# lyclyc52/Instance_NeRF

Measured on AMD Instinct MI355X. Metric: Msamples/sec (train+infer) 3D-FRONT 800x800 at 1/2/4/8 MI355X; PSNR parity, higher is better.
Workload: dtype f32; 1 GPU; render 800x800 synthetic 3D-FRONT-like room, hash-grid NeRF L=16 F=2 T=6119864 sigma+rgb (BASELINE configs[1]), one view per step per GPU; parallelism=views sharded over 1 GPU(s), no data-path collective

## Files before the change

### include/inr.h

```cpp
#ifndef INR_H
#define INR_H

#include <stdint.h>

#ifdef __cplusplus
extern "C" {
#endif

#define INR_ABI_VERSION 13
#define INR_MAX_LEVELS 16

enum {
  INR_OK = 0,
  INR_EINVAL = -1,
  INR_ELAUNCH = -2,
  INR_ENODEV = -3
};

typedef void* inr_stream_t;

enum {
  INR_NUMERICS_TABLE_F16 = 1,
  INR_NUMERICS_MLP_F16 = 2
};

typedef struct inr_grid_desc {
  int32_t num_levels;
  int32_t level_dim;
  uint32_t offsets[INR_MAX_LEVELS + 1];
  float scales[INR_MAX_LEVELS];
  uint32_t resolutions[INR_MAX_LEVELS];
  uint32_t hashed[INR_MAX_LEVELS];
} inr_grid_desc;

int inr_abi_version(void);
const char* inr_last_error(void);
int inr_device_info(int32_t device, int64_t* props);
int inr_set_overlap_placement(int32_t on);
int inr_set_march_mode(int32_t mode);

int inr_get_rays(const float* poses, int64_t B, float fx, float fy, float cx, float cy, int32_t W,
                 const int64_t* inds , int64_t n, float* rays_o, float* rays_d, inr_stream_t s);

int inr_sample_training_batch(const float* pose , float fx, float fy, float cx, float cy, int32_t H, int32_t W,
                              const float* image , int32_t channels, const int32_t* mask ,
                              int32_t num_instances, int64_t seed, int64_t step, int64_t n, int64_t* inds ,
                              float* rays_o, float* rays_d, float* rgb , int64_t* labels ,
                              inr_stream_t s);

int inr_near_far_from_aabb(const float* rays_o, const float* rays_d, const float* aabb ,
                           int64_t N, float min_near, float* nears, float* fars, inr_stream_t s);
int inr_near_far_from_aabb_skip(const float* rays_o, const float* rays_d, const float* aabb , int64_t N,
                                float min_near, const int64_t* labels, int64_t ignore_index, float* nears, float* fars,
                                inr_stream_t s);

int inr_morton3D(const int32_t* coords , int64_t N, int32_t* indices, inr_stream_t s);
int inr_morton3D_invert(const int32_t* indices, int64_t N, int32_t* coords , inr_stream_t s);
int inr_packbits(const float* grid, int64_t n_bytes, float thresh, uint8_t* bitfield, inr_stream_t s);

int inr_mark_untrained_grid(const float* poses, int32_t B, float fx, float fy, float cx, float cy, int32_t H,
                            int32_t cascade, float bound, float* grid , inr_stream_t s);
int inr_occ_cell_positions(const int32_t* morton_idx, const float* noise, int64_t n, int32_t H, float cascade_bound,
                           float* xyz , inr_stream_t s);
int inr_occ_update(float* grid , const float* sigma , const int32_t* morton_idx ,
                   int64_t n_cells, int64_t m, float decay, float density_scale, float* tmp, double* mean_sum,
                   inr_stream_t s);
int inr_packbits_mean(const float* grid, int64_t n_cells , const double* mean_sum, float density_thresh,
                      uint8_t* bitfield, float* mean_out , const int32_t* counters ,
                      int32_t n_counters, int32_t counter_stride , double* stats_out ,
                      inr_stream_t s);
int64_t inr_occ_sample_workspace_bytes(int64_t n_cells);
int inr_occ_sample_cells(const float* grid , int64_t n_cells, const float* u ,
                         int64_t n, int32_t* morton_idx , void* workspace, inr_stream_t s);

int inr_march_write_fills_unowned_rows(int64_t N, int32_t sample_cap, int32_t max_steps);
int64_t inr_march_workspace_bytes(int64_t N, int32_t sample_cap);
int inr_march_rays_train_count(const float* rays_o, const float* rays_d, const uint8_t* bitfield,
                               float bound, float dt_gamma, int32_t max_steps, int64_t N,
                               int32_t cascade, int32_t H, const float* nears, const float* fars,
                               const float* noises , int32_t* rays ,
                               int32_t* counter , void* workspace, int32_t sample_cap, inr_stream_t s);
int inr_march_rays_train_write(const float* rays_o, const float* rays_d, const uint8_t* bitfield,
                               float bound, float dt_gamma, int32_t max_steps, int64_t N,
                               int32_t cascade, int32_t H, int64_t M, const float* nears,
                               const float* fars, const float* noises ,
                               const int32_t* rays , float* xyzs ,
                               float* dirs , float* deltas , const void* workspace,
                               int32_t sample_cap, inr_stream_t s);

int inr_march_rays_patch_write(const float* rays_o, const float* rays_d, const uint8_t* bitfield,
                               float bound, float dt_gamma, int32_t max_steps, int64_t N,
                               int32_t cascade, int32_t H, int64_t M, const float* nears,
                               const float* fars, const float* noises ,
                               const int32_t* rays ,
                               float* xyzs, float* dirs , float* deltas,
                               const void* workspace, int32_t sample_cap, int32_t* ray_ids ,
                               int32_t normalise , inr_stream_t s);
int inr_composite_rays_patch_forward(const float* sigmas, const float* rgbs, const float* deltas,
                                     const int32_t* rays, int64_t N, int64_t M, float T_thresh,
                                     const float* extra , int32_t K,
                                     float* weights_sum, float* depth, float* image,
                                     float* extra_out , float* weights ,
                                     uint64_t* skippable ,
                                     inr_stream_t s);
int inr_project_masks_patch(const float* xyzs, const float* weights, const int32_t* rays, int64_t N, int64_t M,
                            const uint32_t* mask_words, int32_t W, int32_t L, int32_t H, const float* bbox ,
                            int32_t k_total, int32_t k_base, int32_t k_count, float* out, inr_stream_t s);

int inr_march_rays(int64_t n_alive, int32_t n_step, const int32_t* rays_alive, const float* rays_t,
                   const float* rays_o, const float* rays_d, float bound, float dt_gamma,
                   int32_t max_steps, int32_t cascade, int32_t H, const uint8_t* bitfield,
                   const float* nears, const float* fars, float* xyzs, float* dirs, float* deltas,
                   inr_stream_t s);
int inr_composite_rays(int64_t n_alive, int32_t n_step, int32_t* rays_alive, float* rays_t,
                       const float* sigmas, const float* rgbs, const float* deltas,
                       float* weights_sum, float* depth, float* image, float T_thresh,
                       const float* extra , float* extra_acc ,
                       int32_t K, inr_stream_t s);
int inr_compact_alive(const int32_t* rays_alive, int64_t n_alive, int32_t* out, int32_t* n_out,
                      inr_stream_t s);

int inr_composite_rays_train_forward(const float* sigmas, const float* rgbs, const float* deltas,
                                     const int32_t* rays, int64_t N, int64_t M, float T_thresh,
                                     const float* extra , int32_t K,
                                     float* weights_sum, float* depth, float* image,
                                     float* extra_out , float* weights ,
                                     int32_t* sample_ray , inr_stream_t s);
int inr_composite_rays_extra_forward(const float* weights , const float* extra , const int32_t* rays,
                                     int64_t N, int64_t M, int32_t K, float* extra_out ,
                                     const int64_t* labels , int32_t n_classes, int64_t ignore_index,
                                     float* grad_pix, void* workspace, float* loss_out, inr_stream_t s);
int inr_composite_rays_train_backward(const float* grad_weights_sum, const float* grad_image,
                                      const float* grad_extra_out , const float* sigmas,
                                      const float* rgbs, const float* extra, const float* deltas,
                                      const int32_t* rays, const float* weights_sum,
                                      const float* image, const float* weights ,
                                      int64_t N, int64_t M, float T_thresh, int32_t K,
                                      float* grad_sigmas, float* grad_rgbs ,
                                      float* grad_extra , const int32_t* total_dev ,
                                      inr_stream_t s);

int inr_grid_encode_forward(const float* x , const float* embeddings ,
                            const inr_grid_desc* desc , int64_t M, float bound,
                            float* out , inr_stream_t s);
int inr_grid_encode_backward(const float* x, const float* grad_out ,
                             const inr_grid_desc* desc , int64_t M, float bound,
                             float* grad_embeddings , inr_stream_t s);

int inr_grid_encode_backward_ordered(const float* x, const float* grad_out, const int32_t* order,
                                     const inr_grid_desc* desc , int64_t M, float bound,
                                     float* grad_embeddings , inr_stream_t s);
int inr_grid_encode_backward_input(const float* x, const float* grad_out , const float* embeddings,
                                   const inr_grid_desc* desc , int64_t M, float bound, float* grad_x,
                                   inr_stream_t s);
int inr_grid_encode_backward_levels(const float* x, const float* grad_out, const int32_t* order,
                                    const inr_grid_desc* desc, int64_t M, float bound, float* grad_embeddings,
                                    int32_t level_lo, int32_t level_hi, inr_stream_t s);

#define INR_GRID_FX_STATE_FLOATS 4192
int inr_grid_encode_backward_levels_fx(const float* x, const float* grad_out, const int32_t* order,
                                       const inr_grid_desc* desc, int64_t M, float bound, float* grad_embeddings,
                                       int32_t level_lo, int32_t level_hi, float* fx_state ,
                                       inr_stream_t s);
int inr_grid_grad_finish_fx(float* grad_embeddings, const inr_grid_desc* desc , int32_t level_lo,
                            int32_t level_hi, float* fx_state, inr_stream_t s);
int inr_grid_fx_update(float* fx_state, int32_t num_levels, float headroom, int32_t sum_bits , inr_stream_t s);
int inr_grid_encode_backward_levels_fx64(const float* x, const float* grad_out, const int32_t* order,
                                         const inr_grid_desc* desc, int64_t M, float bound, float* grad_embeddings,
                                         int64_t* acc64 , int32_t level_lo, int32_t level_hi, float* fx_state,
                                         inr_stream_t s);
int inr_grid_grad_finish_fx64(int64_t* acc64, float* grad_embeddings, const inr_grid_desc* desc , int32_t level_lo,
                              int32_t level_hi, float* fx_state, inr_stream_t s);

int inr_sh_encode_forward(const float* d , int64_t M, int32_t degree, float* out, inr_stream_t s);
int inr_sh_encode_backward(const float* grad_out, const float* d, int64_t M, int32_t degree,
                           float* grad_d, inr_stream_t s);
int inr_sh_table_q(const float* d , int64_t N, float* out , inr_stream_t s);

int64_t inr_nerf_packed_floats(void);
int inr_nerf_pack_weights(const float* sigma_w0, const float* sigma_w1, const float* color_w0,
                          const float* color_w1, const float* color_w2, float* packed , int32_t numerics);
int64_t inr_instance_packed_floats(int32_t K);
int inr_instance_pack_weights(const float* w0, const float* w1, const float* w2, int32_t K,
                              float* packed , int32_t numerics);
int inr_nerf_forward(const float* x, const float* d, int64_t M, const int32_t* n_samples_dev,
                     float bound, const void* embeddings, const inr_grid_desc* desc ,
                     const float* packed , float density_scale, float* sigma, float* rgb,
                     float* geo_feat, int32_t numerics, inr_stream_t s);
int inr_nerf_forward_table(const float* x01, const int32_t* ray_ids, const float* sh_table_q, int64_t M,
                           float bound, const void* embeddings, const inr_grid_desc* desc ,
                           const float* packed , float density_scale, float* sigma, float* rgb,
                           int32_t numerics, inr_stream_t s);
int64_t inr_nerf_forward_table_sliced_workspace_bytes(int64_t M);
int inr_nerf_forward_table_sliced(const float* x01, const int32_t* ray_ids, const float* sh_table_q, int64_t M,
                                  float bound, const float* embeddings, const inr_grid_desc* desc ,
                                  const float* packed , float density_scale, float* sigma, float* rgb,
                                  float* fine_ws, inr_stream_t s);
int64_t inr_nerf_bwd_packed_floats(void);
int inr_nerf_pack_weights_device(const float* sigma_w0, const float* sigma_w1, const float* color_w0,
                                 const float* color_w1, const float* color_w2, float* packed_fwd,
                                 float* packed_bwd, inr_stream_t s);
int inr_nerf_forward_train(const float* x, const float* d, int64_t M, float bound, const float* embeddings,
                           const inr_grid_desc* desc , const float* packed_fwd, float* sigma, float* rgb,
                           float* enc, float* h1, float* so, float* cin, float* c1, float* c2, inr_stream_t s);
int inr_nerf_backward(const float* grad_sigma, const float* grad_rgb, const float* rgb, const float* so,
                      const float* h1, const float* c1, const float* c2, int64_t M, float density_scale,
                      const float* packed_bwd, float* grad_o, float* grad_zc2, float* grad_zc1, float* grad_so,
                      float* grad_zh1, float* grad_enc, inr_stream_t s);
int inr_nerf_forward_enc(const float* x, const float* d, int64_t M, float bound, const float* embeddings,
                         const inr_grid_desc* desc , const float* packed_fwd, float* sigma, float* rgb,
                         float* enc, inr_stream_t s);
int inr_nerf_head_backward(const float* enc, const float* d, const float* grad_sigma, const float* grad_rgb, int64_t M,
                           float density_scale, const float* packed_fwd, const float* packed_bwd, float* grad_enc,
                           void* workspace, float* grad_ws0, float* grad_ws1, float* grad_wc0, float* grad_wc1,
                           float* grad_wc2, float* zero_buf , int64_t zero_floats, inr_stream_t s);
int64_t inr_instance_bwd_packed_floats(void);
int inr_instance_pack_weights_device(const float* w0 , const float* w1 ,
                                     const float* w2 , int32_t K, float* packed_fwd, float* packed_bwd,
                                     inr_stream_t s);
int inr_instance_forward_train(const float* x, int64_t M, float bound, const float* embeddings,
                               const inr_grid_desc* desc , const float* packed_fwd, int32_t K,
                               float* logits, float* enc, float* h1, float* h2, inr_stream_t s);
int inr_instance_backward(const float* grad_logits, int32_t K, const float* h1, const float* h2, int64_t M,
                          const float* packed_bwd, float* grad_z2, float* grad_z1, float* grad_enc,
                          inr_stream_t s);
int inr_instance_forward_enc(const float* x, int64_t M, const int32_t* n_samples_dev, float bound,
                             const float* embeddings, const inr_grid_desc* desc , const float* packed_fwd,
                             int32_t K, float* logits, float* enc, inr_stream_t s);
int64_t inr_instance_head_workspace_bytes(void);
int inr_instance_head_backward(const float* enc, const float* weights, const int32_t* sample_ray,
                               const float* grad_pix, int32_t K, int64_t N, int64_t M, const int32_t* n_samples_dev,
                               const float* scale_a , const float* scale_b ,
                               const float* packed_fwd, const float* packed_bwd, float* grad_enc, void* workspace,
                               float* grad_w0, float* grad_w1, float* grad_w2, float* zero_buf ,
                               int64_t zero_floats, inr_stream_t s);
int inr_nerf_forward_dirs(const float* x, int64_t M, float bound, const float* embeddings, const inr_grid_desc* desc ,
                          const float* packed , const float* sh_dirs, int32_t n_dirs, float* out, inr_stream_t s);
int inr_nerf_forward_lattice(const float* ax_w, const float* ax_l, const float* ax_h, int32_t W, int32_t L, int32_t H,
                             float bound, const float* embeddings, const inr_grid_desc* desc ,
                             const float* packed , const float* sh_dirs, int32_t n_dirs, float logit_min,
                             float* out, inr_stream_t s);
int inr_instance_forward(const float* x, int64_t M, const int32_t* n_samples_dev, float bound,
                         const float* embeddings, const inr_grid_desc* desc ,
                         const float* packed , int32_t K, float* logits ,
                         inr_stream_t s);
int inr_instance_lattice(const float* ax_w, const float* ax_l, const float* ax_h, int32_t W, int32_t L, int32_t H,
                         float bound, const float* nerf_embeddings, const inr_grid_desc* nerf_desc ,
                         const float* nerf_packed , float density_scale, float sigma_thresh,
                         const float* inst_embeddings, const inr_grid_desc* inst_desc ,
                         const float* inst_packed , int32_t K, uint8_t* labels, float* confidence,
                         float* density_logit, inr_stream_t s);
#define INR_INSTANCE_STATS_WORKSPACE_BYTES (512 * 64 * 8 * 4)
int inr_instance_volume_stats(const uint8_t* labels, const float* confidence, int32_t W, int32_t L, int32_t H, int32_t K,
                              void* workspace, int64_t workspace_bytes, int32_t* counts, int32_t* boxes, float* conf_sum,
                              inr_stream_t s);

int64_t inr_mesh_workspace_bytes(int32_t W, int32_t L, int32_t H, int32_t cap);
int inr_mesh_count(const float* field, int32_t field_stride, float iso, float clamp, const uint8_t* labels ,
                   int32_t select, int32_t W, int32_t L, int32_t H, int32_t cap, void* workspace, int64_t workspace_bytes,
                   int32_t* counts, inr_stream_t s);
int inr_mesh_emit(const float* field, int32_t field_stride, float iso, float clamp, const uint8_t* labels ,
                  int32_t select, const float* rgb , const float* ax_w, const float* ax_l, const float* ax_h,
                  int32_t W, int32_t L, int32_t H, float ext_w, float ext_l, float ext_h, int32_t cap,
                  const void* workspace, int64_t workspace_bytes, int32_t V, int32_t F, float* vertices, int32_t* faces,
                  float* colors , uint8_t* face_labels , inr_stream_t s);

int64_t inr_components_workspace_bytes(int32_t W, int32_t L, int32_t H);
int inr_components_label(const uint8_t* labels, int32_t W, int32_t L, int32_t H, int32_t connectivity, void* workspace,
                         int64_t workspace_bytes, int32_t* roots, inr_stream_t s);
int inr_components_filter(const uint8_t* labels, const int32_t* roots, const float* confidence , int32_t W,
                          int32_t L, int32_t H, int32_t K, int32_t first_channel, int32_t min_voxels, int32_t keep_largest,
                          void* workspace, int64_t workspace_bytes, uint8_t* labels_out, float* confidence_out ,
                          int32_t* n_components, int32_t* kept_voxels, int32_t* kept_root, inr_stream_t s);

int inr_pack_mask_bits(const float* soft, const int64_t* inds , int64_t N, int32_t k, float thresh, int64_t P,
// ... 104 lines not shown
```

### instance_nerf_amd/_lib.py

```python
import ctypes
import os
from ctypes import POINTER, Structure, c_char_p, c_float, c_int32, c_int64, c_uint32, c_void_p

import torch

_HERE = os.path.dirname(os.path.abspath(__file__))
LIB_PATH = os.environ.get("INR_LIB_PATH") or os.path.join(_HERE, "csrc", "libinr_hip.so")
MAX_LEVELS = 16
GRID_FX_STATE_FLOATS = 4192
ROI_MAX_LEVELS = 8
NUMERICS_TABLE_F16, NUMERICS_MLP_F16 = 1, 2


class GridDesc(Structure):
    _fields_ = [("num_levels", c_int32), ("level_dim", c_int32),
                ("offsets", c_uint32 * (MAX_LEVELS + 1)), ("scales", c_float * MAX_LEVELS),
                ("resolutions", c_uint32 * MAX_LEVELS), ("hashed", c_uint32 * MAX_LEVELS)]


P = c_void_p
_SIGS = {
    "inr_abi_version": (c_int32, []),
    "inr_last_error": (c_char_p, []),
    "inr_set_overlap_placement": (c_int32, [c_int32]),
    "inr_set_march_mode": (c_int32, [c_int32]),
    "inr_device_info": (c_int32, [c_int32, POINTER(c_int64)]),
    "inr_get_rays": (c_int32, [P, c_int64, c_float, c_float, c_float, c_float, c_int32, P, c_int64, P, P, P]),
    "inr_sample_training_batch": (c_int32, [P, c_float, c_float, c_float, c_float, c_int32, c_int32, P, c_int32, P, c_int32,
                                            c_int64, c_int64, c_int64, P, P, P, P, P, P]),
    "inr_near_far_from_aabb": (c_int32, [P, P, P, c_int64, c_float, P, P, P]),
    "inr_near_far_from_aabb_skip": (c_int32, [P, P, P, c_int64, c_float, P, c_int64, P, P, P]),
    "inr_morton3D": (c_int32, [P, c_int64, P, P]),
    "inr_morton3D_invert": (c_int32, [P, c_int64, P, P]),
    "inr_packbits": (c_int32, [P, c_int64, c_float, P, P]),
    "inr_mark_untrained_grid": (c_int32, [P, c_int32, c_float, c_float, c_float, c_float, c_int32, c_int32, c_float, P, P]),
    "inr_occ_cell_positions": (c_int32, [P, P, c_int64, c_int32, c_float, P, P]),
    "inr_occ_update": (c_int32, [P, P, P, c_int64, c_int64, c_float, c_float, P, P, P]),
    "inr_packbits_mean": (c_int32, [P, c_int64, P, c_float, P, P, P, c_int32, c_int32, P, P]),
    "inr_occ_sample_workspace_bytes": (c_int64, [c_int64]),
    "inr_occ_sample_cells": (c_int32, [P, c_int64, P, c_int64, P, P, P]),
    "inr_march_write_fills_unowned_rows": (c_int32, [c_int64, c_int32, c_int32]),
    "inr_march_workspace_bytes": (c_int64, [c_int64, c_int32]),
    "inr_march_rays_train_count": (c_int32, [P, P, P, c_float, c_float, c_int32, c_int64, c_int32, c_int32,
                                             P, P, P, P, P, P, c_int32, P]),
    "inr_march_rays_train_write": (c_int32, [P, P, P, c_float, c_float, c_int32, c_int64, c_int32, c_int32,
                                             c_int64, P, P, P, P, P, P, P, P, c_int32, P]),
    "inr_march_rays_patch_write": (c_int32, [P, P, P, c_float, c_float, c_int32, c_int64, c_int32, c_int32,
                                             c_int64, P, P, P, P, P, P, P, P, c_int32, P, c_int32, P]),
    "inr_nerf_bwd_packed_floats": (c_int64, []),
    "inr_nerf_pack_weights_device": (c_int32, [P, P, P, P, P, P, P, P]),
    "inr_nerf_forward_train": (c_int32, [P, P, c_int64, c_float, P, POINTER(GridDesc), P, P, P, P, P, P, P, P, P, P]),
    "inr_nerf_backward": (c_int32, [P, P, P, P, P, P, P, c_int64, c_float, P, P, P, P, P, P, P, P]),
    "inr_instance_bwd_packed_floats": (c_int64, []),
    "inr_instance_pack_weights_device": (c_int32, [P, P, P, c_int32, P, P, P]),
    "inr_instance_forward_train": (c_int32, [P, c_int64, c_float, P, POINTER(GridDesc), P, c_int32, P, P, P, P, P]),
    "inr_instance_backward": (c_int32, [P, c_int32, P, P, c_int64, P, P, P, P, P]),
    "inr_nerf_forward_enc": (c_int32, [P, P, c_int64, c_float, P, POINTER(GridDesc), P, P, P, P, P]),
    "inr_nerf_head_backward": (c_int32, [P, P, P, P, c_int64, c_float, P, P, P, P, P, P, P, P, P, P, c_int64, P]),
    "inr_instance_forward_enc": (c_int32, [P, c_int64, P, c_float, P, POINTER(GridDesc), P, c_int32, P, P, P]),
    "inr_instance_head_workspace_bytes": (c_int64, []),
    "inr_instance_head_backward": (c_int32, [P, P, P, P, c_int32, c_int64, c_int64, P, P, P, P, P, P, P, P, P, P, P, c_int64, P]),
    "inr_adam_step_multi": (c_int32, [c_int32, P, P, P, P, P, P, c_float, c_float, c_float, c_int32, c_float, P]),
    "inr_adam_ema_step_multi": (c_int32, [c_int32, P, P, P, P, P, P, c_float, c_float, c_float, c_int32, c_float, P,
                                          c_float, P]),
    "inr_adam_set_hyper": (c_int32, [P, c_int32, c_float, c_float, c_float, c_int32, P, P]),
    "inr_adam_step_multi_dev": (c_int32, [c_int32, P, P, P, P, P, P, c_float, c_float, c_float, P]),
    "inr_copy_multi": (c_int32, [c_int32, P, P, P, P]),
    "inr_adam_set_hyper_ema": (c_int32, [P, c_int32, c_float, c_float, c_float, c_int32, c_float, P, P]),
    "inr_adam_ema_step_multi_dev": (c_int32, [c_int32, P, P, P, P, P, P, c_float, c_float, c_float, P, P]),
    "inr_cross_entropy": (c_int32, [P, P, c_int64, c_int32, c_int64, P, P, P, P]),
    "inr_finish_rays": (c_int32, [P, P, P, P, P, P, c_float, c_float, c_float, c_int64, P, P, P]),
    "inr_finish_rays_mse": (c_int32, [P, P, P, P, P, c_float, c_float, c_float, P, P, c_int64, P, P, P, P, P]),
    "inr_sh_table_q": (c_int32, [P, c_int64, P, P]),
    "inr_nerf_forward_table": (c_int32, [P, P, P, c_int64, c_float, P, POINTER(GridDesc), P, c_float, P, P, c_int32, P]),
    "inr_nerf_forward_table_sliced_workspace_bytes": (c_int64, [c_int64]),
    "inr_nerf_forward_table_sliced": (c_int32, [P, P, P, c_int64, c_float, P, POINTER(GridDesc), P, c_float, P, P, P, P]),
    "inr_composite_rays_patch_forward": (c_int32, [P, P, P, P, c_int64, c_int64, c_float, P, c_int32, P, P, P, P, P, P, P]),
    "inr_project_masks_patch": (c_int32, [P, P, P, c_int64, c_int64, P, c_int32, c_int32, c_int32, P, c_int32, c_int32, c_int32,
                                          P, P]),
    "inr_march_rays": (c_int32, [c_int64, c_int32, P, P, P, P, c_float, c_float, c_int32, c_int32, c_int32,
                                 P, P, P, P, P, P, P]),
    "inr_composite_rays": (c_int32, [c_int64, c_int32, P, P, P, P, P, P, P, P, c_float, P, P, c_int32, P]),
    "inr_compact_alive": (c_int32, [P, c_int64, P, P, P]),
    "inr_composite_rays_extra_forward": (c_int32, [P, P, P, c_int64, c_int64, c_int32, P, P, c_int32, c_int64, P, P, P, P]),
    "inr_composite_rays_train_forward": (c_int32, [P, P, P, P, c_int64, c_int64, c_float, P, c_int32, P, P, P, P, P, P, P]),
    "inr_composite_rays_train_backward": (c_int32, [P, P, P, P, P, P, P, P, P, P, P, c_int64, c_int64, c_float, c_int32,
                                                    P, P, P, P, P]),
    "inr_grid_encode_forward": (c_int32, [P, P, POINTER(GridDesc), c_int64, c_float, P, P]),
    "inr_grid_encode_backward": (c_int32, [P, P, POINTER(GridDesc), c_int64, c_float, P, P]),
    "inr_grid_encode_backward_ordered": (c_int32, [P, P, P, POINTER(GridDesc), c_int64, c_float, P, P]),
    "inr_grid_encode_backward_input": (c_int32, [P, P, P, POINTER(GridDesc), c_int64, c_float, P, P]),
    "inr_grid_encode_backward_levels": (c_int32, [P, P, P, POINTER(GridDesc), c_int64, c_float, P, c_int32, c_int32, P]),
    "inr_grid_encode_backward_levels_fx": (c_int32, [P, P, P, POINTER(GridDesc), c_int64, c_float, P, c_int32, c_int32, P, P]),
    "inr_grid_grad_finish_fx": (c_int32, [P, POINTER(GridDesc), c_int32, c_int32, P, P]),
    "inr_grid_fx_update": (c_int32, [P, c_int32, c_float, c_int32, P]),
    "inr_grid_encode_backward_levels_fx64": (c_int32, [P, P, P, POINTER(GridDesc), c_int64, c_float, P, P, c_int32, c_int32, P, P]),
    "inr_grid_grad_finish_fx64": (c_int32, [P, P, POINTER(GridDesc), c_int32, c_int32, P, P]),
    "inr_sh_encode_forward": (c_int32, [P, c_int64, c_int32, P, P]),
    "inr_sh_encode_backward": (c_int32, [P, P, c_int64, c_int32, P, P]),
    "inr_nerf_packed_floats": (c_int64, []),
    "inr_nerf_pack_weights": (c_int32, [P, P, P, P, P, P, c_int32]),
    "inr_instance_packed_floats": (c_int64, [c_int32]),
    "inr_instance_pack_weights": (c_int32, [P, P, P, c_int32, P, c_int32]),
    "inr_nerf_forward": (c_int32, [P, P, c_int64, P, c_float, P, POINTER(GridDesc), P, c_float, P, P, P, c_int32, P]),
    "inr_nerf_forward_dirs": (c_int32, [P, c_int64, c_float, P, POINTER(GridDesc), P, P, c_int32, P, P]),
    "inr_nerf_forward_lattice": (c_int32, [P, P, P, c_int32, c_int32, c_int32, c_float, P, POINTER(GridDesc), P, P, c_int32,
                                           c_float, P, P]),
    "inr_instance_forward": (c_int32, [P, c_int64, P, c_float, P, POINTER(GridDesc), P, c_int32, P, P]),
    "inr_instance_lattice": (c_int32, [P, P, P, c_int32, c_int32, c_int32, c_float, P, POINTER(GridDesc), P, c_float,
                                       c_float, P, POINTER(GridDesc), P, c_int32, P, P, P, P]),
    "inr_instance_volume_stats": (c_int32, [P, P, c_int32, c_int32, c_int32, c_int32, P, c_int64, P, P, P, P]),
    "inr_mesh_workspace_bytes": (c_int64, [c_int32, c_int32, c_int32, c_int32]),
    "inr_mesh_count": (c_int32, [P, c_int32, c_float, c_float, P, c_int32, c_int32, c_int32, c_int32, c_int32, P, c_int64, P, P]),
    "inr_mesh_emit": (c_int32, [P, c_int32, c_float, c_float, P, c_int32, P, P, P, P, c_int32, c_int32, c_int32, c_float,
                                c_float, c_float, c_int32, P, c_int64, c_int32, c_int32, P, P, P, P, P]),
    "inr_components_workspace_bytes": (c_int64, [c_int32, c_int32, c_int32]),
    "inr_components_label": (c_int32, [P, c_int32, c_int32, c_int32, c_int32, P, c_int64, P, P]),
    "inr_components_filter": (c_int32, [P, P, P, c_int32, c_int32, c_int32, c_int32, c_int32, c_int32, c_int32, P, c_int64,
                                        P, P, P, P, P, P]),
    "inr_pack_mask_bits": (c_int32, [P, P, c_int64, c_int32, c_float, c_int64, P, P]),
    "inr_match_count": (c_int32, [P, P, c_int64, c_int64, c_int32, c_int32, P, P, P, P, P]),
    "inr_match_assign": (c_int32, [P, P, P, P, P, c_int64, c_int64, c_int32, c_int32, P, P, P, P]),
    "inr_pack_mask_planes": (c_int32, [P, c_int32, c_int64, P, P, P]),
    "inr_pack_label_planes": (c_int32, [P, c_int64, c_int32, c_int32, P, P, P]),
    "inr_mask_overlap": (c_int32, [P, c_int32, P, c_int32, c_int64, c_int32, P, P]),
    "inr_paste_masks": (c_int32, [P, P, c_int32, c_int32, c_int32, c_int32, c_int32, c_float, P, P, P, P]),
    "inr_planes_to_voxel_words": (c_int32, [P, c_int32, c_int64, c_int32, P, P]),
    "inr_nms_3d_pairs": (c_int32, [P, P, c_int32, c_float, P, P]),
    "inr_nms_3d_scan": (c_int32, [P, c_int32, P, P, P]),
    "inr_roi_align_3d_set_mode": (c_int32, [c_int32]),
    "inr_roi_align_3d_forward": (c_int32, [P, P, P, c_int32, c_int32, c_int32, c_int32, c_int32, c_int64, c_int32,
                                           c_int32, c_int32, c_float, P, P]),
    "inr_roi_align_3d_backward": (c_int32, [P, P, P, c_int32, c_int32, c_int32, c_int32, c_int32, c_int64, c_int32,
                                            c_int32, c_int32, c_float, P, P]),
    "inr_roi_align_3d_backward_workspace_bytes": (c_int64, [c_int32, c_int32, c_int32, c_int32, c_int32, c_int64, c_int32,
                                                            c_int32, c_int32]),
    "inr_roi_align_3d_backward_prefers_workspace": (c_int32, [c_int32, c_int32, c_int32, c_int32, c_int32, c_int64, c_int32,
                                                              c_int32, c_int32, c_int64]),
    "inr_roi_align_3d_backward_ws": (c_int32, [P, P, P, c_int32, c_int32, c_int32, c_int32, c_int32, c_int64, c_int32,
                                               c_int32, c_int32, c_float, P, P, c_int64, P]),
    "inr_roi_align_3d_pyramid_forward": (c_int32, [P, P, P, c_int32, P, P, P, P, c_int32, c_int32, c_int64, c_int32,
                                                   c_int32, c_int32, P, P]),
    "inr_roi_align_3d_pyramid_backward": (c_int32, [P, P, P, c_int32, P, P, P, P, c_int32, c_int32, c_int64, c_int32,
                                                    c_int32, c_int32, P, P]),
    "inr_nerf_render": (c_int32, [P, P, P, P, c_int64, c_int64, c_float, P, POINTER(GridDesc), P, c_float, c_float,
                                  P, P, P, P, P, c_int32, c_int32, P]),
    "inr_instance_render": (c_int32, [P, P, P, c_int64, c_int64, c_float, P, POINTER(GridDesc), P, c_int32, P, c_int32, P,
                                      c_int32, P]),
    "inr_linear_wgrad_workspace_bytes": (c_int64, []),
    "inr_linear_wgrad": (c_int32, [P, P, c_int64, c_int32, c_int32, P, P, P]),
    "inr_adam_step": (c_int32, [P, P, P, P, c_int64, c_float, c_float, c_float, c_float, c_int32, c_float, P]),
}
EXPORTS = tuple(_SIGS)

ABI_VERSION = 13
INSTANCE_STATS_WORKSPACE_BYTES = 512 * 64 * 8 * 4
_lib = None


def load():
# ... 76 lines not shown
```

### instance_nerf_amd/build.py

```python
import os
import shutil
import subprocess
import sys

HERE = os.path.dirname(os.path.abspath(__file__))
CSRC = os.path.join(HERE, "csrc")
LIB = os.path.join(CSRC, "libinr_hip.so")
SOURCES = ["raymarch.hip", "encoders.hip", "field_fused.hip", "roialign.hip", "mesh.hip", "components.hip", "match.hip",
           "overlap.hip", "detect.hip"]
HEADERS = ["common.h", "grid_common.h", os.path.join("..", "..", "include", "inr.h")]
FLAGS = ["--offload-arch=gfx950", "-O3", "-std=c++17", "-fPIC", "-ffp-contract=off",
         "-munsafe-fp-atomics", "-Wall", "-Wno-unused-function"]


KERNEL_FILES = {
    "field": ["field_fused.hip", "common.h", "grid_common.h"],
    "scatter": ["encoders.hip", "common.h", "grid_common.h"],
}


def source_sha(kind=None):
    import hashlib
    h = hashlib.sha256()
    for f in sorted(KERNEL_FILES[kind] if kind else SOURCES + HEADERS):
        h.update(f.encode())
        h.update(open(os.path.join(CSRC, f), "rb").read())
    return h.hexdigest()


LIB_FP32 = os.path.join(CSRC, "libinr_hip_fp32.so")


def build_fp32(force=False, verbose=True):
    deps = [os.path.join(CSRC, f) for f in SOURCES + HEADERS] + [os.path.abspath(__file__)]
    if not force and os.path.exists(LIB_FP32) and all(os.path.getmtime(d) <= os.path.getmtime(LIB_FP32) for d in deps):
        return LIB_FP32
    hipcc = shutil.which("hipcc") or "/opt/rocm/bin/hipcc"
    objs = []
    for src in SOURCES:
        obj = os.path.join(CSRC, src.replace(".hip", ".fp32.o"))
        cmd = [hipcc, "-x", "hip", "-c", os.path.join(CSRC, src), "-o", obj, "-DINR_MLP_FP32=1"] + FLAGS
        if verbose:
            print(" ".join(cmd), flush=True)
        subprocess.check_call(cmd)
        objs.append(obj)
    subprocess.check_call([hipcc, "-shared", "-o", LIB_FP32] + objs + ["--offload-arch=gfx950"])
    return LIB_FP32


def _stale():
    if not os.path.exists(LIB):
        return True
    t = os.path.getmtime(LIB)
    deps = [os.path.join(CSRC, f) for f in SOURCES + HEADERS] + [os.path.abspath(__file__)]
    return any(os.path.getmtime(d) > t for d in deps)


def build(force=False, verbose=True):
    if not force and not _stale():
        return LIB
    hipcc = shutil.which("hipcc") or "/opt/rocm/bin/hipcc"
    if not os.path.exists(hipcc):
        raise RuntimeError("hipcc not found: cannot build libinr_hip.so")
    objs = []
    for src in SOURCES:
        obj = os.path.join(CSRC, src.replace(".hip", ".o"))
        cmd = [hipcc, "-x", "hip", "-c", os.path.join(CSRC, src), "-o", obj] + FLAGS
        if verbose:
            print(" ".join(cmd), flush=True)
        subprocess.check_call(cmd)
        objs.append(obj)
    cmd = [hipcc, "-shared", "-o", LIB] + objs + ["--offload-arch=gfx950"]
    if verbose:
        print(" ".join(cmd), flush=True)
    subprocess.check_call(cmd)
    return LIB


if __name__ == "__main__":
    build(force="--force" in sys.argv)
    build_fp32(force="--force" in sys.argv)
    print(LIB)
```

### instance_nerf_amd/csrc/field_fused.hip

```cpp
#include <atomic>
#include <mutex>
#include <type_traits>

#include "common.h"
#include "grid_common.h"

namespace inr {

typedef float f32x4 __attribute__((ext_vector_type(4)));
typedef __bf16 bf16x8 __attribute__((ext_vector_type(8)));

#ifndef INR_MLP_FP32
#define INR_MLP_FP32 0
#endif

#ifdef INR_PROBE_BUILD
#include "probe/field_probe.h"
#else
#if defined(INR_PROBE_MODE) || defined(INR_PROBE_STATIC) || defined(INR_PROBE_SLOW_XCD)
#error "INR_PROBE_* switches need -DINR_PROBE_BUILD (tools/build_probe.py): those variants produce wrong results"
#endif
#define INR_PROBE_PROLOGUE()
#define INR_PROBE_SCHEDULE(steal)
#define INR_PROBE_TILE()
#define INR_PROBE_AFTER_GATHER()
#define INR_PROBE_GEO_IS_OUTPUT 1
#define INR_PROBE_EPILOGUE()
#endif


constexpr int kSig0 = 0;
constexpr int kSig1 = kSig0 + 64 * 32;
constexpr int kCol0 = kSig1 + 16 * 64;
constexpr int kCol1 = kCol0 + 64 * 32;
constexpr int kCol2 = kCol1 + 64 * 64;
constexpr int kNerfFloats = kCol2 + 16 * 64;
constexpr int kIns0 = 0;
constexpr int kIns1 = kIns0 + 64 * 32;
constexpr int kIns2 = kIns1 + 64 * 64;

__host__ __device__ inline int frag_pos(int mt, int ks, int lane, int n_ks) {
  return ((mt * (n_ks / 4) + ks / 4) * 64 + lane) * 4 + (ks & 3);
}

__device__ __forceinline__ f32x4 mfma4(const float4 a, const f32x4 b, f32x4 c) {
  c = __builtin_amdgcn_mfma_f32_16x16x4f32(a.x, b[0], c, 0, 0, 0);
  c = __builtin_amdgcn_mfma_f32_16x16x4f32(a.y, b[1], c, 0, 0, 0);
  c = __builtin_amdgcn_mfma_f32_16x16x4f32(a.z, b[2], c, 0, 0, 0);
  c = __builtin_amdgcn_mfma_f32_16x16x4f32(a.w, b[3], c, 0, 0, 0);
  return c;
}
__device__ __forceinline__ float relu1(float x) { return __int_as_float(max(__float_as_int(x), 0)); }
__device__ __forceinline__ f32x4 relu4(f32x4 v) {
  v[0] = relu1(v[0]); v[1] = relu1(v[1]); v[2] = relu1(v[2]); v[3] = relu1(v[3]);
  return v;
}

struct LevelRec {
  uint4 a, b;
};
constexpr int kLevelRecBytes = 16 * sizeof(LevelRec);

__device__ __forceinline__ void stage_level_recs(const GridDesc& G, LevelRec* recs) {
  const int t = threadIdx.x;
  if (t < 16) {
    const int q = t >> 2, li = t & 3;
    const int l = (li >> 1) * 8 + 2 * q + (li & 1);
    const bool live = l < G.num_levels;
    const int lc = live ? l : 0;
    const uint32_t m = G.mask[lc], s = G.res1[lc];
    LevelRec r;
    r.a.x = live ? __float_as_uint(G.scales[lc]) : 0u;
    r.a.y = live ? G.offsets[lc] * 8u : 0u;
    r.a.z = !live ? 0u : (m ? 2654435761u : s);
    r.a.w = !live ? 0u : (m ? 805459861u : s * s);
    r.b.x = !live ? 0u : (m ? m : 0xFFFFFFFFu);
    r.b.y = (live && m) ? 1u : 0u;
    r.b.z = (live && m) ? 0xFFFFFFFFu : 0u;
    r.b.w = (live && !m) ? 0xFFFFFFFFu : 0u;
    recs[t] = r;
  }
}

__device__ __forceinline__ bool slot_all_hashed(const GridDesc& G, int li) {
  bool ah = true;
#pragma unroll
  for (int qq = 0; qq < 4; ++qq) {
    const int lq = (li >> 1) * 8 + 2 * qq + (li & 1);
// ... 469 lines not shown
  bool dyn;
  __device__ __forceinline__ void init(const TileSched& sched, unsigned long long* cursors) {
    s = sched; cur = cursors; lane = threadIdx.x & 63; it = 0; dyn = false; sub = kStealDraw; k_base = 0; raw_next = 0;
    own = owner = (int)(((blockIdx.x >> 3) % kStealPools) * 8 + (blockIdx.x & 7));
    if (!cursors) s.hybrid = false;
    if (!s.hybrid) s.static_local = s.main_local;
  }
  __device__ __forceinline__ int64_t pool_len(int o) const {
    const int64_t nb = (s.local_end(o & 7) - s.static_local + (1 << kStealBlockLog2) - 1) >> kStealBlockLog2;
    const int p = o >> 3;
    return nb > p ? ((nb - p + kStealPools - 1) / kStealPools) << kStealBlockLog2 : 0;
  }
  __device__ __forceinline__ int64_t local_of(int o, int64_t k) const {
    return s.static_local + ((((k >> kStealBlockLog2) * kStealPools) + (o >> 3)) << kStealBlockLog2) +
           (k & ((1 << kStealBlockLog2) - 1));
  }
  __device__ __forceinline__ unsigned long long issue(int o) const {
    unsigned long long v = 0;
    if (lane == 0) v = atomicAdd(cur + o, (unsigned long long)kStealDraw);
    return v;
  }
  __device__ __forceinline__ static int64_t uniform(unsigned long long v) {
    return (int64_t)(((unsigned long long)(uint32_t)__builtin_amdgcn_readfirstlane((int)(v >> 32)) << 32) |
                     (uint32_t)__builtin_amdgcn_readfirstlane((int)v));
  }
  __device__ __forceinline__ int scan() const {
    bool live = false;
    if (lane < kStealOwners) live = (int64_t)__hip_atomic_load(cur + lane, __ATOMIC_RELAXED, __HIP_MEMORY_SCOPE_AGENT) < pool_len(lane);
    const uint32_t mask = (uint32_t)__ballot(live);
    for (int i = 0; i < kStealOwners; ++i) {
      const int o = (((own >> 3) + i) % kStealPools) * 8 + (((own & 7) + i / kStealPools) & 7);
      if ((mask >> o) & 1u) return o;
    }
    return -1;
  }
  __device__ __forceinline__ int64_t next() {
    if (!dyn) {
      if (!s.hybrid) {
        const int64_t t = s.tile(it++);
        return t < s.hi ? t : -1;
      }
      const int64_t u = s.first + (it++) * s.stride;
      if (u < s.static_local) return s.tile_of((int)s.xcd, u);
      dyn = true;
      raw_next = issue(owner);
    }
    for (;;) {
      if (sub < kStealDraw) {
        const int64_t u = local_of(owner, k_base + sub);
        ++sub;
        if (u < s.local_end(owner & 7)) return s.tile_of(owner & 7, u);
        continue;
      }
      int64_t k = uniform(raw_next);
      while (k >= pool_len(owner)) {
        const int o = scan();
        if (o < 0) return -1;
        owner = o;
        k = uniform(issue(owner));
      }
      k_base = k;
      sub = 0;
      raw_next = issue(owner);
    }
  }
};
constexpr int kFieldMinWaves = 2;

__device__ __forceinline__ f32x4 load4(const float* p) {
  const float4 v = *reinterpret_cast<const float4*>(p);
  return f32x4{v.x, v.y, v.z, v.w};
}
__device__ __forceinline__ void store4(float* p, f32x4 v) {
  *reinterpret_cast<float4*>(p) = make_float4(v[0], v[1], v[2], v[3]);
}
__device__ __forceinline__ f32x4 mask4(f32x4 g, f32x4 h) {
  return f32x4{h[0] > 0.f ? g[0] : 0.f, h[1] > 0.f ? g[1] : 0.f, h[2] > 0.f ? g[2] : 0.f, h[3] > 0.f ? g[3] : 0.f};
}

struct NerfSave {
  float *enc, *h1, *so, *cin, *c1, *c2;
};

template <bool kColor, bool kTable = false, int kSave = 0, bool kHalf = false, bool kFast = false, bool kPre = false>
__global__ void __launch_bounds__(kFieldThreads, kFieldMinWaves) k_nerf_fwd(const float* __restrict__ x, const float* __restrict__ d,
                                                               int64_t M, const int32_t* __restrict__ n_dev, float bound,
                                                               const float2* __restrict__ emb, uint32_t emb_bytes, GridDesc G,
                                                               const float4* __restrict__ packed, float density_scale,
                                                               float* __restrict__ sigma, float* __restrict__ rgb,
                                                               float* __restrict__ geo, const int32_t* __restrict__ ray_ids,
                                                               const float4* __restrict__ shq, NerfSave sv,
                                                               unsigned long long* __restrict__ steal) {
  extern __shared__ __attribute__((aligned(16))) float4 wl[];
  INR_PROBE_PROLOGUE();
  __builtin_amdgcn_s_setprio(3);
  constexpr int kStage = (kColor ? kNerfFloats : kCol0) / 4;
  for (int i = threadIdx.x; i < kStage; i += kFieldThreads) wl[i] = packed[i];
  LevelRec* recs = reinterpret_cast<LevelRec*>(wl + kStage);
  stage_level_recs(G, recs);
  __syncthreads();

  constexpr int kWaves = kFieldThreads / 64;
  const int lane = threadIdx.x & 63, q = lane >> 4, j = lane & 15;
  int64_t n = M;
  if (n_dev) n = min((int64_t)*n_dev, M);
  const int64_t n_tiles = (n + 15) >> 4;
  const float rb = 2.0f * bound;
  const float rb_inv = 0.0f;
  INR_PROBE_SCHEDULE(steal);
  TileWalk walk;
  walk.init(make_sched(n_tiles, kWaves, steal != nullptr), steal);

  const bool all_hashed[4] = {slot_all_hashed(G, 0), slot_all_hashed(G, 1), slot_all_hashed(G, 2), slot_all_hashed(G, 3)};
  const __amdgpu_buffer_rsrc_t rsrc = __builtin_amdgcn_make_buffer_rsrc((void*)emb, 0, (int)emb_bytes, 0x00020000);

  for (int64_t tile = walk.next(); tile >= 0; tile = walk.next()) {
    INR_PROBE_TILE();
    const int64_t m = tile * 16 + j;
    const bool valid = m < n;
    TileIn me;
    f32x4 sh_in = {0.f, 0.f, 0.f, 0.f};
    if constexpr (kTable) {
      const int64_t mm = valid ? m : n - 1;
      me.x0 = x[mm * 3 + 0]; me.x1 = x[mm * 3 + 1]; me.x2 = x[mm * 3 + 2];
      const float4 t4 = shq[(int64_t)ray_ids[mm] * 4 + q];
      sh_in = f32x4{t4.x, t4.y, t4.z, t4.w};
    } else {
      load_tile_in<kColor>(x, d, valid ? m : n - 1, bound, rb, rb_inv, me);
    }

    f32x4 enc[2];
    {
      Gathered g;
      uint32_t rec_off = (uint32_t)q * 4u * (uint32_t)sizeof(LevelRec);
      asm volatile("" : "+v"(rec_off));
      typedef float v2f __attribute__((ext_vector_type(2)));
      v2f fine_a = {0.f, 0.f}, fine_b = {0.f, 0.f};
      if constexpr (kPre) {
        static_assert(!kPre || kTable, "the sliced feed is a variant of the table feed");
        static_assert(kSliceLevels == 3, "lane map below");
        const v2f* pre = reinterpret_cast<const v2f*>(d);
        const int64_t m_pad = (M + 31) & ~(int64_t)31, mm = valid ? m : n - 1;
        const int sl = (q & 1) ? 1 : 0;
        fine_a = __builtin_nontemporal_load(pre + (int64_t)sl * m_pad + mm);
        fine_b = __builtin_nontemporal_load(pre + (int64_t)(sl + 1) * m_pad + mm);
      }
      issue_gathers<kHalf, kPre>(reinterpret_cast<const LevelRec*>(reinterpret_cast<const char*>(recs) + rec_off), all_hashed,
                                 rsrc, me.x0, me.x1, me.x2, g);
      __builtin_amdgcn_sched_barrier(0);
      blend<kHalf>(g, enc[0], enc[1]);
      if constexpr (kPre) {
        if (q == 2) enc[1] = f32x4{enc[1][0], enc[1][1], fine_a.x, fine_a.y};
        else if (q == 3) enc[1] = f32x4{fine_a.x, fine_a.y, fine_b.x, fine_b.y};
      }
    }
    if constexpr (!kTable) {
      if (me.oob) enc[0] = enc[1] = f32x4{0.f, 0.f, 0.f, 0.f};
    }
    INR_PROBE_AFTER_GATHER();

    f32x4 h1[4];
    mlp_layer<4, 2, kFast>(wl + kSig0 / 4, lane, enc, h1);
#pragma unroll
    for (int t = 0; t < 4; ++t) h1[t] = relu4(h1[t]);
    f32x4 h2[1];
    mlp_layer<1, 4, kFast>(wl + kSig1 / 4, lane, h1, h2);

    if (valid) {
      if (q == 0) sigma[m] = __expf(h2[0][0]) * density_scale;
      if (INR_PROBE_GEO_IS_OUTPUT && geo) {
#pragma unroll
        for (int r = 0; r < 4; ++r) {
          const int row = 4 * q + r;
          if (row >= 1) geo[m * 15 + row - 1] = h2[0][r];
        }
      }
    }

    if constexpr (kColor) {
      f32x4 cin[2];
      if constexpr (kTable) {
        cin[0] = sh_in;
      } else {
        float sh[16];
        sh4(me.d0, me.d1, me.d2, sh);
#pragma unroll
        for (int ks = 0; ks < 4; ++ks) cin[0][ks] = select4(q, sh[4 * ks], sh[4 * ks + 1], sh[4 * ks + 2], sh[4 * ks + 3]);
      }
      cin[1] = h2[0];
      f32x4 c1[4], c2[4], o[1];
      mlp_layer<4, 2, kFast>(wl + kCol0 / 4, lane, cin, c1);
#pragma unroll
      for (int t = 0; t < 4; ++t) c1[t] = relu4(c1[t]);
      mlp_layer<4, 4, kFast>(wl + kCol1 / 4, lane, c1, c2);
#pragma unroll
      for (int t = 0; t < 4; ++t) c2[t] = relu4(c2[t]);
      mlp_layer<1, 4, kFast>(wl + kCol2 / 4, lane, c2, o);
      if constexpr (kSave == 2) {
        if (valid) {
#pragma unroll
          for (int t = 0; t < 2; ++t) store4(sv.enc + m * 32 + 16 * t + 4 * q, enc[t]);
        }
      }
      if constexpr (kSave == 1) {
        if (valid) {
// ... 1523 lines not shown
};

struct FieldTable {
  GridDesc G;
  const float2* emb;
  uint32_t bytes;
};
static int field_table(const char* what, const inr_grid_desc* desc, const void* emb, bool half, FieldTable& t) {
  if (int rc = make_grid_desc(desc, t.G)) return rc;
  const uint64_t bytes = (uint64_t)desc->offsets[desc->num_levels] * (half ? 4ull : 8ull);
  if (bytes >= (1ull << 31)) {
    set_error("%s: table larger than 2 GiB is not addressable by the 32-bit gather offsets", what);
    return INR_EINVAL;
  }
  t.emb = reinterpret_cast<const float2*>(emb);
  t.bytes = (uint32_t)bytes;
  return INR_OK;
}
static const float4* f4(const float* p) { return reinterpret_cast<const float4*>(p); }

struct HybridSchedule {
  StealSet set;
  bool begin(hipStream_t s, int64_t n_tiles) {
    if ((n_tiles >> (kXcdChunkLog2 + 3)) < 4 || stream_is_capturing(s)) return true;
    set = steal_cursors(s);
    return set.cursors != nullptr;
  }
  unsigned long long* cursors() const { return set.cursors; }
  void finish(hipStream_t s) { steal_release(set, s); }
};

template <typename Kern, typename... Args>
static void launch_field(Kern kern, size_t lds, int64_t n_tiles, hipStream_t s, Args... args) {
  kern<<<grid_for(kern, lds, n_tiles), kFieldThreads, lds, s>>>(args...);
}

template <typename F>
static void with_kmt(int k_mt, F&& f) {
  switch (k_mt) {
    case 1: f(std::integral_constant<int, 1>{}); break;
    case 2: f(std::integral_constant<int, 2>{}); break;
    case 3: f(std::integral_constant<int, 3>{}); break;
    default: f(std::integral_constant<int, 4>{}); break;
  }
}
template <typename F>
static void with_flag(bool on, F&& f) {
  if (on) f(std::true_type{});
  else f(std::false_type{});
}
template <typename F>
static void with_mlp_f16(bool on, F&& f) {
#if !INR_MLP_FP32
  if (on) return f(std::true_type{});
#endif
  f(std::false_type{});
}

constexpr int kNumericsO = INR_NUMERICS_TABLE_F16 | INR_NUMERICS_MLP_F16;
constexpr unsigned kAcceptPlainOrO = 1u | 1u << kNumericsO;
constexpr unsigned kAcceptAny = 0xFu;
constexpr unsigned kAcceptPack = 1u | 1u << INR_NUMERICS_MLP_F16;
static int check_numerics(const char* what, int32_t numerics, unsigned accepted) {
  if (numerics < 0 || numerics > 3 || !((accepted >> numerics) & 1u)) {
    set_error("%s: numerics %d is not accepted here", what, numerics);
    return INR_EINVAL;
  }
#if INR_MLP_FP32
  if (numerics & INR_NUMERICS_MLP_F16) {
    set_error("%s: INR_NUMERICS_MLP_F16 is not available in the exact-fp32 build", what);
    return INR_EINVAL;
  }
#endif
  return INR_OK;
}

template <class KIdx>
static void pack_section_as(int32_t numerics, float* dst, const float* W, int n_out, int n_in, int n_mt, int n_ks,
                            KIdx kidx) {
  if (numerics & INR_NUMERICS_MLP_F16) pack_section_f16(dst, W, n_out, n_in, n_mt, n_ks, kidx);
  else pack_section(dst, W, n_out, n_in, n_mt, n_ks, kidx);
}

}

using namespace inr;

extern "C" {

int64_t inr_nerf_packed_floats(void) { return kNerfFloats; }

int inr_nerf_pack_weights(const float* sigma_w0, const float* sigma_w1, const float* color_w0, const float* color_w1,
                          const float* color_w2, float* packed, int32_t numerics) {
  INR_REQUIRE(sigma_w0 && sigma_w1 && color_w0 && color_w1 && color_w2 && packed, "null pointer");
  if (int rc = check_numerics(__func__, numerics, kAcceptPack)) return rc;
  pack_section_as(numerics, packed + kSig0, sigma_w0, 64, 32, 4, 8, kidx_enc);
  pack_section_as(numerics, packed + kSig1, sigma_w1, 16, 64, 1, 16, kidx_hidden);
  pack_section_as(numerics, packed + kCol0, color_w0, 64, 31, 4, 8, kidx_color_in);
  pack_section_as(numerics, packed + kCol1, color_w1, 64, 64, 4, 16, kidx_hidden);
  pack_section_as(numerics, packed + kCol2, color_w2, 3, 64, 1, 16, kidx_hidden);
  return INR_OK;
}

int64_t inr_instance_packed_floats(int32_t K) {
  INR_REQUIRE(K > 0 && K <= 64 && K % 16 == 0, "K must be 16, 32, 48 or 64");
  return kIns2 + K * 64;
}

int inr_instance_pack_weights(const float* w0, const float* w1, const float* w2, int32_t K, float* packed,
                              int32_t numerics) {
  INR_REQUIRE(w0 && w1 && w2 && packed, "null pointer");
  INR_REQUIRE(K > 0 && K <= 64 && K % 16 == 0, "K must be 16, 32, 48 or 64");
  if (int rc = check_numerics(__func__, numerics, kAcceptPack)) return rc;
  pack_section_as(numerics, packed + kIns0, w0, 64, 32, 4, 8, kidx_enc);
  pack_section_as(numerics, packed + kIns1, w1, 64, 64, 4, 16, kidx_hidden);
  pack_section_as(numerics, packed + kIns2, w2, K, 64, K / 16, 16, kidx_hidden);
  return INR_OK;
}

int inr_nerf_forward(const float* x, const float* d, int64_t M, const int32_t* n_samples_dev, float bound,
                     const void* embeddings, const inr_grid_desc* desc, const float* packed, float density_scale,
                     float* sigma, float* rgb, float* geo_feat, int32_t numerics, inr_stream_t s) {
  const bool o = numerics == kNumericsO;
  INR_REQUIRE(M >= 0 && desc, "bad argument");
  if (M == 0) return INR_OK;
  INR_REQUIRE(x && embeddings && packed && sigma && (rgb || !o), "null pointer");
  INR_REQUIRE(!rgb || d, "rgb requested without view directions");
  INR_REQUIRE(!(o && geo_feat), "no geo_feat under the -O numerics");
  INR_REQUIRE(((uintptr_t)embeddings & (o ? 3 : 7)) == 0 && ((uintptr_t)packed & 15) == 0, "embeddings/packed misaligned");
  FieldTable t;
  if (int rc = field_table(__func__, desc, embeddings, o, t)) return rc;
  if (int rc = check_numerics(__func__, numerics, kAcceptPlainOrO)) return rc;
  const int64_t n_tiles = (M + 15) / 16;
  const hipStream_t st = as_stream(s);
  HybridSchedule hybrid;
  if (!o && !hybrid.begin(st, n_tiles)) return INR_ELAUNCH;
  const size_t lds = (rgb ? kNerfFloats : kCol0) * sizeof(float) + kLevelRecBytes;
  const auto launch = [&](auto kern) {
    launch_field(kern, lds, n_tiles, st, x, d, M, n_samples_dev, bound, t.emb, t.bytes, t.G, f4(packed), density_scale,
                 sigma, rgb, geo_feat, nullptr, nullptr, NerfSave{}, hybrid.cursors());
  };
  with_mlp_f16(o, [&](auto fast) {
    if constexpr (decltype(fast)::value) launch(k_nerf_fwd<true, false, 0, true, true>);
    else if (rgb) launch(k_nerf_fwd<true>);
    else launch(k_nerf_fwd<false>);
  });
  hybrid.finish(st);
  return check_launch("nerf_forward");
}

int inr_nerf_forward_table(const float* x01, const int32_t* ray_ids, const float* sh_table_q, int64_t M, float bound,
                           const void* embeddings, const inr_grid_desc* desc, const float* packed, float density_scale,
                           float* sigma, float* rgb, int32_t numerics, inr_stream_t s) {
  INR_REQUIRE(M >= 0 && desc, "bad argument");
  if (M == 0) return INR_OK;
  INR_REQUIRE(x01 && ray_ids && sh_table_q && embeddings && packed && sigma && rgb, "null pointer");
  INR_REQUIRE(((uintptr_t)embeddings & 7) == 0 && ((uintptr_t)packed & 15) == 0 && ((uintptr_t)sh_table_q & 15) == 0,
              "embeddings/packed/sh_table_q misaligned");
  FieldTable t;
  if (int rc = field_table(__func__, desc, embeddings, numerics & INR_NUMERICS_TABLE_F16, t)) return rc;
  if (int rc = check_numerics(__func__, numerics, kAcceptAny)) return rc;
  const size_t lds = std::max(kNerfFloats * sizeof(float) + kLevelRecBytes, (size_t)g_field_lds_min);
  const int64_t n_tiles = (M + 15) / 16;
  const hipStream_t st = as_stream(s);
  HybridSchedule hybrid;
  if (!hybrid.begin(st, n_tiles)) return INR_ELAUNCH;
  with_flag(numerics & INR_NUMERICS_TABLE_F16, [&](auto half) {
    with_mlp_f16(numerics & INR_NUMERICS_MLP_F16, [&](auto fast) {
      launch_field(k_nerf_fwd<true, true, 0, decltype(half)::value, decltype(fast)::value>, lds, n_tiles, st, x01,
                   nullptr, M, nullptr, bound, t.emb, t.bytes, t.G, f4(packed), density_scale, sigma, rgb, nullptr,
                   ray_ids, f4(sh_table_q), NerfSave{}, hybrid.cursors());
    });
  });
  hybrid.finish(st);
  return check_launch("nerf_forward_table");
}

int64_t inr_nerf_forward_table_sliced_workspace_bytes(int64_t M) {
  return M < 0 ? -1 : kSliceLevels * ((M + 31) & ~(int64_t)31) * (int64_t)sizeof(float2);
}

int inr_nerf_forward_table_sliced(const float* x01, const int32_t* ray_ids, const float* sh_table_q, int64_t M, float bound,
                                  const float* embeddings, const inr_grid_desc* desc, const float* packed,
                                  float density_scale, float* sigma, float* rgb, float* fine_ws, inr_stream_t s) {
  INR_REQUIRE(M >= 0 && desc, "bad argument");
  if (M == 0) return INR_OK;
  INR_REQUIRE(x01 && ray_ids && sh_table_q && embeddings && packed && sigma && rgb && fine_ws, "null pointer");
  INR_REQUIRE(((uintptr_t)embeddings & 7) == 0 && ((uintptr_t)packed & 15) == 0 && ((uintptr_t)sh_table_q & 15) == 0 &&
              ((uintptr_t)fine_ws & 7) == 0, "embeddings/packed/sh_table_q/fine_ws misaligned");
  INR_REQUIRE(desc->num_levels == 16, "the sliced frame path needs the 16-level table");
  for (int l = 8; l < 16; ++l) INR_REQUIRE(desc->hashed[l], "the sliced frame path needs hashed fine levels (8..15)");
  FieldTable t;
  if (int rc = field_table(__func__, desc, embeddings, false, t)) return rc;
  const size_t lds = std::max(kNerfFloats * sizeof(float) + kLevelRecBytes, (size_t)g_field_lds_min);
  hipStream_t st = as_stream(s);
  static int fit = 0;
  if (fit < 1 && (hipOccupancyMaxActiveBlocksPerMultiprocessor(&fit, k_grid_fine_slices, kSliceThreads, 0) != hipSuccess || fit < 1))
    fit = 4;
  const int64_t per_wg = 32 * kSliceTilesPerIter * (kSliceThreads / 64);
  const int gx = (int)std::max<int64_t>(1, std::min<int64_t>((M + per_wg - 1) / per_wg, (int64_t)cu_count() * fit));
  k_grid_fine_slices<<<dim3(gx, kSliceLevels), kSliceThreads, 0, st>>>(x01, M, t.emb, t.bytes, t.G, fine_ws);
  HybridSchedule hybrid;
  if (!hybrid.begin(st, (M + 15) / 16)) return INR_ELAUNCH;
  launch_field(k_nerf_fwd<true, true, 0, false, false, true>, lds, (M + 15) / 16, st, x01, fine_ws, M, nullptr, bound,
               t.emb, t.bytes, t.G, f4(packed), density_scale, sigma, rgb, nullptr, ray_ids, f4(sh_table_q), NerfSave{},
               hybrid.cursors());
  hybrid.finish(st);
  return check_launch("nerf_forward_table_sliced");
}

int inr_nerf_forward_dirs(const float* x, int64_t M, float bound, const float* embeddings, const inr_grid_desc* desc,
                          const float* packed, const float* sh_dirs, int32_t n_dirs, float* out, inr_stream_t s) {
  INR_REQUIRE(M >= 0 && desc, "bad argument");
  if (M == 0) return INR_OK;
  INR_REQUIRE(x && embeddings && packed && sh_dirs && out, "null pointer");
  INR_REQUIRE(n_dirs >= 1 && n_dirs <= kMaxExtractDirs, "1..8 view directions");
  INR_REQUIRE(((uintptr_t)embeddings & 7) == 0 && ((uintptr_t)packed & 15) == 0 && ((uintptr_t)out & 15) == 0,
              "embeddings/packed/out misaligned");
  FieldTable t;
  if (int rc = field_table(__func__, desc, embeddings, false, t)) return rc;
  const size_t lds = kNerfFloats * sizeof(float) + kLevelRecBytes + kMaxExtractDirs * 16 * sizeof(float);
  launch_field(k_nerf_fwd_dirs<false>, lds, (M + 15) / 16, as_stream(s), x, M, bound, t.emb, t.bytes, t.G, f4(packed),
               sh_dirs, n_dirs, reinterpret_cast<float4*>(out), LatticeDesc{}, -INFINITY);
  return check_launch("nerf_forward_dirs");
}

int inr_nerf_forward_lattice(const float* ax_w, const float* ax_l, const float* ax_h, int32_t W, int32_t L, int32_t H,
                             float bound, const float* embeddings, const inr_grid_desc* desc, const float* packed,
                             const float* sh_dirs, int32_t n_dirs, float logit_min, float* out, inr_stream_t s) {
  INR_REQUIRE(W >= 0 && L >= 0 && H >= 0 && desc, "bad argument");
  if ((int64_t)W * L * H == 0) return INR_OK;
  INR_REQUIRE(ax_w && ax_l && ax_h && embeddings && packed && sh_dirs && out, "null pointer");
  INR_REQUIRE(n_dirs >= 1 && n_dirs <= kMaxExtractDirs, "1..8 view directions");
  INR_REQUIRE(((uintptr_t)embeddings & 7) == 0 && ((uintptr_t)packed & 15) == 0 && ((uintptr_t)out & 15) == 0,
              "embeddings/packed/out misaligned");
  FieldTable t;
  if (int rc = field_table(__func__, desc, embeddings, false, t)) return rc;
  LatticeDesc lat{ax_w, ax_l, ax_h, W, L, H, (W + 15) / 16 * 16};
  const int64_t M = (int64_t)lat.Wp * L * H;
  const size_t lds = kNerfFloats * sizeof(float) + kLevelRecBytes + kMaxExtractDirs * 16 * sizeof(float);
  launch_field(k_nerf_fwd_dirs<true>, lds, (M + 15) / 16, as_stream(s), nullptr, M, bound, t.emb, t.bytes, t.G,
               f4(packed), sh_dirs, n_dirs, reinterpret_cast<float4*>(out), lat, logit_min);
  return check_launch("nerf_forward_lattice");
}

int inr_instance_forward(const float* x, int64_t M, const int32_t* n_samples_dev, float bound, const float* embeddings,
                         const inr_grid_desc* desc, const float* packed, int32_t K, float* logits, inr_stream_t s) {
  INR_REQUIRE(M >= 0 && desc, "bad argument");
  if (M == 0) return INR_OK;
  INR_REQUIRE(x && embeddings && packed && logits, "null pointer");
  INR_REQUIRE(K > 0 && K <= 64 && K % 16 == 0, "K must be 16, 32, 48 or 64");
  INR_REQUIRE(((uintptr_t)embeddings & 7) == 0 && ((uintptr_t)packed & 15) == 0 && ((uintptr_t)logits & 15) == 0,
              "embeddings/packed/logits misaligned");
  FieldTable t;
  if (int rc = field_table(__func__, desc, embeddings, false, t)) return rc;
  const size_t lds = (size_t)(kIns2 + K * 64) * sizeof(float) + kLevelRecBytes;
  with_kmt(K / 16, [&](auto kmt) {
    launch_field(k_instance_fwd<decltype(kmt)::value>, lds, (M + 15) / 16, as_stream(s), x, M, n_samples_dev, bound,
// ... 331 lines not shown
```

### instance_nerf_amd/csrc/raymarch.hip

```cpp
#include "common.h"

namespace inr {

static thread_local char g_err[512] = "";
int g_field_lds_min = 0;
int g_march_lds_pad = 0;
void set_error(const char* fmt, ...) {
  va_list ap;
  va_start(ap, fmt);
  vsnprintf(g_err, sizeof(g_err), fmt, ap);
  va_end(ap);
}

constexpr int kRayBlock = 256;
constexpr float kSqrt3x2 = 3.4641016151377544f;

__global__ void __launch_bounds__(kRayBlock) k_near_far(const float* __restrict__ rays_o,
                                                        const float* __restrict__ rays_d,
                                                        const float* __restrict__ aabb, int64_t N,
                                                        float min_near, float* __restrict__ nears,
                                                        float* __restrict__ fars,
                                                        const int64_t* __restrict__ labels, int64_t ignore) {
  const int64_t n = (int64_t)blockIdx.x * blockDim.x + threadIdx.x;
  if (n >= N) return;
  float near = -INFINITY, far = INFINITY;
  bool miss = labels != nullptr && labels[n] == ignore;
#pragma unroll
  for (int a = 0; a < 3; ++a) {
    const float o = rays_o[n * 3 + a];
    const float rd = 1.0f / rays_d[n * 3 + a];
    const float t0 = (aabb[a] - o) * rd;
    const float t1 = (aabb[a + 3] - o) * rd;
    const float lo = t0 > t1 ? t1 : t0;
    const float hi = t0 > t1 ? t0 : t1;
    if (a > 0) miss = miss || (near > hi) || (lo > far);
    near = lo > near ? lo : near;
    far = hi < far ? hi : far;
  }
  if (near < min_near) near = min_near;
  nears[n] = miss ? 3.402823466e+38f : near;
  fars[n] = miss ? 3.402823466e+38f : far;
}

__global__ void __launch_bounds__(kRayBlock) k_get_rays(const float* __restrict__ poses, int64_t B, float fx, float fy,
                                                        float cx, float cy, int W, const int64_t* __restrict__ inds,
                                                        int64_t n, float* __restrict__ rays_o,
                                                        float* __restrict__ rays_d) {
  const int64_t idx = (int64_t)blockIdx.x * blockDim.x + threadIdx.x;
  if (idx >= B * n) return;
  const int64_t b = idx / n, k = idx - b * n;
  const int64_t pix = inds ? inds[k] : k;
  const float i = (float)(pix % W) + 0.5f, j = (float)(pix / W) + 0.5f;
  const float xs = (i - cx) / fx, ys = (j - cy) / fy;
  const float nrm = sqrtf(xs * xs + ys * ys + 1.0f * 1.0f);
  const float dx = xs / nrm, dy = ys / nrm, dz = 1.0f / nrm;
  const float* P = poses + b * 16;
#pragma unroll
  for (int r = 0; r < 3; ++r) {
    rays_d[idx * 3 + r] = dx * P[r * 4 + 0] + dy * P[r * 4 + 1] + dz * P[r * 4 + 2];
    rays_o[idx * 3 + r] = P[r * 4 + 3];
  }
}

__device__ __forceinline__ uint64_t mix64(uint64_t z) {
  z = (z ^ (z >> 30)) * 0xBF58476D1CE4E5B9ull;
  z = (z ^ (z >> 27)) * 0x94D049BB133111EBull;
  return z ^ (z >> 31);
}
__global__ void __launch_bounds__(kRayBlock) k_sample_batch(const float* __restrict__ pose, float fx, float fy, float cx,
                                                            float cy, int H, int W, const float* __restrict__ image,
                                                            int C, const int32_t* __restrict__ mask, int num_instances,
                                                            uint64_t seed, uint64_t step, int64_t n,
                                                            int64_t* __restrict__ inds, float* __restrict__ rays_o,
                                                            float* __restrict__ rays_d, float* __restrict__ rgb,
                                                            int64_t* __restrict__ labels) {
  const int64_t k = (int64_t)blockIdx.x * blockDim.x + threadIdx.x;
  if (k >= n) return;
  const uint64_t h = mix64(seed + 0x9E3779B97F4A7C15ull * ((step << 32) + (uint64_t)k));
  const uint64_t pix = ((h >> 32) * (uint64_t)((int64_t)H * W)) >> 32;
  inds[k] = (int64_t)pix;
  const float i = (float)(pix % (uint64_t)W) + 0.5f, j = (float)(pix / (uint64_t)W) + 0.5f;
  const float xs = (i - cx) / fx, ys = (j - cy) / fy;
  const float nrm = sqrtf(xs * xs + ys * ys + 1.0f * 1.0f);
// ... 98 lines not shown
  for (int64_t i = n4 * 4 + (int64_t)blockIdx.x * blockDim.x + threadIdx.x; i < n; i += (int64_t)gridDim.x * blockDim.x) {
    bool changed = false;
    const float g = cell(grid[i], tmp[i], changed);
    if (changed) grid[i] = g;
  }
#pragma unroll
  for (int d = 32; d >= 1; d >>= 1) acc += __shfl_xor(acc, d, 64);
  if ((threadIdx.x & 63) == 0) red[threadIdx.x >> 6] = acc;
  __syncthreads();
  if (threadIdx.x == 0) atomicAdd(mean_sum, red[0] + red[1] + red[2] + red[3]);
}
__global__ void k_packbits_mean(const float* __restrict__ grid, int64_t n_bytes, const double* __restrict__ mean_sum,
                                double inv_cells, float density_thresh, uint8_t* __restrict__ bits,
                                float* __restrict__ mean_out, const int32_t* __restrict__ counters, int n_counters,
                                int counter_stride, double* __restrict__ stats_out) {
  const int64_t n = (int64_t)blockIdx.x * blockDim.x + threadIdx.x;
  const float mean = (float)(*mean_sum * inv_cells);
  if (n == 0 && mean_out) *mean_out = mean;
  if (n == 0 && stats_out) {
    int64_t total = 0;
    for (int k = 0; k < n_counters; ++k) total += counters[(int64_t)k * counter_stride];
    stats_out[0] = (double)mean;
    stats_out[1] = (double)total;
  }
  if (n >= n_bytes) return;
  const float thresh = fminf(mean, density_thresh);
  const float4 a = reinterpret_cast<const float4*>(grid)[n * 2];
  const float4 b = reinterpret_cast<const float4*>(grid)[n * 2 + 1];
  uint32_t v = (a.x > thresh) | ((a.y > thresh) << 1) | ((a.z > thresh) << 2) | ((a.w > thresh) << 3) |
               ((b.x > thresh) << 4) | ((b.y > thresh) << 5) | ((b.z > thresh) << 6) | ((b.w > thresh) << 7);
  bits[n] = (uint8_t)v;
}

struct MarchParams {
  const uint8_t* bits;
  float bound, dt_gamma, dt_min, dt_max, rH;
  int C, H, H3;
};

struct Ray {
  float ox, oy, oz, dx, dy, dz, rdx, rdy, rdz, sx, sy, sz;
};

__device__ __forceinline__ Ray load_ray(const float* __restrict__ o, const float* __restrict__ d, int64_t n) {
  Ray r;
  r.ox = o[n * 3]; r.oy = o[n * 3 + 1]; r.oz = o[n * 3 + 2];
  r.dx = d[n * 3]; r.dy = d[n * 3 + 1]; r.dz = d[n * 3 + 2];
  r.rdx = 1.0f / r.dx; r.rdy = 1.0f / r.dy; r.rdz = 1.0f / r.dz;
  r.sx = copysignf(1.0f, r.dx); r.sy = copysignf(1.0f, r.dy); r.sz = copysignf(1.0f, r.dz);
  return r;
}

__device__ __forceinline__ float step_dt(const MarchParams& P, float t) {
  return clampf(t * P.dt_gamma, P.dt_min, P.dt_max);
}
template <bool kConst>
struct StepRule {
  float c;
  __device__ __forceinline__ explicit StepRule(const MarchParams& P) : c(step_dt(P, 0.0f)) {}
  __device__ __forceinline__ float operator()(const MarchParams& P, float t) const {
    if constexpr (kConst) return c;
    else return step_dt(P, t);
  }
};

struct MortonCalc {
  __device__ __forceinline__ uint32_t operator()(uint32_t x, uint32_t y, uint32_t z) const { return morton3(x, y, z); }
};
struct MortonLut {
  const uint32_t* lut;
  __device__ __forceinline__ uint32_t operator()(uint32_t x, uint32_t y, uint32_t z) const {
    return lut[x] | (lut[y] << 1) | (lut[z] << 2);
  }
};

template <bool kSingle = false, bool kConstDt = false, class Emit, class Advance, class Morton = MortonCalc>
__device__ __forceinline__ int march_ray(const MarchParams& P, const Ray& r, float t, float far,
                                         int max_emit, Emit&& emit, Advance&& advance, Morton morton = Morton()) {
  int n = 0;
  float last_t = t;
  const StepRule<kConstDt> step(P);
  const float mb1 = fminf(ldexpf(1.0f, 0), P.bound), rmb1 = 1.0f / mb1;
  while (t < far && n < max_emit) {
    const float px = clampf(r.ox + t * r.dx, -P.bound, P.bound);
    const float py = clampf(r.oy + t * r.dy, -P.bound, P.bound);
    const float pz = clampf(r.oz + t * r.dz, -P.bound, P.bound);
    const float dt = step(P, t);
    int level = 0;
    float mb = mb1, rmb = rmb1;
    if constexpr (!kSingle) {
      int e0, e1;
      (void)frexpf(fmaxf(fabsf(px), fmaxf(fabsf(py), fabsf(pz))), &e0);
      (void)frexpf(dt * (float)P.H * 0.5f, &e1);
      level = max(clampi(e0, 0, P.C - 1), clampi(e1, 0, P.C - 1));
      mb = fminf(ldexpf(1.0f, level), P.bound);
      rmb = 1.0f / mb;
    }
    const int nx = clampi((int)(((px * rmb + 1.0f) * 0.5f) * (float)P.H), 0, P.H - 1);
    const int ny = clampi((int)(((py * rmb + 1.0f) * 0.5f) * (float)P.H), 0, P.H - 1);
    const int nz = clampi((int)(((pz * rmb + 1.0f) * 0.5f) * (float)P.H), 0, P.H - 1);
    const uint32_t idx = (uint32_t)level * (uint32_t)P.H3 + morton((uint32_t)nx, (uint32_t)ny, (uint32_t)nz);
    const bool occ = (P.bits[idx >> 3] >> (idx & 7)) & 1;
    if (occ) {
      const float tn = t + dt;
      emit(px, py, pz, dt, tn - last_t, t);
      t = tn;
      advance();
      last_t = tn;
      ++n;
    } else {
      const float ax = ((float)nx + 0.5f) + 0.5f * r.sx;
      const float ay = ((float)ny + 0.5f) + 0.5f * r.sy;
      const float az = ((float)nz + 0.5f) + 0.5f * r.sz;
      const float cx = (((ax * P.rH) * 2.0f - 1.0f) * mb - px) * r.rdx;
      const float cy = (((ay * P.rH) * 2.0f - 1.0f) * mb - py) * r.rdy;
      const float cz = (((az * P.rH) * 2.0f - 1.0f) * mb - pz) * r.rdz;
      const float tt = t + fmaxf(0.0f, fminf(cx, fminf(cy, cz)));
      do {
        t = t + step(P, t);
        advance();
      } while (t < tt);
    }
  }
  return n;
}
template <class Emit>
__device__ __forceinline__ int march_ray(const MarchParams& P, const Ray& r, float t, float far,
                                         int max_emit, Emit&& emit) {
  return P.dt_gamma == 0.0f ? march_ray<false, true>(P, r, t, far, max_emit, emit, [] {})
                            : march_ray<false, false>(P, r, t, far, max_emit, emit, [] {});
}
template <class Emit, class Advance, class Morton>
__device__ __forceinline__ int march_ray_any(const MarchParams& P, const Ray& r, float t, float far,
                                             int max_emit, Emit&& emit, Advance&& advance, Morton morton) {
  if (P.dt_gamma == 0.0f)
    return P.C == 1 ? march_ray<true, true>(P, r, t, far, max_emit, emit, advance, morton)
                    : march_ray<false, true>(P, r, t, far, max_emit, emit, advance, morton);
  return P.C == 1 ? march_ray<true, false>(P, r, t, far, max_emit, emit, advance, morton)
                  : march_ray<false, false>(P, r, t, far, max_emit, emit, advance, morton);
}

__device__ __forceinline__ float start_t(const MarchParams& P, float near, float noise) {
  return near + step_dt(P, near) * noise;
}

__global__ void __launch_bounds__(kRayBlock) k_march_count(MarchParams P, const float* __restrict__ rays_o,
                                                           const float* __restrict__ rays_d, int64_t N,
                                                           int max_steps, const float* __restrict__ nears,
                                                           const float* __restrict__ fars,
                                                           const float* __restrict__ noises,
                                                           int32_t* __restrict__ counts,
                                                           int32_t* __restrict__ block_sums,
                                                           uint32_t* __restrict__ mask, int cap_words) {
  __shared__ int32_t wsum[kRayBlock / 64];
  __shared__ uint32_t lut[1024];
  for (int i = threadIdx.x; i < P.H; i += kRayBlock) lut[i] = expand_bits10((uint32_t)i);
  __syncthreads();
  const MortonLut morton{lut};
  const int64_t n = (int64_t)blockIdx.x * blockDim.x + threadIdx.x;
  int cnt = 0;
  if (n < N) {
    const Ray r = load_ray(rays_o, rays_d, n);
    const float t0 = start_t(P, nears[n], noises ? noises[n] : 0.0f);
    if (cap_words > 0) {
      uint32_t word = 0;
      int widx = 0, cand = 0;
      bool ok = true;
      cnt = march_ray_any(P, r, t0, fars[n], max_steps,
                      [&](float, float, float, float, float, float) {
// ... 12 lines not shown
                      [&] { ++cand; }, morton);
      if (widx < cap_words) mask[(int64_t)widx * N + n] = word;
      mask[(int64_t)cap_words * N + n] = ok ? 1u : 0u;
    } else {
      cnt = march_ray_any(P, r, t0, fars[n], max_steps, [](float, float, float, float, float, float) {}, [] {}, morton);
    }
    counts[n] = cnt;
  }
  const int incl = wave_inclusive_scan(cnt);
  if ((threadIdx.x & 63) == 63) wsum[threadIdx.x >> 6] = incl;
  __syncthreads();
  if (threadIdx.x == 0) {
    int s = 0;
#pragma unroll
    for (int w = 0; w < kRayBlock / 64; ++w) s += wsum[w];
    block_sums[blockIdx.x] = s;
  }
}

__global__ void __launch_bounds__(1024) k_scan_block_sums(int32_t* __restrict__ block_sums, int n_blocks,
                                                          int64_t N, int32_t* __restrict__ counter) {
  __shared__ int32_t wsum[16];
  __shared__ int32_t carry_s;
  if (threadIdx.x == 0) carry_s = 0;
  __syncthreads();
  for (int base = 0; base < n_blocks; base += 1024) {
    const int i = base + threadIdx.x;
    const int v = i < n_blocks ? block_sums[i] : 0;
    const int incl = wave_inclusive_scan(v);
    if ((threadIdx.x & 63) == 63) wsum[threadIdx.x >> 6] = incl;
    __syncthreads();
    int wave_off = 0;
    for (int w = 0; w < (int)(threadIdx.x >> 6); ++w) wave_off += wsum[w];
    const int carry = carry_s;
    if (i < n_blocks) block_sums[i] = carry + wave_off + incl - v;
    __syncthreads();
    if (threadIdx.x == 1023) carry_s = carry + wave_off + incl;
    __syncthreads();
  }
  if (threadIdx.x == 0) {
    counter[0] = carry_s;
    counter[1] = (int32_t)N;
  }
}

__global__ void __launch_bounds__(kRayBlock) k_finalize_offsets(const int32_t* __restrict__ counts,
                                                                const int32_t* __restrict__ block_prefix,
                                                                int64_t N, int32_t* __restrict__ rays) {
  __shared__ int32_t wsum[kRayBlock / 64];
  const int64_t n = (int64_t)blockIdx.x * blockDim.x + threadIdx.x;
  const int cnt = n < N ? counts[n] : 0;
  const int incl = wave_inclusive_scan(cnt);
  if ((threadIdx.x & 63) == 63) wsum[threadIdx.x >> 6] = incl;
  __syncthreads();
  int off = block_prefix[blockIdx.x] + incl - cnt;
  for (int w = 0; w < (int)(threadIdx.x >> 6); ++w) off += wsum[w];
  if (n < N) {
    rays[n * 3 + 0] = (int32_t)n;
    rays[n * 3 + 1] = off;
    rays[n * 3 + 2] = cnt;
  }
}

template <bool kConstDt, class Emit>
__device__ __forceinline__ void replay_ray_t(const MarchParams& P, const Ray& r, const uint32_t* __restrict__ mask, int64_t N,
                                             int64_t n, float t, int cnt, Emit&& emit) {
  const StepRule<kConstDt> step(P);
  float last_t = t;
  int emitted = 0;
  for (int w = 0; emitted < cnt; ++w) {
    const uint32_t bits = mask[(int64_t)w * N + n];
    for (int b0 = 0; b0 < 32; b0 += 8) {
      const uint32_t sub = (bits >> b0) & 0xFFu;
      if (__ballot(sub != 0u) == 0ull) {
#pragma unroll
        for (int j = 0; j < 8; ++j) t = t + step(P, t);
        continue;
      }
#pragma unroll
      for (int j = 0; j < 8; ++j) {
        const float dt = step(P, t);
        const float tn = t + dt;
        if (sub & (1u << j)) {
          const float px = clampf(r.ox + t * r.dx, -P.bound, P.bound);
          const float py = clampf(r.oy + t * r.dy, -P.bound, P.bound);
          const float pz = clampf(r.oz + t * r.dz, -P.bound, P.bound);
          emit(px, py, pz, dt, tn - last_t, t);
          last_t = tn;
          ++emitted;
        }
        t = tn;
      }
    }
  }
}
template <class Emit>
__device__ __forceinline__ void replay_ray(const MarchParams& P, const Ray& r, const uint32_t* __restrict__ mask, int64_t N,
                                           int64_t n, float t, int cnt, Emit&& emit) {
  if (P.dt_gamma == 0.0f) replay_ray_t<true>(P, r, mask, N, n, t, cnt, emit);
  else replay_ray_t<false>(P, r, mask, N, n, t, cnt, emit);
}

__global__ void __launch_bounds__(kRayBlock) k_march_write(MarchParams P, const float* __restrict__ rays_o,
                                                           const float* __restrict__ rays_d, int64_t N,
                                                           int64_t M, const float* __restrict__ nears,
                                                           const float* __restrict__ fars,
                                                           const float* __restrict__ noises,
                                                           const int32_t* __restrict__ rays,
                                                           float* __restrict__ xyzs, float* __restrict__ dirs,
                                                           float* __restrict__ deltas,
                                                           const uint32_t* __restrict__ mask, int cap_words) {
  const int64_t n = (int64_t)blockIdx.x * blockDim.x + threadIdx.x;
  if (n >= N) return;
  const int off = rays[n * 3 + 1];
  const int cnt = rays[n * 3 + 2];
  if (cnt == 0 || (int64_t)off + cnt > M) return;
  const Ray r = load_ray(rays_o, rays_d, n);
  int64_t i = off;
  auto emit = [&](float px, float py, float pz, float dt, float delta, float) {
    xyzs[i * 3 + 0] = px; xyzs[i * 3 + 1] = py; xyzs[i * 3 + 2] = pz;
    dirs[i * 3 + 0] = r.dx; dirs[i * 3 + 1] = r.dy; dirs[i * 3 + 2] = r.dz;
    deltas[i * 2 + 0] = dt; deltas[i * 2 + 1] = delta;
    ++i;
  };
  const float t0 = start_t(P, nears[n], noises ? noises[n] : 0.0f);
  if (cap_words > 0 && mask[(int64_t)cap_words * N + n]) {
    replay_ray(P, r, mask, N, n, t0, cnt, emit);
  } else {
    march_ray(P, r, t0, fars[n], cnt, emit);
  }
}

template <bool kSingle = false, class Emit>
__device__ __forceinline__ int march_ray_coop(const MarchParams& P, const Ray& r, float t, float far, int max_emit,
                                              Emit&& emit) {
  const float mb1 = fminf(ldexpf(1.0f, 0), P.bound), rmb1 = 1.0f / mb1;
  const int lane = threadIdx.x & 63;
  const uint64_t lt_mask = (1ull << lane) - 1ull;
  int n = 0;
  float last_t = t;
  while (t < far && n < max_emit) {
    float c = t;
    if (P.dt_gamma == 0.0f) {
      const float dt0 = step_dt(P, t);
      asm volatile(
          ".rept 63\n"
          "s_nop 1\n"
          "v_add_f32_dpp %0, %0, %1 wave_shr:1 row_mask:0xf bank_mask:0xf\n"
          ".endr\n"
          : "+v"(c)
          : "v"(dt0));
    } else {
      for (int j = 0; j < 63; ++j) c = j < lane ? c + step_dt(P, c) : c;
    }
    const bool in = c < far;
    const float px = clampf(r.ox + c * r.dx, -P.bound, P.bound);
    const float py = clampf(r.oy + c * r.dy, -P.bound, P.bound);
    const float pz = clampf(r.oz + c * r.dz, -P.bound, P.bound);
    const float dt = step_dt(P, c);
    const float tn = c + dt;
    int level = 0;
    float mb = mb1, rmb = rmb1;
    if constexpr (!kSingle) {
      int e0, e1;
      (void)frexpf(fmaxf(fabsf(px), fmaxf(fabsf(py), fabsf(pz))), &e0);
      (void)frexpf(dt * (float)P.H * 0.5f, &e1);
      level = max(clampi(e0, 0, P.C - 1), clampi(e1, 0, P.C - 1));
      mb = fminf(ldexpf(1.0f, level), P.bound);
      rmb = 1.0f / mb;
    }
    const int nx = clampi((int)(((px * rmb + 1.0f) * 0.5f) * (float)P.H), 0, P.H - 1);
    const int ny = clampi((int)(((py * rmb + 1.0f) * 0.5f) * (float)P.H), 0, P.H - 1);
    const int nz = clampi((int)(((pz * rmb + 1.0f) * 0.5f) * (float)P.H), 0, P.H - 1);
    const uint32_t idx = (uint32_t)level * (uint32_t)P.H3 + morton3((uint32_t)nx, (uint32_t)ny, (uint32_t)nz);
    const bool occ = (P.bits[idx >> 3] >> (idx & 7)) & 1;
    const float ax = ((float)nx + 0.5f) + 0.5f * r.sx;
    const float ay = ((float)ny + 0.5f) + 0.5f * r.sy;
    const float az = ((float)nz + 0.5f) + 0.5f * r.sz;
    const float cx = (((ax * P.rH) * 2.0f - 1.0f) * mb - px) * r.rdx;
    const float cy = (((ay * P.rH) * 2.0f - 1.0f) * mb - py) * r.rdy;
    const float cz = (((az * P.rH) * 2.0f - 1.0f) * mb - pz) * r.rdz;
    const float tt = c + fmaxf(0.0f, fminf(cx, fminf(cy, cz)));
    int lo = lane + 1, hi = 64;
    bool settled_all = false;
    if (P.dt_gamma == 0.0f) {
      const int i0 = lane + (int)fminf((tt - c) * (1.0f / dt), 64.0f);
      const float ca = __shfl(c, clampi(i0 - 1, 0, 63), 64);
      const float cb = __shfl(c, min(i0, 63), 64);
      const float cc = __shfl(c, min(i0 + 1, 63), 64);
      const bool lt_a = i0 - 1 <= lane || ca < tt;
      const bool ge_b = i0 >= 64 || !(cb < tt);
      const bool ge_c = i0 + 1 >= 64 || !(cc < tt);
      const bool take_b = i0 > lane && ge_b;
      const bool settled = take_b ? lt_a : ge_c;
      lo = take_b ? min(i0, 64) : i0 + 1;
      settled_all = __ballot(in && !occ && !settled) == 0;
    }
    if (!settled_all) {
      lo = lane + 1;
#pragma unroll
      for (int it = 0; it < 7; ++it) {
        const int mid = (lo + hi) >> 1;
        const float cm = __shfl(c, min(mid, 63), 64);
        const bool below = mid < 64 && cm < tt;
        if (lo < hi) {
          if (below) lo = mid + 1; else hi = mid;
        }
      }
    }
    const int next = lo;
    const uint64_t in_mask = __ballot(in);
    const uint64_t miss_mask = __ballot(in && !occ);
    const int n_in = __popcll(in_mask);
    uint64_t visited = 0;
    int v = 0, last_miss = -1;
    while (v < n_in) {
      const uint64_t rest = miss_mask >> v;
      const int m = rest ? v + __builtin_ctzll(rest) : 64;
      const int stop = min(m, n_in);
      if (stop > v) visited |= (stop - v >= 64 ? ~0ull : ((1ull << (stop - v)) - 1ull)) << v;
      if (m >= n_in) { v = stop; last_miss = -1; break; }
      visited |= 1ull << m;
      last_miss = m;
      v = __builtin_amdgcn_readlane(next, m);
    }
    uint64_t emit_mask = visited & in_mask & ~miss_mask;
    int k_new = __popcll(emit_mask);
    bool full = false;
    if (n + k_new >= max_emit) {
      full = true;
      const int keep = max_emit - n;
      uint64_t m2 = emit_mask;
      for (int i = 0; i < keep; ++i) m2 &= m2 - 1;
      emit_mask &= ~m2;
      k_new = keep;
    }
    const uint64_t before = emit_mask & lt_mask;
    const int prev = before ? 63 - __builtin_clzll(before) : 0;
    const float prev_tn = __shfl(tn, prev, 64);
    if ((emit_mask >> lane) & 1ull) {
      const float last = before ? prev_tn : last_t;
// ... 651 lines not shown
    }
    float alpha = 0.f, d0 = 0.f, cr = 0.f, cg = 0.f, cb = 0.f;
    if (act) {
      d0 = deltas[i * 2];
      alpha = 1.0f - expf(-sigmas[i] * d0);
      cr = rgbs[i * 3]; cg = rgbs[i * 3 + 1]; cb = rgbs[i * 3 + 2];
    }
    const float P = wave_incl_prod(1.0f - alpha, lane);
    float Pprev = __shfl_up(P, 1, 64);
    if (lane == 0) Pprev = 1.0f;
    const float T = T_carry * Pprev, Tn = T_carry * P;
    const bool used = act && (T >= T_thresh || (base + lane) == 0);
    const float w = used ? alpha * T : 0.0f;
    const float ar = cr_carry + wave_incl_sum(w * cr, lane);
    const float ag = cg_carry + wave_incl_sum(w * cg, lane);
    const float ab = cb_carry + wave_incl_sum(w * cb, lane);
    if (act) {
      grad_rgbs[i * 3] = gr * w; grad_rgbs[i * 3 + 1] = gg * w; grad_rgbs[i * 3 + 2] = gb * w;
      grad_sigmas[i] = used ? d0 * (gr * (Tn * cr - (rf - ar)) + gg * (Tn * cg - (gf - ag)) + gb * (Tn * cb - (bf - ab)) +
                                    gw * (1.0f - wsf))
                            : 0.0f;
    }
    T_carry *= __shfl(P, 63, 64);
    cr_carry = __shfl(ar, 63, 64); cg_carry = __shfl(ag, 63, 64); cb_carry = __shfl(ab, 63, 64);
    if (!(T_carry >= T_thresh)) dead = true;
  }
}

__global__ void __launch_bounds__(kRayBlock) k_composite_train_extra_bwd(
    const float* __restrict__ g_extra_out, const float* __restrict__ wbuf, const int32_t* __restrict__ rays, int64_t N,
    int64_t M, int K, float* __restrict__ grad_extra) {
  const int64_t n = ((int64_t)blockIdx.x * blockDim.x + threadIdx.x) >> 6;
  const int lane = threadIdx.x & 63;
  if (n >= N) return;
  const int32_t rid = rays[n * 3], off = rays[n * 3 + 1];
  int32_t cnt = rays[n * 3 + 2];
  if ((int64_t)off + cnt > M) cnt = 0;
  if (lane >= K) return;
  const float g = g_extra_out[(int64_t)rid * K + lane];
  for (int s = 0; s < cnt; ++s) grad_extra[((int64_t)off + s) * K + lane] = wbuf[(int64_t)off + s] * g;
}

constexpr int kGroup = 16;

struct GroupCursor {
  int c[kGroup];
  int S;
  int r;
  int k;
  __device__ __forceinline__ void init(int my_count, int my_offset) {
    const int lane = threadIdx.x & 63, g0 = lane & ~(kGroup - 1);
    r = lane & (kGroup - 1);
#pragma unroll
    for (int i = 0; i < kGroup; ++i) c[i] = __shfl(my_count, g0 + i, 64);
    S = __shfl(my_offset, g0, 64);
    k = 0;
  }
  __device__ __forceinline__ int total() const {
    int t = 0;
#pragma unroll
    for (int i = 0; i < kGroup; ++i) t += c[i];
    return t;
  }
  int nact_ = 0, rank_ = 0, k_change_ = 0;
  __device__ __forceinline__ int next() {
    if (k >= k_change_) {
      int nact = 0, rank = 0, nxt = 0x7FFFFFFF;
#pragma unroll
      for (int i = 0; i < kGroup; ++i) {
        const bool gt = c[i] > k;
        nact += gt ? 1 : 0;
        rank += (gt && i < r) ? 1 : 0;
        nxt = gt ? min(nxt, c[i]) : nxt;
      }
      nact_ = nact; rank_ = rank; k_change_ = nxt;
    }
    const int slot = S + rank_;
    S += nact_;
    ++k;
    return slot;
  }
};

__global__ void __launch_bounds__(kRayBlock) k_march_write_patch(MarchParams P, const float* __restrict__ rays_o,
                                                                 const float* __restrict__ rays_d, int64_t N, int64_t M,
                                                                 const float* __restrict__ nears,
                                                                 const float* __restrict__ fars,
                                                                 const float* __restrict__ noises,
                                                                 const int32_t* __restrict__ rays,
                                                                 float* __restrict__ xyzs, float* __restrict__ dirs,
                                                                 float* __restrict__ deltas,
                                                                 const uint32_t* __restrict__ mask, int cap_words,
                                                                 int32_t* __restrict__ ray_ids, int normalise) {
  const int64_t n = (int64_t)blockIdx.x * blockDim.x + threadIdx.x;
  const int off = n < N ? rays[n * 3 + 1] : 0;
  const int cnt = n < N ? rays[n * 3 + 2] : 0;
  GroupCursor cur;
  cur.init(cnt, off);
  if (cnt == 0 || (int64_t)cur.S + cur.total() > M) return;
  const Ray r = load_ray(rays_o, rays_d, n);
  const float rb = 2.0f * P.bound;
  auto emit = [&](float px, float py, float pz, float dt, float delta, float) {
    const int64_t i = cur.next();
    if (normalise) {
      px = (px + P.bound) / rb; py = (py + P.bound) / rb; pz = (pz + P.bound) / rb;
    }
    xyzs[i * 3 + 0] = px; xyzs[i * 3 + 1] = py; xyzs[i * 3 + 2] = pz;
    if (dirs) { dirs[i * 3 + 0] = r.dx; dirs[i * 3 + 1] = r.dy; dirs[i * 3 + 2] = r.dz; }
    if (ray_ids) ray_ids[i] = (int32_t)n;
    deltas[i * 2 + 0] = dt; deltas[i * 2 + 1] = delta;
  };
  const float t0 = start_t(P, nears[n], noises ? noises[n] : 0.0f);
  if (cap_words > 0 && mask[(int64_t)cap_words * N + n]) {
    replay_ray(P, r, mask, N, n, t0, cnt, emit);
  } else {
    march_ray(P, r, t0, fars[n], cnt, emit);
  }
}

__global__ void __launch_bounds__(kRayBlock) k_composite_patch_fwd(const float* __restrict__ sigmas,
                                                                   const float* __restrict__ rgbs,
                                                                   const float* __restrict__ deltas,
                                                                   const int32_t* __restrict__ rays, int64_t N, int64_t M,
                                                                   float T_thresh, float* __restrict__ wbuf,
                                                                   float* __restrict__ weights_sum,
                                                                   float* __restrict__ depth, float* __restrict__ image,
                                                                   unsigned long long* __restrict__ skippable) {
  const int64_t n = (int64_t)blockIdx.x * blockDim.x + threadIdx.x;
  const int lane = threadIdx.x & 63, g0 = lane & ~(kGroup - 1), rr = lane & (kGroup - 1);
  const int32_t rid = n < N ? rays[n * 3] : 0;
  const int off = n < N ? rays[n * 3 + 1] : 0;
  int cnt = n < N ? rays[n * 3 + 2] : 0;
  int S = __shfl(off, g0, 64);
  int gtot = cnt;
#pragma unroll
  for (int d = 1; d < kGroup; d <<= 1) gtot += __shfl_xor(gtot, d, 64);
  if ((int64_t)S + gtot > M) cnt = 0;
  int maxc = cnt;
#pragma unroll
  for (int d = 1; d < 64; d <<= 1) maxc = max(maxc, __shfl_xor(maxc, d, 64));
  float T = 1.0f, r = 0, g = 0, b = 0, ws = 0, t = 0, dsum = 0;
  bool done = false;
  unsigned n_skip = 0;
  constexpr int kAhead = 8;
  for (int k = 0; k < maxc; k += kAhead) {
    unsigned field[kAhead];
    int64_t slot[kAhead];
    bool active[kAhead];
    float2 dl[kAhead];
    float sg[kAhead], cr[kAhead], cg[kAhead], cb[kAhead];
#pragma unroll
    for (int j = 0; j < kAhead; ++j) {
      active[j] = k + j < cnt;
      field[j] = (unsigned)(__ballot(active[j]) >> g0) & 0xFFFFu;
      slot[j] = (int64_t)S + __popc(field[j] & ((1u << rr) - 1u));
      S += __popc(field[j]);
      const int64_t i = (active[j] && !done) ? slot[j] : 0;
      dl[j] = reinterpret_cast<const float2*>(deltas)[i];
      sg[j] = sigmas[i];
      cr[j] = rgbs[i * 3]; cg[j] = rgbs[i * 3 + 1]; cb[j] = rgbs[i * 3 + 2];
    }
#pragma unroll
    for (int j = 0; j < kAhead; ++j) {
      if (skippable) {
        const unsigned live = (unsigned)(__ballot(active[j] && !done) >> g0) & 0xFFFFu;
        if (rr == 0 && field[j] != 0 && live == 0) n_skip += __popc(field[j]);
      }
      if (active[j] && !done) {
        const float alpha = 1.0f - expf(-sg[j] * dl[j].x);
        const float w = alpha * T;
        r += w * cr[j]; g += w * cg[j]; b += w * cb[j];
        t += dl[j].y;
        dsum += w * t;
        ws += w;
        if (wbuf) wbuf[slot[j]] = w;
        T *= 1.0f - alpha;
        if (T < T_thresh) done = true;
      } else if (active[j] && wbuf) {
        wbuf[slot[j]] = 0.0f;
      }
    }
  }
  if (n < N) {
    weights_sum[rid] = ws; depth[rid] = dsum;
    image[rid * 3] = r; image[rid * 3 + 1] = g; image[rid * 3 + 2] = b;
  }
  if (skippable) {
#pragma unroll
    for (int d = 1; d < 64; d <<= 1) n_skip += __shfl_xor(n_skip, d, 64);
    if (lane == 0 && n_skip) atomicAdd(skippable, (unsigned long long)n_skip);
  }
}

__global__ void __launch_bounds__(kRayBlock) k_composite_patch_extra(const float* __restrict__ wbuf,
                                                                     const float* __restrict__ extra,
                                                                     const int32_t* __restrict__ rays, int64_t N,
                                                                     int64_t M, int K, float* __restrict__ extra_out) {
  const int64_t n = ((int64_t)blockIdx.x * blockDim.x + threadIdx.x) >> 6;
  const int lane = threadIdx.x & 63;
  if (n >= N) return;
  const int64_t g0 = n & ~(int64_t)(kGroup - 1);
  const int r = (int)(n - g0);
  int c[kGroup];
  int total = 0;
#pragma unroll
  for (int i = 0; i < kGroup; ++i) {
    c[i] = (g0 + i < N) ? rays[(g0 + i) * 3 + 2] : 0;
    total += c[i];
  }
  const int32_t rid = rays[n * 3];
  int64_t S = rays[g0 * 3 + 1];
  const int cnt = (S + total <= M) ? c[r] : 0;
  float acc = 0.0f;
  for (int k = 0; k < cnt; ++k) {
    int nact = 0, rank = 0;
#pragma unroll
    for (int i = 0; i < kGroup; ++i) {
      const int gt = c[i] > k ? 1 : 0;
      nact += gt;
      rank += (i < r) ? gt : 0;
    }
    const int64_t slot = S + rank;
    S += nact;
    const float w = wbuf[slot];
    if (lane < K && w != 0.0f) acc += w * extra[slot * K + lane];
  }
  if (lane < K) extra_out[(int64_t)rid * K + lane] = acc;
}

struct MaskVolume {
  float lo[3], hi[3], res[3];
  int W, L, H;
};
__global__ void __launch_bounds__(kRayBlock) k_project_masks_patch(const float* __restrict__ xyzs,
                                                                   const float* __restrict__ wbuf,
                                                                   const int32_t* __restrict__ rays, int64_t N, int64_t M,
                                                                   const uint32_t* __restrict__ words, MaskVolume V,
                                                                   int k_total, int k_base, int k_count,
                                                                   float* __restrict__ out) {
  const int64_t n = (int64_t)blockIdx.x * blockDim.x + threadIdx.x;
  const int lane = threadIdx.x & 63, g0 = lane & ~(kGroup - 1), rr = lane & (kGroup - 1);
  const int32_t rid = n < N ? rays[n * 3] : 0;
  const int off = n < N ? rays[n * 3 + 1] : 0;
  int cnt = n < N ? rays[n * 3 + 2] : 0;
  int S = __shfl(off, g0, 64);
  int gtot = cnt;
#pragma unroll
  for (int d = 1; d < kGroup; d <<= 1) gtot += __shfl_xor(gtot, d, 64);
  if ((int64_t)S + gtot > M) cnt = 0;
  int maxc = cnt;
#pragma unroll
// ... 259 lines not shown
  return (b + 15) / 16 * 16;
}
int inr_march_write_fills_unowned_rows(int64_t N, int32_t sample_cap, int32_t max_steps) {
  return use_stage(N, sample_cap, max_steps) ? 1 : 0;
}
int64_t inr_march_workspace_bytes(int64_t N, int32_t sample_cap) {
  const int64_t base = stage_offset_bytes(N, sample_cap);
  return base + (N <= kStageMaxRays && sample_cap == 0 ? N * (int64_t)kStagePitch * 5 * (int64_t)sizeof(float) : 0);
}

static size_t march_lds_pad() { return (size_t)inr::g_march_lds_pad; }

int inr_march_rays_train_count(const float* rays_o, const float* rays_d, const uint8_t* bitfield, float bound,
                               float dt_gamma, int32_t max_steps, int64_t N, int32_t cascade, int32_t H,
                               const float* nears, const float* fars, const float* noises, int32_t* rays,
                               int32_t* counter, void* workspace, int32_t sample_cap, inr_stream_t s) {
  INR_REQUIRE(rays_o && rays_d && bitfield && nears && fars && rays && counter && workspace, "null pointer");
  INR_REQUIRE(N > 0 && N < (1ll << 31), "N out of range");
  INR_REQUIRE(max_steps > 0 && cascade >= 1 && H >= 8 && H <= 1024, "bad grid parameters");
  const MarchParams P = make_params(bitfield, bound, dt_gamma, max_steps, cascade, H);
  const unsigned nb = blocks_for(N, kRayBlock);
  INR_REQUIRE(sample_cap >= 0 && ((uintptr_t)workspace & 7) == 0, "workspace must be 8-byte aligned");
  int32_t* counts = reinterpret_cast<int32_t*>(workspace);
  int32_t* block_sums = counts + N;
  uint32_t* mask = reinterpret_cast<uint32_t*>(counts + ws_ints(N));
  hipStream_t st = as_stream(s);
  if (use_coop(N, sample_cap)) {
    float* stage = use_stage(N, sample_cap, max_steps)
                       ? reinterpret_cast<float*>(reinterpret_cast<char*>(workspace) + stage_offset_bytes(N, sample_cap)) : nullptr;
    k_march_count_coop<<<blocks_for(N, kCoopRaysPerBlock), kCoopRaysPerBlock * 64, 0, st>>>(P, rays_o, rays_d, N, max_steps,
                                                                                          nears, fars, noises, counts, stage,
                                                                                          kStagePitch);
    k_scan_counts<<<1, 1024, 0, st>>>(counts, N, rays, counter);
    return check_launch("march_rays_train_count");
  }
  k_march_count<<<nb, kRayBlock, march_lds_pad(), st>>>(P, rays_o, rays_d, N, max_steps, nears, fars, noises, counts, block_sums,
                                          mask, cap_words_of(sample_cap));
  k_scan_block_sums<<<1, 1024, 0, st>>>(block_sums, (int)nb, N, counter);
  k_finalize_offsets<<<nb, kRayBlock, 0, st>>>(counts, block_sums, N, rays);
  return check_launch("march_rays_train_count");
}

int inr_march_rays_train_write(const float* rays_o, const float* rays_d, const uint8_t* bitfield, float bound,
                               float dt_gamma, int32_t max_steps, int64_t N, int32_t cascade, int32_t H, int64_t M,
                               const float* nears, const float* fars, const float* noises, const int32_t* rays,
                               float* xyzs, float* dirs, float* deltas, const void* workspace, int32_t sample_cap,
                               inr_stream_t s) {
  INR_REQUIRE(rays_o && rays_d && bitfield && nears && fars && rays, "null pointer");
  INR_REQUIRE(N > 0 && M >= 0, "bad sizes");
  if (M == 0) return INR_OK;
  INR_REQUIRE(M == 0 || (xyzs && dirs && deltas), "null output");
  const MarchParams P = make_params(bitfield, bound, dt_gamma, max_steps, cascade, H);
  INR_REQUIRE(sample_cap == 0 || workspace, "sample_cap > 0 needs the workspace of the count pass");
  const uint32_t* mask = sample_cap > 0 ? reinterpret_cast<const uint32_t*>(reinterpret_cast<const int32_t*>(workspace) + ws_ints(N)) : nullptr;
  if (use_stage(N, sample_cap, max_steps)) {
    INR_REQUIRE(workspace, "the staged marcher needs the workspace of the count pass");
    const float* stage = reinterpret_cast<const float*>(reinterpret_cast<const char*>(workspace) + stage_offset_bytes(N, sample_cap));
    k_march_write_staged<<<blocks_for(N, kCoopRaysPerBlock), kCoopRaysPerBlock * 64, 0, as_stream(s)>>>(
        rays_d, N, M, rays, stage, kStagePitch, xyzs, dirs, deltas);
    return check_launch("march_rays_train_write");
  }
  if (use_coop(N, sample_cap)) {
    k_march_write_coop<<<blocks_for(N, kCoopRaysPerBlock), kCoopRaysPerBlock * 64, 0, as_stream(s)>>>(
        P, rays_o, rays_d, N, M, nears, fars, noises, rays, xyzs, dirs, deltas);
    return check_launch("march_rays_train_write");
  }
  k_march_write<<<blocks_for(N, kRayBlock), kRayBlock, 0, as_stream(s)>>>(P, rays_o, rays_d, N, M, nears, fars, noises,
                                                                          rays, xyzs, dirs, deltas, mask, cap_words_of(sample_cap));
  return check_launch("march_rays_train_write");
}

int inr_march_rays_patch_write(const float* rays_o, const float* rays_d, const uint8_t* bitfield, float bound,
                               float dt_gamma, int32_t max_steps, int64_t N, int32_t cascade, int32_t H, int64_t M,
                               const float* nears, const float* fars, const float* noises, const int32_t* rays,
                               float* xyzs, float* dirs, float* deltas, const void* workspace, int32_t sample_cap,
                               int32_t* ray_ids, int32_t normalise, inr_stream_t s) {
  INR_REQUIRE(rays_o && rays_d && bitfield && nears && fars && rays, "null pointer");
  INR_REQUIRE(N > 0 && M >= 0, "bad sizes");
  if (M == 0) return INR_OK;
  INR_REQUIRE(M == 0 || (xyzs && deltas && (dirs || ray_ids)), "null output");
  const MarchParams P = make_params(bitfield, bound, dt_gamma, max_steps, cascade, H);
  INR_REQUIRE(sample_cap == 0 || workspace, "sample_cap > 0 needs the workspace of the count pass");
  const uint32_t* mask = sample_cap > 0 ? reinterpret_cast<const uint32_t*>(reinterpret_cast<const int32_t*>(workspace) + ws_ints(N)) : nullptr;
  k_march_write_patch<<<blocks_for(N, kRayBlock), kRayBlock, march_lds_pad(), as_stream(s)>>>(P, rays_o, rays_d, N, M, nears, fars,
                                                                                noises, rays, xyzs, dirs, deltas, mask,
                                                                                cap_words_of(sample_cap), ray_ids, normalise);
  return check_launch("march_rays_patch_write");
}

int inr_composite_rays_patch_forward(const float* sigmas, const float* rgbs, const float* deltas, const int32_t* rays,
                                     int64_t N, int64_t M, float T_thresh, const float* extra, int32_t K,
                                     float* weights_sum, float* depth, float* image, float* extra_out,
                                     float* weights, uint64_t* skippable, inr_stream_t s) {
  INR_REQUIRE(N >= 0 && M >= 0, "bad sizes");
  if (N == 0) return INR_OK;
  INR_REQUIRE(rays && weights_sum && depth && image, "null pointer");
  INR_REQUIRE(M == 0 || (sigmas && rgbs && deltas), "null sample arrays");
  INR_REQUIRE(!extra || (extra_out && weights && K > 0 && K <= 64), "extra needs extra_out, weights and 0 < K <= 64");
  INR_REQUIRE(((uintptr_t)deltas & 7) == 0, "deltas must be 8-byte aligned");
  hipStream_t st = as_stream(s);
  k_composite_patch_fwd<<<blocks_for(N, kRayBlock), kRayBlock, 0, st>>>(sigmas, rgbs, deltas, rays, N, M, T_thresh,
                                                                        weights, weights_sum, depth, image,
                                                                        reinterpret_cast<unsigned long long*>(skippable));
  if (extra_out && K > 0)
    k_composite_patch_extra<<<blocks_for(N * 64, kRayBlock), kRayBlock, 0, st>>>(weights, extra, rays, N, M, K,
                                                                                 extra_out);
  return check_launch("composite_rays_patch_forward");
}

int inr_project_masks_patch(const float* xyzs, const float* weights, const int32_t* rays, int64_t N, int64_t M,
                            const uint32_t* mask_words, int32_t W, int32_t L, int32_t H, const float* bbox ,
                            int32_t k_total, int32_t k_base, int32_t k_count, float* out, inr_stream_t s) {
  INR_REQUIRE(N >= 0 && M >= 0 && W > 0 && L > 0 && H > 0, "bad sizes");
  INR_REQUIRE(k_total > 0 && k_base >= 0 && k_count > 0 && k_count <= 32 && k_base + k_count <= k_total, "bad mask range");
  if (N == 0) return INR_OK;
  INR_REQUIRE(rays && mask_words && bbox && out, "null pointer");
  INR_REQUIRE(M == 0 || (xyzs && weights), "null sample arrays");
  MaskVolume V;
  for (int a = 0; a < 3; ++a) { V.lo[a] = bbox[a]; V.hi[a] = bbox[3 + a]; }
  V.res[0] = (float)W; V.res[1] = (float)L; V.res[2] = (float)H;
  V.W = W; V.L = L; V.H = H;
  k_project_masks_patch<<<blocks_for(N, kRayBlock), kRayBlock, 0, as_stream(s)>>>(xyzs, weights, rays, N, M, mask_words, V,
                                                                                 k_total, k_base, k_count, out);
  return check_launch("project_masks_patch");
}

int inr_march_rays(int64_t n_alive, int32_t n_step, const int32_t* rays_alive, const float* rays_t,
                   const float* rays_o, const float* rays_d, float bound, float dt_gamma, int32_t max_steps,
                   int32_t cascade, int32_t H, const uint8_t* bitfield, const float* nears, const float* fars,
                   float* xyzs, float* dirs, float* deltas, inr_stream_t s) {
  (void)nears;
  INR_REQUIRE(rays_alive && rays_t && rays_o && rays_d && bitfield && fars && xyzs && dirs && deltas, "null pointer");
  INR_REQUIRE(n_alive >= 0 && n_step > 0, "bad sizes");
  if (n_alive == 0) return INR_OK;
  const MarchParams P = make_params(bitfield, bound, dt_gamma, max_steps, cascade, H);
  k_march_rays<<<blocks_for(n_alive, kRayBlock), kRayBlock, 0, as_stream(s)>>>(P, n_alive, n_step, rays_alive, rays_t,
                                                                               rays_o, rays_d, fars, xyzs, dirs, deltas);
  return check_launch("march_rays");
}

int inr_composite_rays(int64_t n_alive, int32_t n_step, int32_t* rays_alive, float* rays_t, const float* sigmas,
                       const float* rgbs, const float* deltas, float* weights_sum, float* depth, float* image,
                       float T_thresh, const float* extra, float* extra_acc, int32_t K, inr_stream_t s) {
  INR_REQUIRE(rays_alive && rays_t && sigmas && rgbs && deltas && weights_sum && depth && image, "null pointer");
  INR_REQUIRE(!extra || (extra_acc && K > 0), "extra given without extra_acc/K");
  if (n_alive == 0) return INR_OK;
  k_composite_rays<<<blocks_for(n_alive, kRayBlock), kRayBlock, 0, as_stream(s)>>>(
      n_alive, n_step, rays_alive, rays_t, sigmas, rgbs, deltas, weights_sum, depth, image, T_thresh, extra, extra_acc, K);
  return check_launch("composite_rays");
}

int inr_compact_alive(const int32_t* rays_alive, int64_t n_alive, int32_t* out, int32_t* n_out, inr_stream_t s) {
  INR_REQUIRE(rays_alive && out && n_out && n_alive >= 0, "bad argument");
  if (n_alive == 0) {
    (void)hipMemsetAsync(n_out, 0, 2 * sizeof(int32_t), as_stream(s));
    return check_launch("compact_alive");
  }
  const unsigned nb = blocks_for(n_alive, kRayBlock);
  int32_t* counts = out + n_alive;
  int32_t* block_sums = counts + n_alive;
  hipStream_t st = as_stream(s);
  k_alive_flags<<<nb, kRayBlock, 0, st>>>(rays_alive, n_alive, counts, block_sums);
  k_scan_block_sums<<<1, 1024, 0, st>>>(block_sums, (int)nb, n_alive, n_out);
  k_alive_scatter<<<nb, kRayBlock, 0, st>>>(rays_alive, n_alive, block_sums, out);
  return check_launch("compact_alive");
}

int inr_cross_entropy(const float* logits, const int64_t* labels, int64_t N, int32_t K, int64_t ignore_index,
                      float* grad_logits, float* acc, float* loss, inr_stream_t s) {
  INR_REQUIRE(N >= 0 && K > 0 && K <= 64, "K must be in 1..64");
  INR_REQUIRE(acc && loss && ((uintptr_t)acc & 7) == 0, "null or misaligned pointer");
  hipStream_t st = as_stream(s);
  int nb = 0;
  if (N > 0) {
    INR_REQUIRE(logits && labels && grad_logits, "null pointer");
    nb = (int)std::min<int64_t>((N + 3) / 4, kCeBlocks);
    k_ce_rows<<<nb, 256, 0, st>>>(logits, labels, N, K, ignore_index, grad_logits, reinterpret_cast<float2*>(acc));
  }
  const unsigned nb2 = (unsigned)std::max<int64_t>(1, std::min<int64_t>((N * K + 255) / 256, (int64_t)cu_count() * 4));
  k_ce_scale<<<nb2, 256, 0, st>>>(grad_logits, N * K, reinterpret_cast<const float2*>(acc), nb, loss);
  return check_launch("cross_entropy");
}

int inr_finish_rays(const float* image, const float* depth, const float* weights_sum, const float* nears,
                    const float* fars, const float* t0, float bg_r, float bg_g, float bg_b, int64_t N, float* image_out,
                    float* depth_out, inr_stream_t s) {
  INR_REQUIRE(N >= 0, "negative N");
  if (N == 0) return INR_OK;
  INR_REQUIRE(image && depth && weights_sum && nears && fars && image_out && depth_out, "null pointer");
  k_finish_rays<<<blocks_for(N, 256), 256, 0, as_stream(s)>>>(image, depth, weights_sum, nears, fars, t0, bg_r, bg_g, bg_b,
// ... 79 lines not shown
```

### instance_nerf_amd/nerf/network.py

```python
import os

import torch
import torch.nn as nn
import torch.nn.functional as F

from .. import _lib
from .._lib import check, host_ptr, ptr, stream_ptr
from ..activation import trunc_exp
from ..encoding import get_encoder
from .renderer import NeRFRenderer

_O_NUMERICS = _lib.NUMERICS_TABLE_F16 | _lib.NUMERICS_MLP_F16


class _LinearFn(torch.autograd.Function):

    @staticmethod
    def forward(ctx, x, w):
        ctx.save_for_backward(x, w)
        return F.linear(x, w)

    @staticmethod
    def backward(ctx, gy):
        x, w = ctx.saved_tensors
        gx = gw = None
        if ctx.needs_input_grad[0]:
            gx = gy @ w
        if ctx.needs_input_grad[1]:
            lib = _lib.load()
            gyc, xc = gy.contiguous(), x.contiguous()
            gw = torch.zeros_like(w)
            ws = torch.empty(lib.inr_linear_wgrad_workspace_bytes() // 4, dtype=torch.float32, device=w.device)
            check(lib.inr_linear_wgrad(ptr(xc, torch.float32, "x"), ptr(gyc, torch.float32, "grad_y"), xc.shape[0],
                                       w.shape[1], w.shape[0], ptr(gw), ptr(ws), stream_ptr()), "linear_wgrad")
        return gx, gw


_before_scatter = {}


def _fx_env():
    v = os.environ.get("INR_FX_GRAD", "0")
    return {"0": 0, "": 0, "1": 32, "32": 32, "64": 64}.get(v, 0)


FX_GRAD = _fx_env()
FX_HEADROOM = float(os.environ.get("INR_FX_HEADROOM", "128"))
FX_HEADROOM64 = float(os.environ.get("INR_FX_HEADROOM64", "1024"))


def fx_bits():
    return 64 if FX_GRAD == 64 else (32 if FX_GRAD else 0)


def fx_acc64(emb, create=True):
    acc = getattr(emb, "_fx_acc64", None)
    if (acc is None or acc.device != emb.device or acc.shape != emb.shape) and create and emb.is_cuda:
        acc = torch.zeros(emb.shape, dtype=torch.int64, device=emb.device)
        emb._fx_acc64 = acc
    return acc


def fx_state(emb, create=True):
    st = getattr(emb, "_fx_state", None)
    if (st is None or st.device != emb.device) and create and emb.is_cuda:
        st = torch.zeros(_lib.GRID_FX_STATE_FLOATS, dtype=torch.float32, device=emb.device)
        emb._fx_state = st
        emb._fx_primed = 0
    return st


def _table_backward(lib, x, denc, desc, M, bound, g_emb, emb):
    from .utils import grad_sync
    L = int(desc.num_levels)
    hook = _before_scatter.pop("hook", None)
    if hook is not None:
        hook()
    if grad_sync.active() and emb.data_ptr() in grad_sync.early:
        raise RuntimeError("gradient accumulation over several backward passes is not supported together with the "
                           "overlapped table-gradient all-reduce; set INR_GRAD_OVERLAP=0")
    overlap = grad_sync.active() and L > 8 and emb.grad is None
    bits = fx_bits() if (g_emb.is_cuda and g_emb.data_ptr() % 16 == 0) else 0
# ... 285 lines not shown
        if (x.is_cuda and x.dim() == 2 and x.dtype == torch.float32 and self.in_features <= 64
                and self.out_features <= 64 and torch.is_grad_enabled() and self.weight.requires_grad):
            return _LinearFn.apply(x, self.weight)
        return F.linear(x, self.weight)


def _mlp(in_dim, hidden, out_dim, num_layers):
    layers = []
    for l in range(num_layers):
        layers.append(HipLinear(in_dim if l == 0 else hidden, out_dim if l == num_layers - 1 else hidden, bias=False))
    return nn.ModuleList(layers)


def _run_mlp(net, h):
    for l, layer in enumerate(net):
        h = layer(h)
        if l != len(net) - 1:
            h = F.relu(h, inplace=True)
    return h


class NeRFNetwork(NeRFRenderer):
    _warned_unfused = False

    def __init__(self, encoding="hashgrid", encoding_dir="sphere_harmonics", encoding_bg="hashgrid", num_layers=2,
                 hidden_dim=64, geo_feat_dim=15, num_layers_color=3, hidden_dim_color=64, num_layers_bg=2,
                 hidden_dim_bg=64, bound=1, num_instances=0, num_layers_instance=3, hidden_dim_instance=64,
                 encoder_kwargs=None, **kwargs):
        super().__init__(bound, **kwargs)
        self.num_layers, self.hidden_dim, self.geo_feat_dim = num_layers, hidden_dim, geo_feat_dim
        enc_kw = dict(desired_resolution=2048 * bound)
        enc_kw.update(encoder_kwargs or {})
        self.encoder, self.in_dim = get_encoder(encoding, **enc_kw)
        self.sigma_net = _mlp(self.in_dim, hidden_dim, 1 + geo_feat_dim, num_layers)
        self.num_layers_color, self.hidden_dim_color = num_layers_color, hidden_dim_color
        self.encoder_dir, self.in_dim_dir = get_encoder(encoding_dir)
        self.color_net = _mlp(self.in_dim_dir + geo_feat_dim, hidden_dim_color, 3, num_layers_color)
        self.num_instances = int(num_instances)
        in_dim_inst = 0
        if self.num_instances:
            self.instance_encoder, in_dim_inst = get_encoder(encoding, **enc_kw)
            self.instance_net = _mlp(in_dim_inst, hidden_dim_instance, self.num_instances, num_layers_instance)
        for enc in (self.encoder, getattr(self, "instance_encoder", None)):
            desc = getattr(enc, "desc", None)
            if desc is not None and int(desc.num_levels) > 8:
                enc.embeddings._inr_split_row = int(desc.offsets[8])
        self._fusable = (encoding == "hashgrid" and encoding_dir == "sphere_harmonics" and num_layers == 2
                         and hidden_dim == 64 and geo_feat_dim == 15 and num_layers_color == 3
                         and hidden_dim_color == 64 and self.in_dim == 32)
        self._k_pad = 16 * ((self.num_instances + 15) // 16)
        self._fusable_inst = (0 < self.num_instances <= 64 and num_layers_instance == 3
                              and hidden_dim_instance == 64 and encoding == "hashgrid" and in_dim_inst == 32)
        why = []
        if not self._fusable:
            why.append("NeRF field: " + ", ".join(
                f"{n}={v!r} (fused: {w!r})" for n, v, w in (
                    ("encoding", encoding, "hashgrid"), ("encoding_dir", encoding_dir, "sphere_harmonics"),
                    ("num_layers", num_layers, 2), ("hidden_dim", hidden_dim, 64), ("geo_feat_dim", geo_feat_dim, 15),
                    ("num_layers_color", num_layers_color, 3), ("hidden_dim_color", hidden_dim_color, 64),
                    ("encoder output (levels x features)", self.in_dim, 32)) if v != w))
        if self.num_instances and not self._fusable_inst:
            why.append("instance field: " + ", ".join(
                f"{n}={v!r} (fused: {w})" for n, v, w in (
                    ("num_instances", self.num_instances, "<= 64"), ("num_layers_instance", num_layers_instance, 3),
                    ("hidden_dim_instance", hidden_dim_instance, 64), ("encoder output", in_dim_inst, 32))
                if not (v <= 64 if w == "<= 64" else v == w)))
        self.unfused_reason = "; ".join(why) or None
        if self.unfused_reason and not NeRFNetwork._warned_unfused:
            NeRFNetwork._warned_unfused = True
            import warnings
            warnings.warn("NeRFNetwork: this shape leaves the fused HIP field kernels and runs on the composable path "
                          "(HIP hash-grid / SH encoders + BLAS MLP layers; slower, not the benchmarked path) - "
                          + self.unfused_reason, RuntimeWarning, stacklevel=2)
        self._packed = {}
        self.fused_instance_train = True
        self.fused_nerf_train = True
        self.fused_nerf_head = True
        self.half_table = False
        self._half_cache = {}
        self.mlp_fp16 = False
        self.frame_slices = __import__("os").environ.get("INR_FRAME_SLICES", "auto")
        self._slice_probe = None
        self.last_frame_path = "fused"

    def _packed_weights(self, which, numerics=0):
        lib = _lib.load()
        mlp_f16 = numerics & _lib.NUMERICS_MLP_F16
        if which == "nerf":
            ws = [self.sigma_net[0].weight, self.sigma_net[1].weight, self.color_net[0].weight,
                  self.color_net[1].weight, self.color_net[2].weight]
        else:
            ws = [l.weight for l in self.instance_net]
        key = tuple((w.data_ptr(), w._version) for w in ws)
        hit = self._packed.get((which, mlp_f16))
        if hit is not None and hit[0] == key:
            return hit[1]
        if not mlp_f16 and ws[0].is_cuda and not getattr(self, "_host_pack_only", False):
            f32 = torch.float32
            dev_ws = [w.detach().float().contiguous() for w in ws]
            try:
                if which == "nerf":
                    pf = torch.empty(lib.inr_nerf_packed_floats(), dtype=f32, device=ws[0].device)
                    pb = torch.empty(lib.inr_nerf_bwd_packed_floats(), dtype=f32, device=ws[0].device)
                    check(lib.inr_nerf_pack_weights_device(*[ptr(w, f32, "weight") for w in dev_ws], ptr(pf), ptr(pb),
                                                           stream_ptr()), "nerf_pack_weights_device")
                else:
                    if self._k_pad != self.num_instances:
                        dev_ws[2] = torch.nn.functional.pad(dev_ws[2], (0, 0, 0, self._k_pad - self.num_instances)).contiguous()
                    pf = torch.empty(lib.inr_instance_packed_floats(self._k_pad), dtype=f32, device=ws[0].device)
                    pb = torch.empty(lib.inr_instance_bwd_packed_floats(), dtype=f32, device=ws[0].device)
                    check(lib.inr_instance_pack_weights_device(*[ptr(w, f32, "weight") for w in dev_ws], self._k_pad,
                                                               ptr(pf), ptr(pb), stream_ptr()), "instance_pack_weights_device")
                self._packed[(which, mlp_f16)] = (key, pf)
                return pf
            except RuntimeError:
                self._host_pack_only = True
        host = [w.detach().float().cpu().contiguous() for w in ws]
        if which == "instance" and self._k_pad != self.num_instances:
            host[2] = torch.nn.functional.pad(host[2], (0, 0, 0, self._k_pad - self.num_instances)).contiguous()
        if which == "nerf":
            buf = torch.empty(lib.inr_nerf_packed_floats(), dtype=torch.float32)
            check(lib.inr_nerf_pack_weights(*[host_ptr(h, torch.float32) for h in host], host_ptr(buf, torch.float32),
                                            mlp_f16), "nerf_pack_weights")
        else:
            buf = torch.empty(lib.inr_instance_packed_floats(self._k_pad), dtype=torch.float32)
            check(lib.inr_instance_pack_weights(*[host_ptr(h, torch.float32) for h in host], self._k_pad,
                                                host_ptr(buf, torch.float32), mlp_f16), "instance_pack_weights")
        dev = buf.to(ws[0].device)
        self._packed[(which, mlp_f16)] = (key, dev)
        return dev

    def _table_ptr(self, encoder, numerics=0):
        emb = encoder.embeddings
        if not numerics & _lib.NUMERICS_TABLE_F16:
            return ptr(emb.data, torch.float32, "embeddings")
        key = (emb.data_ptr(), emb._version)
        hit = self._half_cache.get(id(encoder))
        if hit is None or hit[0] != key:
            hit = self._half_cache[id(encoder)] = (key, emb.detach().to(torch.float16).contiguous())
        return ptr(hit[1], torch.float16, "embeddings")

    def _needs_grad(self, params):
        return torch.is_grad_enabled() and any(p.requires_grad for p in params)

    def _nerf_params(self):
        return [self.encoder.embeddings] + [l.weight for l in self.sigma_net] + [l.weight for l in self.color_net]

    def _fused_nerf(self, x, d, want_rgb, want_geo, out=None):
        lib = _lib.load()
        x = x.contiguous().float()
        M = x.shape[0]
        dev = x.device
        if out is not None:
            sigma, rgb = out
        else:
            sigma = torch.empty(M, dtype=torch.float32, device=dev)
            rgb = torch.empty(M, 3, dtype=torch.float32, device=dev) if want_rgb else None
        geo = torch.empty(M, self.geo_feat_dim, dtype=torch.float32, device=dev) if want_geo else None
        if want_rgb:
            d = d.contiguous().float()
        numerics = 0
        if (want_rgb and not want_geo and self.half_table and self.mlp_fp16
                and (not self.training or not self.encoder.embeddings.requires_grad)):
            numerics = _O_NUMERICS
        check(lib.inr_nerf_forward(ptr(x, torch.float32, "x"), ptr(d, torch.float32, "d", allow_none=not want_rgb),
                                   M, None, float(self.bound), self._table_ptr(self.encoder, numerics),
# ... 1 lines not shown
                                   ptr(rgb, allow_none=True), ptr(geo, allow_none=True), numerics, stream_ptr()),
              "nerf_forward")
        return sigma, rgb, geo

    _SLICE_PROBE_ORDER = (False, True, True, False, False, True)

    def _use_slices(self, M):
        mode = self.frame_slices
        self.last_frame_path = "fused"
        if mode in (False, 0, "0", "off", "False"):
            return False
        tb = self.encoder.table
        if not (M > 0 and int(tb["num_levels"]) == 16 and bool(tb["hashed"][8:].all())):
            return False
        if mode in (True, 1, "1", "on", "True"):
            self.last_frame_path = "sliced"
            return True
        if M < (1 << 21):
            return False
        if int(tb["resolutions"][-1]) < 8192:
            return False
        p = self._slice_probe
        if p is not None and p["choice"] is not None:
            mc = int(getattr(self, "mean_count", 0) or 0)
            if (getattr(self, "iter_density", 0) != p["iter_density"] and p["mean_count"] > 0 and mc > 0
                    and abs(mc - p["mean_count"]) > 0.1 * p["mean_count"]):
                p = self._slice_probe = None
        if p is None:
            p = self._slice_probe = {"calls": 0, "pending": [], "ms": {False: [], True: []}, "choice": None,
                                     "iter_density": 0, "mean_count": 0, "decisions": getattr(self, "_slice_decisions", 0)}
        if p["choice"] is not None:
            self.last_frame_path = "sliced" if p["choice"] else "fused"
            return p["choice"]
        for rec in list(p["pending"]):
            if rec[1].query():
                p["ms"][rec[2]].append(rec[0].elapsed_time(rec[1]) / max(rec[3], 1))
                p["pending"].remove(rec)
        if len(p["ms"][False]) >= 3 and len(p["ms"][True]) >= 3:
            med = {k: sorted(v)[len(v) // 2] for k, v in p["ms"].items()}
            p["choice"] = med[True] < 0.97 * med[False]
            p["iter_density"] = getattr(self, "iter_density", 0)
            p["mean_count"] = int(getattr(self, "mean_count", 0) or 0)
            self._slice_decisions = p["decisions"] + 1
            self.last_frame_path = "sliced" if p["choice"] else "fused"
            return p["choice"]
        if p["calls"] >= len(self._SLICE_PROBE_ORDER) + 6:
            return False
        use = self._SLICE_PROBE_ORDER[p["calls"] % len(self._SLICE_PROBE_ORDER)]
        p["calls"] += 1
        p["armed"] = (use, M)
        self.last_frame_path = ("sliced" if use else "fused") + " (probing)"
        return use

    def _open_slice_probe(self):
        p = self._slice_probe
        if p and p.get("armed") is not None:
            use, M = p.pop("armed")
            e0 = torch.cuda.Event(enable_timing=True)
            e0.record()
            p["open"] = (e0, use, M)

    def _close_slice_probe(self):
        p = self._slice_probe
        if p and p.get("open") is not None:
            e0, use, M = p.pop("open")
            e1 = torch.cuda.Event(enable_timing=True)
            e1.record()
            p["pending"].append((e0, e1, use, M))

    def load_state_dict(self, state_dict, *args, **kwargs):
        out = super().load_state_dict(state_dict, *args, **kwargs)
        self._slice_probe = None
        return out

    @torch.no_grad()
    def sh_table(self, rays_d):
        lib = _lib.load()
        rays_d = rays_d.contiguous().float().view(-1, 3)
        shq = torch.empty(rays_d.shape[0], 16, dtype=torch.float32, device=rays_d.device)
        check(lib.inr_sh_table_q(ptr(rays_d, torch.float32, "rays_d"), rays_d.shape[0], ptr(shq), stream_ptr()),
              "sh_table_q")
        return shq

    def forward_table(self, x01, ray_ids, rays_d, shq=None):
        if not self._fusable:
            return None
        lib = _lib.load()
        M = x01.shape[0]
        dev = x01.device
        if shq is None:
            shq = self.sh_table(rays_d)
        sigma = torch.empty(M, dtype=torch.float32, device=dev)
        rgb = torch.empty(M, 3, dtype=torch.float32, device=dev)
        numerics = 0
        if not self.training:
            numerics = ((_lib.NUMERICS_TABLE_F16 if self.half_table else 0)
                        | (_lib.NUMERICS_MLP_F16 if self.mlp_fp16 else 0))
        if not numerics and self._use_slices(M):
            need = lib.inr_nerf_forward_table_sliced_workspace_bytes(M) // 4
            ws = self.__dict__.get("_slice_ws")
            if ws is None or ws.numel() < need or ws.device != dev:
                ws = self.__dict__["_slice_ws"] = torch.empty(int(need * 1.25), dtype=torch.float32, device=dev)
            ws.record_stream(torch.cuda.current_stream())
            self._open_slice_probe()
            check(lib.inr_nerf_forward_table_sliced(ptr(x01, torch.float32, "x01"), ptr(ray_ids, torch.int32, "ray_ids"),
                                                    ptr(shq), M, float(self.bound),
                                                    ptr(self.encoder.embeddings.data, torch.float32), self.encoder.desc,
                                                    ptr(self._packed_weights("nerf")), 1.0, ptr(sigma), ptr(rgb), ptr(ws),
                                                    stream_ptr()), "nerf_forward_table_sliced")
            self._close_slice_probe()
            return sigma, rgb
        self._open_slice_probe()
        check(lib.inr_nerf_forward_table(ptr(x01, torch.float32, "x01", allow_none=M == 0),
                                         ptr(ray_ids, torch.int32, "ray_ids", allow_none=M == 0), ptr(shq), M,
                                         float(self.bound), self._table_ptr(self.encoder, numerics),
                                         self.encoder.desc, ptr(self._packed_weights("nerf", numerics)), 1.0,
                                         ptr(sigma, allow_none=M == 0), ptr(rgb, allow_none=M == 0), numerics,
                                         stream_ptr()), "nerf_forward_table")
        self._close_slice_probe()
        return sigma, rgb

    @torch.no_grad()
    def forward_dirs(self, x, dirs):
        if not self._fusable:
            return None
        lib = _lib.load()
        x = x.contiguous().float()
        M, D = x.shape[0], dirs.shape[0]
        sh = self.encoder_dir(dirs.to(x.device).contiguous().float()).contiguous()
        out = torch.empty(M, 4, dtype=torch.float32, device=x.device)
        check(lib.inr_nerf_forward_dirs(ptr(x, torch.float32, "x", allow_none=M == 0), M, float(self.bound),
                                        ptr(self.encoder.embeddings.data, torch.float32), self.encoder.desc,
                                        ptr(self._packed_weights("nerf")), ptr(sh, torch.float32, "sh_dirs"), D,
                                        ptr(out, allow_none=M == 0), stream_ptr()), "nerf_forward_dirs")
        return out

    def _lattice_args(self, axes):
        ax = [a.contiguous().float() for a in axes]
        W, L, H = (int(a.shape[0]) for a in ax)
        if W * L * H == 0:
            return (W, L, H), ax, None
        return (W, L, H), ax, (ptr(ax[0], torch.float32, "ax_w"), ptr(ax[1], torch.float32, "ax_l"),
                               ptr(ax[2], torch.float32, "ax_h"), W, L, H, float(self.bound),
                               ptr(self.encoder.embeddings.data, torch.float32), self.encoder.desc,
                               ptr(self._packed_weights("nerf")))

    @torch.no_grad()
    def forward_lattice(self, axes, dirs, logit_min=float("-inf"), sh=None):
        if not self._fusable:
            return None
        lib = _lib.load()
        shape, ax, head = self._lattice_args(axes)
        if sh is None:
            sh = self.encoder_dir(dirs.to(ax[0].device).contiguous().float()).contiguous()
        out = torch.empty(*shape, 4, dtype=torch.float32, device=ax[0].device)
        if head is not None:
            check(lib.inr_nerf_forward_lattice(*head, ptr(sh, torch.float32, "sh_dirs"), dirs.shape[0], float(logit_min),
                                               ptr(out), stream_ptr()), "nerf_forward_lattice")
        return out

    @torch.no_grad()
    def instance_lattice(self, axes, sigma_thresh, want_logit=False):
        if not (self._fusable and self.num_instances and self._fusable_inst):
            return None
        lib = _lib.load()
        shape, ax, head = self._lattice_args(axes)
        dev = ax[0].device
        labels = torch.empty(shape, dtype=torch.uint8, device=dev)
        conf = torch.empty(shape, dtype=torch.float32, device=dev)
        logit = torch.empty(shape, dtype=torch.float32, device=dev) if want_logit else None
        if head is not None:
            check(lib.inr_instance_lattice(*head, float(self.density_scale), float(sigma_thresh),
                                           ptr(self.instance_encoder.embeddings.data, torch.float32),
                                           self.instance_encoder.desc, ptr(self._packed_weights("instance")),
                                           self.num_instances, ptr(labels, torch.uint8), ptr(conf),
                                           ptr(logit, allow_none=True), stream_ptr()), "instance_lattice")
        return (labels, conf, logit) if want_logit else (labels, conf)

    def forward(self, x, d):
        if self._fusable and not self._needs_grad(self._nerf_params()):
            sigma, rgb, _ = self._fused_nerf(x, d, True, False)
# ... 143 lines not shown
```

### instance_nerf_amd/nerf/renderer.py

```python
import math
import os

import torch
import torch.nn as nn

from .. import _lib, raymarching
from .._lib import check, ptr, stream_ptr


def sample_pdf(bins, weights, n_samples, det=False):
    weights = weights + 1e-5
    pdf = weights / torch.sum(weights, -1, keepdim=True)
    cdf = torch.cat([torch.zeros_like(pdf[..., :1]), torch.cumsum(pdf, -1)], -1)
    if det:
        u = torch.linspace(0.5 / n_samples, 1 - 0.5 / n_samples, steps=n_samples, device=weights.device)
        u = u.expand(list(cdf.shape[:-1]) + [n_samples])
    else:
        u = torch.rand(list(cdf.shape[:-1]) + [n_samples], device=weights.device)
    u = u.contiguous()
    inds = torch.searchsorted(cdf, u, right=True)
    below = torch.max(torch.zeros_like(inds - 1), inds - 1)
    above = torch.min((cdf.shape[-1] - 1) * torch.ones_like(inds), inds)
    cdf_g = torch.stack([torch.gather(cdf, 1, below), torch.gather(cdf, 1, above)], -1)
    bins_g = torch.stack([torch.gather(bins, 1, below), torch.gather(bins, 1, above)], -1)
# ... 192 lines not shown
        return self.instance(x)

    def run_cuda(self, rays_o, rays_d, dt_gamma=0, bg_color=None, perturb=False, force_all_rays=False,
                 max_steps=1024, T_thresh=1e-4, infer_mode="auto", noises=None, field_gate=None, ce_labels=None,
                 ce_ignore_index=-1, mse_target=None, marched=None, ce_prune=False, **kwargs):
        prefix = rays_o.shape[:-1]
        rays_o = rays_o.contiguous().view(-1, 3).float()
        rays_d = rays_d.contiguous().view(-1, 3).float()
        N = rays_o.shape[0]
        aabb = self.aabb_train if self.training else self.aabb_infer
        if marched is not None and not marched.fits(self.training, N, self.iter_density):
            self.drop_ahead(marched)
            marched = None
        if marched is not None:
            marched.wait()
            nears, fars = marched.nears, marched.fars
        elif self.training and ce_prune and ce_labels is not None:
            nears, fars = raymarching.near_far_from_aabb(rays_o, rays_d, aabb, self.min_near, skip_labels=ce_labels,
                                                         ignore_index=ce_ignore_index)
        else:
            nears, fars = raymarching.near_far_from_aabb(rays_o, rays_d, aabb, self.min_near)
        if not self.training and infer_mode == "auto":
            infer_mode = "fused_terminate" if self._recent_skippable() > self.terminate_above else "fused"
        gate = _NO_GATE if field_gate is None else field_gate
        jitter = noises if perturb else None
        all_fused = self._fusable and (self._fusable_inst or self.num_instances == 0)
        results = {}
        if self.training or infer_mode == "fused_raymajor":
            weights_sum, depth, image = self._render_ray_major(
                results, prefix, rays_o, rays_d, nears, fars, marched, dt_gamma, max_steps, perturb, noises,
                force_all_rays, T_thresh, ce_labels, ce_ignore_index)
        elif infer_mode == "fused_terminate" and all_fused:
            weights_sum, depth, image = self._render_terminating(
                results, prefix, rays_o, rays_d, nears, fars, dt_gamma, max_steps, jitter, T_thresh, gate)
        elif infer_mode in ("fused", "fused_terminate"):
            weights_sum, depth, image = self._render_two_kernel(
                results, prefix, rays_o, rays_d, nears, fars, dt_gamma, max_steps, jitter, T_thresh, gate, all_fused)
        elif infer_mode == "wavefront":
            weights_sum, depth, image = self._render_wavefront(
                results, prefix, rays_o, rays_d, nears, fars, dt_gamma, max_steps, perturb, T_thresh)
        else:
            raise ValueError(f"unknown infer_mode {infer_mode!r}")
        one_pass = not self.training and infer_mode != "wavefront"
        return self._finish_rays(results, prefix, weights_sum, depth, image, nears, fars,
                                 1 if bg_color is None else bg_color, mse_target, one_pass, jitter, dt_gamma, max_steps)

    def _take_counter_slot(self):
        index = self.local_step % 16
        self.local_step += 1
        return index, self.step_counter[index]

    def _composite_with_logits(self, composite, results, prefix, xyzs, *args, **kwargs):
        with_instance = self.num_instances > 0
        extra = self._instance_for_compositing(xyzs) if with_instance else None
        out = composite(*args, extra=extra, **kwargs)
        if with_instance:
            results["instance"] = out[3][:, :self.num_instances].reshape(*prefix, -1)
        return out[0], out[1], out[2]

    def _render_terminating(self, results, prefix, rays_o, rays_d, nears, fars, dt_gamma, max_steps, jitter, T_thresh, gate):
        with_instance = self.num_instances > 0
        counter = torch.zeros(2, dtype=torch.int32, device=rays_o.device)
        xyzs, _, deltas, rays = raymarching.march_rays_patch(
            rays_o, rays_d, self.bound, self.density_bitfield, self.cascade, self.grid_size, nears, fars,
            dt_gamma, max_steps, noises=jitter, counter=counter, table=True)
        gate.acquire()
        weights_sum, depth, image, wbuf, evaluated = self.nerf_render(xyzs, deltas, rays, rays_d, T_thresh,
                                                                      want_weights=with_instance, normalised=True)
        gate.release()
        if with_instance:
            gate.acquire()
            results["instance"] = self.instance_render(xyzs, rays, wbuf, normalised=True).view(*prefix, -1)
            gate.release()
        results["num_samples"] = counter
        results["num_evaluated"] = evaluated
        self._note_skippable(evaluated, int(xyzs.shape[0]), True)
        return weights_sum, depth, image

    def _render_two_kernel(self, results, prefix, rays_o, rays_d, nears, fars, dt_gamma, max_steps, jitter, T_thresh, gate,
                           table):
        device = rays_o.device
        fused_inst = self.num_instances > 0 and self._fusable_inst
        counter = torch.zeros(2, dtype=torch.int32, device=device)
        early = {}

        def while_waiting():
            early["skippable"] = torch.zeros(1, dtype=torch.int64, device=device)
            if table:
                early["shq"] = self.sh_table(rays_d)
        xyzs, dirs, deltas, rays = raymarching.march_rays_patch(
            rays_o, rays_d, self.bound, self.density_bitfield, self.cascade, self.grid_size, nears, fars,
            dt_gamma, max_steps, noises=jitter, counter=counter, table=table, while_waiting=while_waiting)
        gate.acquire()
        sigmas, rgbs = self.forward_table(xyzs, dirs, rays_d, shq=early.get("shq")) if table else self(xyzs, dirs)
        gate.release()
        if self.density_scale != 1:
            sigmas = self.density_scale * sigmas
        skippable = early["skippable"]
        if fused_inst:
            weights_sum, depth, image, wbuf = raymarching.composite_rays_patch(sigmas, rgbs, deltas, rays, T_thresh,
                                                                              return_weights=True, skippable=skippable)
            gate.acquire()
            results["instance"] = self.instance_render(xyzs, rays, wbuf, normalised=table).view(*prefix, -1)
            gate.release()
        else:
            weights_sum, depth, image = self._composite_with_logits(
                raymarching.composite_rays_patch, results, prefix, xyzs, sigmas, rgbs, deltas, rays, T_thresh,
                skippable=skippable)
        results["num_samples"] = counter
        if table:
            results["frame_path"] = self.last_frame_path
        self._note_skippable(skippable, int(xyzs.shape[0]), False)
        return weights_sum, depth, image

    def _render_ray_major(self, results, prefix, rays_o, rays_d, nears, fars, marched, dt_gamma, max_steps, perturb, noises,
                          force_all_rays, T_thresh, ce_labels, ce_ignore_index):
        with_instance = self.num_instances > 0
        if marched is not None:
            counter = marched.counter
            xyzs, dirs, deltas, rays = marched.xyzs, marched.dirs, marched.deltas, marched.rays
        else:
            if self.training:
                _, counter = self._take_counter_slot()
                mean_count = self.mean_count
            else:
                counter = torch.zeros(2, dtype=torch.int32, device=rays_o.device)
                mean_count = -1
                force_all_rays = True
            xyzs, dirs, deltas, rays = raymarching.march_rays_train(
                rays_o, rays_d, self.bound, self.density_bitfield, self.cascade, self.grid_size, nears, fars,
                counter, mean_count, perturb, 128, force_all_rays, dt_gamma, max_steps, noises=noises)
        if self.training:
            self.last_counter = counter
        head = with_instance and self.instance_head_available(xyzs)
        shaded = marched.shaded_for(T_thresh, self.density_scale) if marched is not None else None
        if shaded is not None and not (head and self.shade_ahead_applies()):
            shaded = None
        if shaded is None:
            sigmas, rgbs = self(xyzs, dirs)
            if self.density_scale != 1:
                sigmas = self.density_scale * sigmas
        if head:
            weights_sum, depth, image, wbuf, sample_ray = shaded if shaded is not None else raymarching.composite_rays_train(
                sigmas, rgbs, deltas, rays, T_thresh, return_weights=True, total_dev=counter)
            if ce_labels is not None:
                inst, results["instance_ce"] = self.instance_head_train(
                    xyzs, wbuf, sample_ray, rays, n_dev=counter, ce_labels=ce_labels.reshape(-1),
                    ce_ignore_index=ce_ignore_index)
            else:
                inst = self.instance_head_train(xyzs, wbuf, sample_ray, rays, n_dev=counter)
            results["instance"] = inst[:, :self.num_instances].reshape(*prefix, -1)
        else:
            weights_sum, depth, image = self._composite_with_logits(
                raymarching.composite_rays_train, results, prefix, xyzs, sigmas, rgbs, deltas, rays, T_thresh,
                total_dev=counter)
        results["num_samples"] = counter
        return weights_sum, depth, image

    def _render_wavefront(self, results, prefix, rays_o, rays_d, nears, fars, dt_gamma, max_steps, perturb, T_thresh):
        N, device = rays_o.shape[0], rays_o.device
        with_instance = self.num_instances > 0
        dtype = torch.float32
        weights_sum = torch.zeros(N, dtype=dtype, device=device)
        depth = torch.zeros(N, dtype=dtype, device=device)
        image = torch.zeros(N, 3, dtype=dtype, device=device)
        inst = torch.zeros(N, self.num_instances, dtype=dtype, device=device) if with_instance else None
        n_alive = N
        rays_alive = torch.arange(n_alive, dtype=torch.int32, device=device)
        rays_t = nears.clone()
        step = 0
        while step < max_steps and n_alive > 0:
            n_step = max(min(N // n_alive, 8), 1)
            xyzs, dirs, deltas = raymarching.march_rays(n_alive, n_step, rays_alive, rays_t, rays_o, rays_d,
                                                        self.bound, self.density_bitfield, self.cascade,
                                                        self.grid_size, nears, fars, 128, perturb, dt_gamma,
                                                        max_steps)
            sigmas, rgbs = self(xyzs, dirs)
            sigmas = self.density_scale * sigmas
            extra = self.instance(xyzs) if with_instance else None
            raymarching.composite_rays(n_alive, n_step, rays_alive, rays_t, sigmas, rgbs, deltas, weights_sum,
                                       depth, image, T_thresh, extra=extra, extra_acc=inst)
            rays_alive, n_alive = raymarching.compact_alive(rays_alive, n_alive)
            step += n_step
        if with_instance:
            results["instance"] = inst.view(*prefix, -1)
        return weights_sum, depth, image

    def _finish_rays(self, results, prefix, weights_sum, depth, image, nears, fars, bg_color, mse_target, one_pass, jitter,
                     dt_gamma, max_steps):
        N = weights_sum.shape[0]
        t_start = None
        if one_pass:
            t_start = nears
            if jitter is not None:
# ... 288 lines not shown
```

### instance_nerf_amd/raymarching.py

```python
import math

import torch

from . import _lib
from ._lib import check, ptr, stream_ptr

F32, I32, U8 = torch.float32, torch.int32, torch.uint8

SAMPLE_CAP = int(__import__("os").environ.get("INR_SAMPLE_CAP", "1024"))
SAMPLE_CAP_TRAIN = int(__import__("os").environ.get("INR_SAMPLE_CAP_TRAIN", "0"))


def _f(t):
    return t.contiguous().float() if (t.dtype != F32 or not t.is_contiguous()) else t


def set_overlap_placement(on):
    check(_lib.load().inr_set_overlap_placement(1 if on else 0), "set_overlap_placement")


def set_march_mode(mode):
    code = {None: -1, "auto": -1, "lane_per_ray": 0, "wave_per_ray": 1}[mode]
    check(_lib.load().inr_set_march_mode(code), "set_march_mode")

# ... 63 lines not shown
                           stream_ptr()), "packbits")
    return bitfield


def sample_capacity(mean_count):
    return (int(mean_count) + 127) // 128 * 128


def march_train_buffers(n_rays, n_samples, device, shade=False):
    lib = _lib.load()
    b = {"n_rays": n_rays, "n_samples": n_samples,
         "nears": torch.empty(n_rays, dtype=F32, device=device), "fars": torch.empty(n_rays, dtype=F32, device=device),
         "noises": torch.empty(n_rays, dtype=F32, device=device), "rays": torch.empty(n_rays, 3, dtype=I32, device=device),
         "ws": torch.empty(lib.inr_march_workspace_bytes(n_rays, SAMPLE_CAP_TRAIN) // 8 + 1, dtype=torch.int64, device=device),
         "buf": torch.empty(n_samples * 8, dtype=F32, device=device)}
    if shade:
        b.update({"sigmas": torch.empty(n_samples, dtype=F32, device=device),
                  "rgbs": torch.empty(n_samples, 3, dtype=F32, device=device),
                  "weights_sum": torch.empty(n_rays, dtype=F32, device=device),
                  "depth": torch.empty(n_rays, dtype=F32, device=device),
                  "image": torch.empty(n_rays, 3, dtype=F32, device=device),
                  "weights": torch.empty(n_samples, dtype=F32, device=device),
                  "sample_ray": torch.empty(n_samples, dtype=I32, device=device)})
    return b


def march_rays_train(rays_o, rays_d, bound, density_bitfield, C, H, nears, fars, step_counter=None,
                     mean_count=-1, perturb=False, align=-1, force_all_rays=False, dt_gamma=0, max_steps=1024,
                     noises=None, separate_buffers=False, out=None):
    lib = _lib.load()
    rays_o, rays_d = _f(rays_o).view(-1, 3), _f(rays_d).view(-1, 3)
    dev = rays_o.device
    N = rays_o.shape[0]
    nears, fars = _f(nears), _f(fars)
    if noises is None:
        if not perturb:
            noises = None
        elif out is not None:
            noises = torch.rand(N, dtype=F32, device=dev, out=out["noises"])
        else:
            noises = torch.rand(N, dtype=F32, device=dev)
    else:
        noises = _f(noises)
    if step_counter is None:
        step_counter = torch.zeros(2, dtype=I32, device=dev)
    cap = SAMPLE_CAP_TRAIN
    if out is not None:
        if force_all_rays or mean_count <= 0 or out["n_rays"] != N or out["n_samples"] < int(mean_count):
            raise RuntimeError("march_rays_train(out=) needs the steady state and buffers of the batch's size")
        rays, ws = out["rays"], out["ws"]
    else:
        rays = torch.empty(N, 3, dtype=I32, device=dev)
        ws = torch.empty(lib.inr_march_workspace_bytes(N, cap) // 8 + 1, dtype=torch.int64, device=dev)
    args = (ptr(rays_o, F32, "rays_o"), ptr(rays_d, F32, "rays_d"), ptr(density_bitfield, U8, "density_bitfield"),
            float(bound), float(dt_gamma), int(max_steps), N, int(C), int(H))
    check(lib.inr_march_rays_train_count(*args, ptr(nears, F32, "nears"), ptr(fars, F32, "fars"),
                                         ptr(noises, F32, "noises", allow_none=True), ptr(rays),
                                         ptr(step_counter, I32, "step_counter"), ptr(ws), cap, stream_ptr()),
          "march_rays_train_count")
    if force_all_rays or mean_count <= 0:
        M = int(step_counter[0].item())
    else:
        M = int(mean_count)
    if align > 0:
        M += align - M % align if M % align else 0
    alloc = torch.empty if lib.inr_march_write_fills_unowned_rows(N, cap, int(max_steps)) else torch.zeros
    if out is not None:
        if alloc is not torch.empty or M > out["n_samples"]:
            raise RuntimeError("march_rays_train(out=) needs the staged marcher (it clears unowned rows itself)")
        buf = out["buf"]
        xyzs, dirs, deltas = buf[:M * 3].view(M, 3), buf[M * 3:M * 6].view(M, 3), buf[M * 6:M * 8].view(M, 2)
    elif separate_buffers:
        xyzs, dirs, deltas = (alloc(M, 3, dtype=F32, device=dev), alloc(M, 3, dtype=F32, device=dev),
                              alloc(M, 2, dtype=F32, device=dev))
    else:
        buf = alloc(M * 8, dtype=F32, device=dev)
        xyzs, dirs, deltas = buf[:M * 3].view(M, 3), buf[M * 3:M * 6].view(M, 3), buf[M * 6:].view(M, 2)
    check(lib.inr_march_rays_train_write(*args, M, ptr(nears), ptr(fars), ptr(noises, F32, "noises", allow_none=True),
                                         ptr(rays), ptr(xyzs), ptr(dirs), ptr(deltas), ptr(ws), cap, stream_ptr()),
          "march_rays_train_write")
    return xyzs, dirs, deltas, rays


GROUP = 16


_PINNED_COUNT = {}


def _read_count(counter, while_waiting=None):
    key = counter.device.index
    host = _PINNED_COUNT.get(key)
    if host is None:
        host = _PINNED_COUNT[key] = torch.empty(2, dtype=I32, pin_memory=True)
    host.copy_(counter[:2], non_blocking=True)
    ev = torch.cuda.Event()
    ev.record()
    if while_waiting is not None:
        while_waiting()
    ev.synchronize()
    return int(host[0])


def march_rays_patch(rays_o, rays_d, bound, density_bitfield, C, H, nears, fars, dt_gamma=0, max_steps=1024,
                     noises=None, counter=None, table=False, while_waiting=None):
    lib = _lib.load()
    rays_o, rays_d = _f(rays_o).view(-1, 3), _f(rays_d).view(-1, 3)
    dev = rays_o.device
    N = rays_o.shape[0]
    nears, fars = _f(nears), _f(fars)
    noises = _f(noises) if noises is not None else None
    if counter is None:
        counter = torch.zeros(2, dtype=I32, device=dev)
    rays = torch.empty(N, 3, dtype=I32, device=dev)
    cap = SAMPLE_CAP
    ws = torch.empty(lib.inr_march_workspace_bytes(N, cap) // 8 + 1, dtype=torch.int64, device=dev)
    args = (ptr(rays_o, F32, "rays_o"), ptr(rays_d, F32, "rays_d"), ptr(density_bitfield, U8, "density_bitfield"),
            float(bound), float(dt_gamma), int(max_steps), N, int(C), int(H))
    check(lib.inr_march_rays_train_count(*args, ptr(nears, F32, "nears"), ptr(fars, F32, "fars"),
                                         ptr(noises, F32, "noises", allow_none=True), ptr(rays),
                                         ptr(counter, I32, "counter"), ptr(ws), cap, stream_ptr()),
          "march_rays_train_count")
    M = _read_count(counter, while_waiting)
    xyzs = torch.empty(M, 3, dtype=F32, device=dev)
    dirs = None if table else torch.empty(M, 3, dtype=F32, device=dev)
    ray_ids = torch.empty(M, dtype=I32, device=dev) if table else None
    deltas = torch.empty(M, 2, dtype=F32, device=dev)
    check(lib.inr_march_rays_patch_write(*args, M, ptr(nears), ptr(fars), ptr(noises, F32, "noises", allow_none=True),
                                         ptr(rays), ptr(xyzs, allow_none=M == 0), ptr(dirs, allow_none=True),
                                         ptr(deltas, allow_none=M == 0), ptr(ws), cap,
                                         ptr(ray_ids, allow_none=True), 1 if table else 0, stream_ptr()),
          "march_rays_patch_write")
    return xyzs, (ray_ids if table else dirs), deltas, rays


def composite_rays_patch(sigmas, rgbs, deltas, rays, T_thresh=1e-4, extra=None, return_weights=False, skippable=None):
    lib = _lib.load()
    sigmas, rgbs, deltas = _f(sigmas), _f(rgbs), _f(deltas)
    dev = rays.device
    N, M = rays.shape[0], sigmas.shape[0]
    K = 0 if extra is None else extra.shape[1]
    ws = torch.empty(N, dtype=F32, device=dev)
    depth = torch.empty(N, dtype=F32, device=dev)
    image = torch.empty(N, 3, dtype=F32, device=dev)
    extra_out = torch.empty(N, K, dtype=F32, device=dev) if K else None
    wbuf = torch.empty(max(M, 1), dtype=F32, device=dev) if (K or return_weights) else None
    none_ok = M == 0
    check(lib.inr_composite_rays_patch_forward(
        ptr(sigmas, F32, "sigmas", allow_none=none_ok), ptr(rgbs, F32, "rgbs", allow_none=none_ok),
        ptr(deltas, F32, "deltas", allow_none=none_ok), ptr(rays, I32, "rays"), N, M, float(T_thresh),
        ptr(_f(extra) if extra is not None else None, allow_none=True), K, ptr(ws), ptr(depth), ptr(image),
        ptr(extra_out, allow_none=True), ptr(wbuf, allow_none=True), ptr(skippable, torch.int64, "skippable", allow_none=True),
        stream_ptr()), "composite_rays_patch_forward")
    out = (ws, depth, image) + ((extra_out,) if K else ())
    return out + ((wbuf,) if return_weights else ())


def patch_slots(rays):
    r = rays.cpu().long()
    N = r.shape[0]
    cnt, off = r[:, 2], r[:, 1]
    pad = (-N) % GROUP
    c = torch.cat([cnt, torch.zeros(pad, dtype=torch.long)]).view(-1, GROUP)
    base = torch.cat([off, torch.zeros(pad, dtype=torch.long)]).view(-1, GROUP)[:, 0]
    out = []
    for g in range(c.shape[0]):
        cg = c[g]
        kmax = int(cg.max())
        if kmax == 0:
            continue
        k = torch.arange(kmax)[:, None]
        act = cg[None, :] > k
        nact = act.sum(1)
        S = base[g] + torch.cat([torch.zeros(1, dtype=torch.long), nact.cumsum(0)[:-1]])
        rank = act.long().cumsum(1) - act.long()
        slot = S[:, None] + rank
        for i in range(GROUP):
            out.append(slot[: int(cg[i]), i])
    return torch.cat(out) if out else torch.zeros(0, dtype=torch.long)


class _CompositeRaysTrain(torch.autograd.Function):
    @staticmethod
    def forward(ctx, sigmas, rgbs, extra, deltas, rays, T_thresh, want_weights=False, total_dev=None):
        lib = _lib.load()
        sigmas, rgbs, deltas = _f(sigmas), _f(rgbs), _f(deltas)
        dev = sigmas.device
        N = rays.shape[0]
        K = 0 if extra is None else extra.shape[1]
        if extra is not None:
            extra = _f(extra)
        ws = torch.empty(N, dtype=F32, device=dev)
        depth = torch.empty(N, dtype=F32, device=dev)
        image = torch.empty(N, 3, dtype=F32, device=dev)
        extra_out = torch.empty(N, K, dtype=F32, device=dev) if K else None
        wbuf = torch.empty(sigmas.shape[0], dtype=F32, device=dev) if (K or want_weights) else None
        sample_ray = torch.empty(sigmas.shape[0], dtype=I32, device=dev) if want_weights else None
        check(lib.inr_composite_rays_train_forward(
            ptr(sigmas, F32, "sigmas"), ptr(rgbs, F32, "rgbs"), ptr(deltas, F32, "deltas"), ptr(rays, I32, "rays"),
            N, sigmas.shape[0], float(T_thresh), ptr(extra, F32, "extra", allow_none=True), K, ptr(ws), ptr(depth),
            ptr(image),
            ptr(extra_out, allow_none=True), ptr(wbuf, allow_none=True), ptr(sample_ray, allow_none=True), stream_ptr()),
            "composite_rays_train_forward")
        ctx.save_for_backward(sigmas, rgbs, extra, deltas, rays, ws, image, wbuf, total_dev)
        ctx.T_thresh = T_thresh
        ctx.K = K
        ctx.set_materialize_grads(False)
        if ctx.needs_input_grad[0] or ctx.needs_input_grad[1]:
            ctx.mark_non_differentiable(depth)
        else:
            ctx.mark_non_differentiable(depth, ws, image)
        out = (ws, depth, image) + ((extra_out,) if K else ())
        if want_weights:
            ctx.mark_non_differentiable(wbuf, sample_ray)
            out = out + (wbuf, sample_ray)
        ctx.n_out = len(out)
        return out

    @staticmethod
    def backward(ctx, g_ws, g_depth, g_image, *rest):
        g_extra = rest[0] if ctx.K else None
        lib = _lib.load()
        sigmas, rgbs, extra, deltas, rays, ws, image, wbuf, total_dev = ctx.saved_tensors
        N = rays.shape[0]
        K = ctx.K
        dev = sigmas.device
        need_field = ctx.needs_input_grad[0] or ctx.needs_input_grad[1]
        gs = gc = None
        if need_field:
            g_ws = _f(g_ws) if g_ws is not None else None
# ... 183 lines not shown
```

Before: 6540 Msamples/s.

## Add compact per-sample records feed (t + ray id) for inference ray marching

Inference marching can now write only a scalar t and a ray id per sample instead of xyz, ray id and two deltas. The field kernel rebuilds positions from a per-ray table holding SH coefficients, origin and direction, and compositing recomputes deltas from t, nears and the step rule. This cuts per-sample write and read traffic between march, field and composite. The cost is recomputation in the consumers, a power-of-two bound requirement, and a shared sample_pos helper that keeps positions bit-consistent.

```diff
diff --git a/include/inr.h b/include/inr.h
--- a/include/inr.h
+++ b/include/inr.h
@@ -103,6 +103,21 @@
                                      float* extra_out , float* weights ,
                                      uint64_t* skippable ,
                                      inr_stream_t s);
+int inr_march_rays_patch_write_records(const float* rays_o, const float* rays_d, const uint8_t* bitfield,
+                                       float bound, float dt_gamma, int32_t max_steps, int64_t N,
+                                       int32_t cascade, int32_t H, int64_t M, const float* nears,
+                                       const float* fars, const float* noises ,
+                                       const int32_t* rays ,
+                                       float* t , int32_t* ray_ids , const void* workspace,
+                                       int32_t sample_cap, inr_stream_t s);
+int inr_composite_rays_patch_forward_records(const float* sigmas, const float* rgbs, const float* t ,
+                                             const int32_t* rays, int64_t N, int64_t M, float T_thresh,
+                                             const float* nears , const float* noises ,
+                                             float dt_gamma, int32_t max_steps, int32_t cascade, int32_t H,
+                                             const float* extra , int32_t K,
+                                             float* weights_sum, float* depth, float* image,
+                                             float* extra_out , float* weights ,
+                                             uint64_t* skippable , inr_stream_t s);
 int inr_project_masks_patch(const float* xyzs, const float* weights, const int32_t* rays, int64_t N, int64_t M,
                             const uint32_t* mask_words, int32_t W, int32_t L, int32_t H, const float* bbox ,
                             int32_t k_total, int32_t k_base, int32_t k_count, float* out, inr_stream_t s);
@@ -191,6 +206,12 @@
                            float bound, const void* embeddings, const inr_grid_desc* desc ,
                            const float* packed , float density_scale, float* sigma, float* rgb,
                            int32_t numerics, inr_stream_t s);
+#define INR_RAY_TABLE_FLOATS 24
+int inr_ray_table_q(const float* rays_o , const float* rays_d , int64_t N, float* out, inr_stream_t s);
+int inr_nerf_forward_table_records(const float* t, const int32_t* ray_ids, const float* ray_table_q, int64_t M,
+                             float bound, const void* embeddings, const inr_grid_desc* desc ,
+                             const float* packed , float density_scale, float* sigma, float* rgb,
+                             int32_t numerics, inr_stream_t s);
 int64_t inr_nerf_forward_table_sliced_workspace_bytes(int64_t M);
 int inr_nerf_forward_table_sliced(const float* x01, const int32_t* ray_ids, const float* sh_table_q, int64_t M,
                                   float bound, const float* embeddings, const inr_grid_desc* desc ,
diff --git a/instance_nerf_amd/_lib.py b/instance_nerf_amd/_lib.py
--- a/instance_nerf_amd/_lib.py
+++ b/instance_nerf_amd/_lib.py
@@ -10,6 +10,7 @@
 GRID_FX_STATE_FLOATS = 4192
 ROI_MAX_LEVELS = 8
 NUMERICS_TABLE_F16, NUMERICS_MLP_F16 = 1, 2
+RAY_TABLE_FLOATS = 24
 
 
 class GridDesc(Structure):
@@ -76,6 +77,12 @@
     "inr_nerf_forward_table_sliced_workspace_bytes": (c_int64, [c_int64]),
     "inr_nerf_forward_table_sliced": (c_int32, [P, P, P, c_int64, c_float, P, POINTER(GridDesc), P, c_float, P, P, P, P]),
     "inr_composite_rays_patch_forward": (c_int32, [P, P, P, P, c_int64, c_int64, c_float, P, c_int32, P, P, P, P, P, P, P]),
+    "inr_march_rays_patch_write_records": (c_int32, [P, P, P, c_float, c_float, c_int32, c_int64, c_int32, c_int32,
+                                                     c_int64, P, P, P, P, P, P, P, c_int32, P]),
+    "inr_composite_rays_patch_forward_records": (c_int32, [P, P, P, P, c_int64, c_int64, c_float, P, P, c_float, c_int32,
+                                                           c_int32, c_int32, P, c_int32, P, P, P, P, P, P, P]),
+    "inr_ray_table_q": (c_int32, [P, P, c_int64, P, P]),
+    "inr_nerf_forward_table_records": (c_int32, [P, P, P, c_int64, c_float, P, POINTER(GridDesc), P, c_float, P, P, c_int32, P]),
     "inr_project_masks_patch": (c_int32, [P, P, P, c_int64, c_int64, P, c_int32, c_int32, c_int32, P, c_int32, c_int32, c_int32,
                                           P, P]),
     "inr_march_rays": (c_int32, [c_int64, c_int32, P, P, P, P, c_float, c_float, c_int32, c_int32, c_int32,
diff --git a/instance_nerf_amd/build.py b/instance_nerf_amd/build.py
--- a/instance_nerf_amd/build.py
+++ b/instance_nerf_amd/build.py
@@ -8,13 +8,13 @@
 LIB = os.path.join(CSRC, "libinr_hip.so")
 SOURCES = ["raymarch.hip", "encoders.hip", "field_fused.hip", "roialign.hip", "mesh.hip", "components.hip", "match.hip",
            "overlap.hip", "detect.hip"]
-HEADERS = ["common.h", "grid_common.h", os.path.join("..", "..", "include", "inr.h")]
+HEADERS = ["common.h", "grid_common.h", "sample_pos.h", os.path.join("..", "..", "include", "inr.h")]
 FLAGS = ["--offload-arch=gfx950", "-O3", "-std=c++17", "-fPIC", "-ffp-contract=off",
          "-munsafe-fp-atomics", "-Wall", "-Wno-unused-function"]
 
 
 KERNEL_FILES = {
-    "field": ["field_fused.hip", "common.h", "grid_common.h"],
+    "field": ["field_fused.hip", "common.h", "grid_common.h", "sample_pos.h"],
     "scatter": ["encoders.hip", "common.h", "grid_common.h"],
 }
 
diff --git a/instance_nerf_amd/csrc/field_fused.hip b/instance_nerf_amd/csrc/field_fused.hip
--- a/instance_nerf_amd/csrc/field_fused.hip
+++ b/instance_nerf_amd/csrc/field_fused.hip
@@ -4,6 +4,7 @@
 
 #include "common.h"
 #include "grid_common.h"
+#include "sample_pos.h"
 
 namespace inr {
 
@@ -639,7 +640,9 @@
   float *enc, *h1, *so, *cin, *c1, *c2;
 };
 
-template <bool kColor, bool kTable = false, int kSave = 0, bool kHalf = false, bool kFast = false, bool kPre = false>
+constexpr int kRayRowVec = INR_RAY_TABLE_FLOATS / 4;
+template <bool kColor, bool kTable = false, int kSave = 0, bool kHalf = false, bool kFast = false, bool kPre = false,
+          bool kRec = false>
 __global__ void __launch_bounds__(kFieldThreads, kFieldMinWaves) k_nerf_fwd(const float* __restrict__ x, const float* __restrict__ d,
                                                                int64_t M, const int32_t* __restrict__ n_dev, float bound,
                                                                const float2* __restrict__ emb, uint32_t emb_bytes, GridDesc G,
@@ -677,7 +680,18 @@
     const bool valid = m < n;
     TileIn me;
     f32x4 sh_in = {0.f, 0.f, 0.f, 0.f};
-    if constexpr (kTable) {
+    if constexpr (kRec) {
+      static_assert(!kRec || (kTable && !kPre), "the records feed is a variant of the fused table feed");
+      const int64_t mm = valid ? m : n - 1;
+      const float t = x[mm];
+      const float4* row = shq + (int64_t)ray_ids[mm] * kRayRowVec;
+      const float4 t4 = row[q], o4 = row[4], d4 = row[5];
+      sh_in = f32x4{t4.x, t4.y, t4.z, t4.w};
+      const float rb_rcp = 1.0f / rb;
+      me.x0 = sample_x01_pow2(sample_pos(o4.x, t, d4.x, bound), bound, rb_rcp);
+      me.x1 = sample_x01_pow2(sample_pos(o4.y, t, d4.y, bound), bound, rb_rcp);
+      me.x2 = sample_x01_pow2(sample_pos(o4.z, t, d4.z, bound), bound, rb_rcp);
+    } else if constexpr (kTable) {
       const int64_t mm = valid ? m : n - 1;
       me.x0 = x[mm * 3 + 0]; me.x1 = x[mm * 3 + 1]; me.x2 = x[mm * 3 + 2];
       const float4 t4 = shq[(int64_t)ray_ids[mm] * 4 + q];
@@ -2367,6 +2381,43 @@
   else pack_section(dst, W, n_out, n_in, n_mt, n_ks, kidx);
 }
 
+template <bool kRec>
+static int forward_table_launch(const char* what, const float* x, const int32_t* ray_ids, const float* table, int64_t M,
+                                float bound, const void* embeddings, const inr_grid_desc* desc, const float* packed,
+                                float density_scale, float* sigma, float* rgb, int32_t numerics, inr_stream_t s) {
+  FieldTable t;
+  if (int rc = field_table(what, desc, embeddings, numerics & INR_NUMERICS_TABLE_F16, t)) return rc;
+  if (int rc = check_numerics(what, numerics, kAcceptAny)) return rc;
+  const size_t lds = std::max(kNerfFloats * sizeof(float) + kLevelRecBytes, (size_t)g_field_lds_min);
+  const int64_t n_tiles = (M + 15) / 16;
+  const hipStream_t st = as_stream(s);
+  HybridSchedule hybrid;
+  if (!hybrid.begin(st, n_tiles)) return INR_ELAUNCH;
+  with_flag(numerics & INR_NUMERICS_TABLE_F16, [&](auto half) {
+    with_mlp_f16(numerics & INR_NUMERICS_MLP_F16, [&](auto fast) {
+      launch_field(k_nerf_fwd<true, true, 0, decltype(half)::value, decltype(fast)::value, false, kRec>, lds, n_tiles, st,
+                   x, nullptr, M, nullptr, bound, t.emb, t.bytes, t.G, f4(packed), density_scale, sigma, rgb, nullptr,
+                   ray_ids, f4(table), NerfSave{}, hybrid.cursors());
+    });
+  });
+  hybrid.finish(st);
+  return check_launch(what + 4);
+}
+
+__global__ void __launch_bounds__(256) k_ray_table_q(const float* __restrict__ o, const float* __restrict__ d, int64_t N,
+                                                     float4* __restrict__ out) {
+  const int64_t n = (int64_t)blockIdx.x * blockDim.x + threadIdx.x;
+  if (n >= N) return;
+  const float dx = d[n * 3], dy = d[n * 3 + 1], dz = d[n * 3 + 2];
+  float v[16];
+  sh4(dx, dy, dz, v);
+  float4* row = out + n * kRayRowVec;
+#pragma unroll
+  for (int q = 0; q < 4; ++q) row[q] = make_float4(v[q], v[4 + q], v[8 + q], v[12 + q]);
+  row[4] = make_float4(o[n * 3], o[n * 3 + 1], o[n * 3 + 2], 0.0f);
+  row[5] = make_float4(dx, dy, dz, 0.0f);
+}
+
 }
 
 using namespace inr;
@@ -2442,23 +2493,30 @@
   INR_REQUIRE(x01 && ray_ids && sh_table_q && embeddings && packed && sigma && rgb, "null pointer");
   INR_REQUIRE(((uintptr_t)embeddings & 7) == 0 && ((uintptr_t)packed & 15) == 0 && ((uintptr_t)sh_table_q & 15) == 0,
               "embeddings/packed/sh_table_q misaligned");
-  FieldTable t;
-  if (int rc = field_table(__func__, desc, embeddings, numerics & INR_NUMERICS_TABLE_F16, t)) return rc;
-  if (int rc = check_numerics(__func__, numerics, kAcceptAny)) return rc;
-  const size_t lds = std::max(kNerfFloats * sizeof(float) + kLevelRecBytes, (size_t)g_field_lds_min);
-  const int64_t n_tiles = (M + 15) / 16;
-  const hipStream_t st = as_stream(s);
-  HybridSchedule hybrid;
-  if (!hybrid.begin(st, n_tiles)) return INR_ELAUNCH;
-  with_flag(numerics & INR_NUMERICS_TABLE_F16, [&](auto half) {
-    with_mlp_f16(numerics & INR_NUMERICS_MLP_F16, [&](auto fast) {
-      launch_field(k_nerf_fwd<true, true, 0, decltype(half)::value, decltype(fast)::value>, lds, n_tiles, st, x01,
-                   nullptr, M, nullptr, bound, t.emb, t.bytes, t.G, f4(packed), density_scale, sigma, rgb, nullptr,
-                   ray_ids, f4(sh_table_q), NerfSave{}, hybrid.cursors());
-    });
-  });
-  hybrid.finish(st);
-  return check_launch("nerf_forward_table");
+  return forward_table_launch<false>(__func__, x01, ray_ids, sh_table_q, M, bound, embeddings, desc, packed,
+                                     density_scale, sigma, rgb, numerics, s);
+}
+
+int inr_ray_table_q(const float* rays_o, const float* rays_d, int64_t N, float* out, inr_stream_t s) {
+  INR_REQUIRE(N >= 0, "bad sizes");
+  if (N == 0) return INR_OK;
+  INR_REQUIRE(rays_o && rays_d && out, "null pointer");
+  INR_REQUIRE(((uintptr_t)out & 15) == 0, "out misaligned");
+  k_ray_table_q<<<blocks_for(N, 256), 256, 0, as_stream(s)>>>(rays_o, rays_d, N, reinterpret_cast<float4*>(out));
+  return check_launch("ray_table_q");
+}
+
+int inr_nerf_forward_table_records(const float* t, const int32_t* ray_ids, const float* ray_table_q, int64_t M, float bound,
+                             const void* embeddings, const inr_grid_desc* desc, const float* packed, float density_scale,
+                             float* sigma, float* rgb, int32_t numerics, inr_stream_t s) {
+  INR_REQUIRE(records_bound_ok(bound), "the records feed needs a power-of-two 2*bound (take the positions feed)");
+  INR_REQUIRE(M >= 0 && desc, "bad argument");
+  if (M == 0) return INR_OK;
+  INR_REQUIRE(t && ray_ids && ray_table_q && embeddings && packed && sigma && rgb, "null pointer");
+  INR_REQUIRE(((uintptr_t)embeddings & 7) == 0 && ((uintptr_t)packed & 15) == 0 && ((uintptr_t)ray_table_q & 15) == 0,
+              "embeddings/packed/ray_table_q misaligned");
+  return forward_table_launch<true>(__func__, t, ray_ids, ray_table_q, M, bound, embeddings, desc, packed, density_scale,
+                                    sigma, rgb, numerics, s);
 }
 
 int64_t inr_nerf_forward_table_sliced_workspace_bytes(int64_t M) {
diff --git a/instance_nerf_amd/csrc/raymarch.hip b/instance_nerf_amd/csrc/raymarch.hip
--- a/instance_nerf_amd/csrc/raymarch.hip
+++ b/instance_nerf_amd/csrc/raymarch.hip
@@ -1,4 +1,5 @@
 #include "common.h"
+#include "sample_pos.h"
 
 namespace inr {
 
@@ -263,9 +264,9 @@
   const StepRule<kConstDt> step(P);
   const float mb1 = fminf(ldexpf(1.0f, 0), P.bound), rmb1 = 1.0f / mb1;
   while (t < far && n < max_emit) {
-    const float px = clampf(r.ox + t * r.dx, -P.bound, P.bound);
-    const float py = clampf(r.oy + t * r.dy, -P.bound, P.bound);
-    const float pz = clampf(r.oz + t * r.dz, -P.bound, P.bound);
+    const float px = sample_pos(r.ox, t, r.dx, P.bound);
+    const float py = sample_pos(r.oy, t, r.dy, P.bound);
+    const float pz = sample_pos(r.oz, t, r.dz, P.bound);
     const float dt = step(P, t);
     int level = 0;
     float mb = mb1, rmb = rmb1;
@@ -444,9 +445,9 @@
         const float dt = step(P, t);
         const float tn = t + dt;
         if (sub & (1u << j)) {
-          const float px = clampf(r.ox + t * r.dx, -P.bound, P.bound);
-          const float py = clampf(r.oy + t * r.dy, -P.bound, P.bound);
-          const float pz = clampf(r.oz + t * r.dz, -P.bound, P.bound);
+          const float px = sample_pos(r.ox, t, r.dx, P.bound);
+          const float py = sample_pos(r.oy, t, r.dy, P.bound);
+          const float pz = sample_pos(r.oz, t, r.dz, P.bound);
           emit(px, py, pz, dt, tn - last_t, t);
           last_t = tn;
           ++emitted;
@@ -516,9 +517,9 @@
       for (int j = 0; j < 63; ++j) c = j < lane ? c + step_dt(P, c) : c;
     }
     const bool in = c < far;
-    const float px = clampf(r.ox + c * r.dx, -P.bound, P.bound);
-    const float py = clampf(r.oy + c * r.dy, -P.bound, P.bound);
-    const float pz = clampf(r.oz + c * r.dz, -P.bound, P.bound);
+    const float px = sample_pos(r.ox, c, r.dx, P.bound);
+    const float py = sample_pos(r.oy, c, r.dy, P.bound);
+    const float pz = sample_pos(r.oz, c, r.dz, P.bound);
     const float dt = step_dt(P, c);
     const float tn = c + dt;
     int level = 0;
@@ -1336,6 +1337,7 @@
   }
 };
 
+template <bool kRec>
 __global__ void __launch_bounds__(kRayBlock) k_march_write_patch(MarchParams P, const float* __restrict__ rays_o,
                                                                  const float* __restrict__ rays_d, int64_t N, int64_t M,
                                                                  const float* __restrict__ nears,
@@ -1354,8 +1356,13 @@
   if (cnt == 0 || (int64_t)cur.S + cur.total() > M) return;
   const Ray r = load_ray(rays_o, rays_d, n);
   const float rb = 2.0f * P.bound;
-  auto emit = [&](float px, float py, float pz, float dt, float delta, float) {
+  auto emit = [&](float px, float py, float pz, float dt, float delta, float t) {
     const int64_t i = cur.next();
+    if constexpr (kRec) {
+      xyzs[i] = t;
+      ray_ids[i] = (int32_t)n;
+      return;
+    }
     if (normalise) {
       px = (px + P.bound) / rb; py = (py + P.bound) / rb; pz = (pz + P.bound) / rb;
     }
@@ -1372,6 +1379,7 @@
   }
 }
 
+template <bool kRec>
 __global__ void __launch_bounds__(kRayBlock) k_composite_patch_fwd(const float* __restrict__ sigmas,
                                                                    const float* __restrict__ rgbs,
                                                                    const float* __restrict__ deltas,
@@ -1379,7 +1387,9 @@
                                                                    float T_thresh, float* __restrict__ wbuf,
                                                                    float* __restrict__ weights_sum,
                                                                    float* __restrict__ depth, float* __restrict__ image,
-                                                                   unsigned long long* __restrict__ skippable) {
+                                                                   unsigned long long* __restrict__ skippable,
+                                                                   MarchParams P, const float* __restrict__ nears,
+                                                                   const float* __restrict__ noises) {
   const int64_t n = (int64_t)blockIdx.x * blockDim.x + threadIdx.x;
   const int lane = threadIdx.x & 63, g0 = lane & ~(kGroup - 1), rr = lane & (kGroup - 1);
   const int32_t rid = n < N ? rays[n * 3] : 0;
@@ -1394,6 +1404,10 @@
 #pragma unroll
   for (int d = 1; d < 64; d <<= 1) maxc = max(maxc, __shfl_xor(maxc, d, 64));
   float T = 1.0f, r = 0, g = 0, b = 0, ws = 0, t = 0, dsum = 0;
+  float last_t = 0.0f;
+  if constexpr (kRec) {
+    if (n < N) last_t = start_t(P, nears[n], noises ? noises[n] : 0.0f);
+  }
   bool done = false;
   unsigned n_skip = 0;
   constexpr int kAhead = 8;
@@ -1410,7 +1424,8 @@
       slot[j] = (int64_t)S + __popc(field[j] & ((1u << rr) - 1u));
       S += __popc(field[j]);
       const int64_t i = (active[j] && !done) ? slot[j] : 0;
-      dl[j] = reinterpret_cast<const float2*>(deltas)[i];
+      if constexpr (kRec) dl[j] = make_float2(deltas[i], 0.0f);
+      else dl[j] = reinterpret_cast<const float2*>(deltas)[i];
       sg[j] = sigmas[i];
       cr[j] = rgbs[i * 3]; cg[j] = rgbs[i * 3 + 1]; cb[j] = rgbs[i * 3 + 2];
     }
@@ -1421,6 +1436,11 @@
         if (rr == 0 && field[j] != 0 && live == 0) n_skip += __popc(field[j]);
       }
       if (active[j] && !done) {
+        if constexpr (kRec) {
+          const float dt = step_dt(P, dl[j].x), tn = dl[j].x + dt;
+          dl[j] = make_float2(dt, tn - last_t);
+          last_t = tn;
+        }
         const float alpha = 1.0f - expf(-sg[j] * dl[j].x);
         const float w = alpha * T;
         r += w * cr[j]; g += w * cg[j]; b += w * cb[j];
@@ -1846,10 +1866,27 @@
   const MarchParams P = make_params(bitfield, bound, dt_gamma, max_steps, cascade, H);
   INR_REQUIRE(sample_cap == 0 || workspace, "sample_cap > 0 needs the workspace of the count pass");
   const uint32_t* mask = sample_cap > 0 ? reinterpret_cast<const uint32_t*>(reinterpret_cast<const int32_t*>(workspace) + ws_ints(N)) : nullptr;
-  k_march_write_patch<<<blocks_for(N, kRayBlock), kRayBlock, march_lds_pad(), as_stream(s)>>>(P, rays_o, rays_d, N, M, nears, fars,
-                                                                                noises, rays, xyzs, dirs, deltas, mask,
-                                                                                cap_words_of(sample_cap), ray_ids, normalise);
+  k_march_write_patch<false><<<blocks_for(N, kRayBlock), kRayBlock, march_lds_pad(), as_stream(s)>>>(
+      P, rays_o, rays_d, N, M, nears, fars, noises, rays, xyzs, dirs, deltas, mask, cap_words_of(sample_cap), ray_ids,
+      normalise);
   return check_launch("march_rays_patch_write");
+}
+
+int inr_march_rays_patch_write_records(const float* rays_o, const float* rays_d, const uint8_t* bitfield, float bound,
+                                       float dt_gamma, int32_t max_steps, int64_t N, int32_t cascade, int32_t H,
+                                       int64_t M, const float* nears, const float* fars, const float* noises,
+                                       const int32_t* rays, float* t, int32_t* ray_ids, const void* workspace,
+                                       int32_t sample_cap, inr_stream_t s) {
+  INR_REQUIRE(rays_o && rays_d && bitfield && nears && fars && rays, "null pointer");
+  INR_REQUIRE(N > 0 && M >= 0, "bad sizes");
+  if (M == 0) return INR_OK;
+  INR_REQUIRE(t && ray_ids, "null output");
+  const MarchParams P = make_params(bitfield, bound, dt_gamma, max_steps, cascade, H);
+  INR_REQUIRE(sample_cap == 0 || workspace, "sample_cap > 0 needs the workspace of the count pass");
+  const uint32_t* mask = sample_cap > 0 ? reinterpret_cast<const uint32_t*>(reinterpret_cast<const int32_t*>(workspace) + ws_ints(N)) : nullptr;
+  k_march_write_patch<true><<<blocks_for(N, kRayBlock), kRayBlock, march_lds_pad(), as_stream(s)>>>(
+      P, rays_o, rays_d, N, M, nears, fars, noises, rays, t, nullptr, nullptr, mask, cap_words_of(sample_cap), ray_ids, 0);
+  return check_launch("march_rays_patch_write_records");
 }
 
 int inr_composite_rays_patch_forward(const float* sigmas, const float* rgbs, const float* deltas, const int32_t* rays,
@@ -1863,13 +1900,36 @@
   INR_REQUIRE(!extra || (extra_out && weights && K > 0 && K <= 64), "extra needs extra_out, weights and 0 < K <= 64");
   INR_REQUIRE(((uintptr_t)deltas & 7) == 0, "deltas must be 8-byte aligned");
   hipStream_t st = as_stream(s);
-  k_composite_patch_fwd<<<blocks_for(N, kRayBlock), kRayBlock, 0, st>>>(sigmas, rgbs, deltas, rays, N, M, T_thresh,
-                                                                        weights, weights_sum, depth, image,
-                                                                        reinterpret_cast<unsigned long long*>(skippable));
+  k_composite_patch_fwd<false><<<blocks_for(N, kRayBlock), kRayBlock, 0, st>>>(
+      sigmas, rgbs, deltas, rays, N, M, T_thresh, weights, weights_sum, depth, image,
+      reinterpret_cast<unsigned long long*>(skippable), MarchParams{}, nullptr, nullptr);
   if (extra_out && K > 0)
     k_composite_patch_extra<<<blocks_for(N * 64, kRayBlock), kRayBlock, 0, st>>>(weights, extra, rays, N, M, K,
                                                                                  extra_out);
   return check_launch("composite_rays_patch_forward");
+}
+
+int inr_composite_rays_patch_forward_records(const float* sigmas, const float* rgbs, const float* t, const int32_t* rays,
+                                             int64_t N, int64_t M, float T_thresh, const float* nears,
+                                             const float* noises, float dt_gamma, int32_t max_steps, int32_t cascade,
+                                             int32_t H, const float* extra, int32_t K, float* weights_sum, float* depth,
+                                             float* image, float* extra_out, float* weights, uint64_t* skippable,
+                                             inr_stream_t s) {
+  INR_REQUIRE(N >= 0 && M >= 0, "bad sizes");
+  if (N == 0) return INR_OK;
+  INR_REQUIRE(rays && nears && weights_sum && depth && image, "null pointer");
+  INR_REQUIRE(M == 0 || (sigmas && rgbs && t), "null sample arrays");
+  INR_REQUIRE(max_steps > 0 && cascade > 0 && H > 0, "bad step parameters");
+  INR_REQUIRE(!extra || (extra_out && weights && K > 0 && K <= 64), "extra needs extra_out, weights and 0 < K <= 64");
+  hipStream_t st = as_stream(s);
+  const MarchParams P = make_params(nullptr, 0.0f, dt_gamma, max_steps, cascade, H);
+  k_composite_patch_fwd<true><<<blocks_for(N, kRayBlock), kRayBlock, 0, st>>>(
+      sigmas, rgbs, t, rays, N, M, T_thresh, weights, weights_sum, depth, image,
+      reinterpret_cast<unsigned long long*>(skippable), P, nears, noises);
+  if (extra_out && K > 0)
+    k_composite_patch_extra<<<blocks_for(N * 64, kRayBlock), kRayBlock, 0, st>>>(weights, extra, rays, N, M, K,
+                                                                                 extra_out);
+  return check_launch("composite_rays_patch_forward_records");
 }
 
 int inr_project_masks_patch(const float* xyzs, const float* weights, const int32_t* rays, int64_t N, int64_t M,
diff --git a/instance_nerf_amd/csrc/sample_pos.h b/instance_nerf_amd/csrc/sample_pos.h
--- /dev/null
+++ b/instance_nerf_amd/csrc/sample_pos.h
@@ -0,0 +1,17 @@
+#pragma once
+#include "common.h"
+
+namespace inr {
+
+__device__ __forceinline__ float sample_pos(float o, float t, float d, float bound) {
+  return clampf(o + t * d, -bound, bound);
+}
+
+__device__ __forceinline__ float sample_x01_pow2(float p, float bound, float rb_inv) { return (p + bound) * rb_inv; }
+
+inline bool records_bound_ok(float bound) {
+  int e = 0;
+  return bound > 0.0f && bound < 1e30f && frexpf(2.0f * bound, &e) == 0.5f && e > -100;
+}
+
+}
diff --git a/instance_nerf_amd/nerf/network.py b/instance_nerf_amd/nerf/network.py
--- a/instance_nerf_amd/nerf/network.py
+++ b/instance_nerf_amd/nerf/network.py
@@ -1,3 +1,4 @@
+import math
 import os
 
 import torch
@@ -449,6 +450,8 @@
         self.frame_slices = __import__("os").environ.get("INR_FRAME_SLICES", "auto")
         self._slice_probe = None
         self.last_frame_path = "fused"
+        self.frame_records = __import__("os").environ.get("INR_FRAME_RECORDS", "1") not in ("0", "off", "False", "false")
+        self.last_frame_feed = "positions"
 
     def _packed_weights(self, which, numerics=0):
         lib = _lib.load()
@@ -616,21 +619,61 @@
               "sh_table_q")
         return shq
 
-    def forward_table(self, x01, ray_ids, rays_d, shq=None):
+    @torch.no_grad()
+    def ray_table(self, rays_o, rays_d):
+        lib = _lib.load()
+        rays_o = rays_o.contiguous().float().view(-1, 3)
+        rays_d = rays_d.contiguous().float().view(-1, 3)
+        rows = torch.empty(rays_d.shape[0], _lib.RAY_TABLE_FLOATS, dtype=torch.float32, device=rays_d.device)
+        check(lib.inr_ray_table_q(ptr(rays_o, torch.float32, "rays_o"), ptr(rays_d, torch.float32, "rays_d"),
+                                  rays_d.shape[0], ptr(rows), stream_ptr()), "ray_table_q")
+        return rows
+
+    def records_apply(self):
+        return bool(self.frame_records and self._fusable and self.bound > 0
+                    and math.frexp(2.0 * float(self.bound))[0] == 0.5)
+
+    def _table_numerics(self):
+        if self.training:
+            return 0
+        return ((_lib.NUMERICS_TABLE_F16 if self.half_table else 0) | (_lib.NUMERICS_MLP_F16 if self.mlp_fp16 else 0))
+
+    def plan_frame(self, M, records=False):
+        numerics = self._table_numerics()
+        sliced = bool(not numerics and self._use_slices(M))
+        settled = bool(numerics) or self.last_frame_path == "fused"
+        feed = "records" if (records and self.records_apply() and not sliced and settled) else "positions"
+        return {"sliced": sliced, "feed": feed}
+
+    def forward_table(self, x01, ray_ids, rays_d, shq=None, rays_o=None, plan=None):
         if not self._fusable:
             return None
         lib = _lib.load()
         M = x01.shape[0]
         dev = x01.device
+        records = x01.dim() == 1
+        if records:
+            if rays_o is None or not self.records_apply():
+                raise ValueError("forward_table: the records feed needs rays_o, a power-of-two 2*bound and frame_records")
+            if plan is not None and plan["feed"] != "records":
+                raise ValueError("forward_table: this frame was planned on the positions feed")
+        if plan is None:
+            plan = {"sliced": False, "feed": "records"} if records else self.plan_frame(M)
         if shq is None:
-            shq = self.sh_table(rays_d)
+            shq = self.ray_table(rays_o, rays_d) if records else self.sh_table(rays_d)
         sigma = torch.empty(M, dtype=torch.float32, device=dev)
         rgb = torch.empty(M, 3, dtype=torch.float32, device=dev)
-        numerics = 0
-        if not self.training:
-            numerics = ((_lib.NUMERICS_TABLE_F16 if self.half_table else 0)
-                        | (_lib.NUMERICS_MLP_F16 if self.mlp_fp16 else 0))
-        if not numerics and self._use_slices(M):
+        numerics = self._table_numerics()
+        self.last_frame_feed = plan["feed"]
+        if records:
+            check(lib.inr_nerf_forward_table_records(ptr(x01, torch.float32, "t", allow_none=M == 0),
+                                               ptr(ray_ids, torch.int32, "ray_ids", allow_none=M == 0), ptr(shq), M,
+                                               float(self.bound), self._table_ptr(self.encoder, numerics),
+                                               self.encoder.desc, ptr(self._packed_weights("nerf", numerics)), 1.0,
+                                               ptr(sigma, allow_none=M == 0), ptr(rgb, allow_none=M == 0), numerics,
+                                               stream_ptr()), "nerf_forward_table_records")
+            return sigma, rgb
+        if plan["sliced"]:
             need = lib.inr_nerf_forward_table_sliced_workspace_bytes(M) // 4
             ws = self.__dict__.get("_slice_ws")
             if ws is None or ws.numel() < need or ws.device != dev:
diff --git a/instance_nerf_amd/nerf/renderer.py b/instance_nerf_amd/nerf/renderer.py
--- a/instance_nerf_amd/nerf/renderer.py
+++ b/instance_nerf_amd/nerf/renderer.py
@@ -298,17 +298,33 @@
         device = rays_o.device
         fused_inst = self.num_instances > 0 and self._fusable_inst
         counter = torch.zeros(2, dtype=torch.int32, device=device)
+        may_record = bool(table and self.num_instances == 0 and self.records_apply())
         early = {}
 
         def while_waiting():
             early["skippable"] = torch.zeros(1, dtype=torch.int64, device=device)
-            if table:
+            if may_record:
+                early["rows"] = self.ray_table(rays_o, rays_d)
+            elif table:
                 early["shq"] = self.sh_table(rays_d)
+
+        def feed_of(M):
+            early["plan"] = self.plan_frame(M, records=may_record)
+            return raymarching.RECORDS if early["plan"]["feed"] == "records" else True
         xyzs, dirs, deltas, rays = raymarching.march_rays_patch(
             rays_o, rays_d, self.bound, self.density_bitfield, self.cascade, self.grid_size, nears, fars,
-            dt_gamma, max_steps, noises=jitter, counter=counter, table=table, while_waiting=while_waiting)
+            dt_gamma, max_steps, noises=jitter, counter=counter, table=feed_of if table else False,
+            while_waiting=while_waiting)
+        records = None
         gate.acquire()
-        sigmas, rgbs = self.forward_table(xyzs, dirs, rays_d, shq=early.get("shq")) if table else self(xyzs, dirs)
+        if not table:
+            sigmas, rgbs = self(xyzs, dirs)
+        elif early["plan"]["feed"] == "records":
+            records = raymarching.MarchRecords(nears, jitter, dt_gamma, max_steps, self.cascade, self.grid_size)
+            sigmas, rgbs = self.forward_table(xyzs, dirs, rays_d, shq=early["rows"], rays_o=rays_o, plan=early["plan"])
+            deltas = xyzs
+        else:
+            sigmas, rgbs = self.forward_table(xyzs, dirs, rays_d, shq=early.get("shq"), plan=early["plan"])
         gate.release()
         if self.density_scale != 1:
             sigmas = self.density_scale * sigmas
@@ -322,10 +338,11 @@
         else:
             weights_sum, depth, image = self._composite_with_logits(
                 raymarching.composite_rays_patch, results, prefix, xyzs, sigmas, rgbs, deltas, rays, T_thresh,
-                skippable=skippable)
+                skippable=skippable, **({"records": records} if records is not None else {}))
         results["num_samples"] = counter
         if table:
             results["frame_path"] = self.last_frame_path
+            results["frame_feed"] = early["plan"]["feed"]
         self._note_skippable(skippable, int(xyzs.shape[0]), False)
         return weights_sum, depth, image
 
diff --git a/instance_nerf_amd/raymarching.py b/instance_nerf_amd/raymarching.py
--- a/instance_nerf_amd/raymarching.py
+++ b/instance_nerf_amd/raymarching.py
@@ -169,6 +169,8 @@
     return xyzs, dirs, deltas, rays
 
 
+RECORDS = "records"
+
 GROUP = 16
 
 
@@ -209,6 +211,16 @@
                                          ptr(counter, I32, "counter"), ptr(ws), cap, stream_ptr()),
           "march_rays_train_count")
     M = _read_count(counter, while_waiting)
+    if callable(table):
+        table = table(M)
+    if table == RECORDS:
+        t = torch.empty(M, dtype=F32, device=dev)
+        ray_ids = torch.empty(M, dtype=I32, device=dev)
+        check(lib.inr_march_rays_patch_write_records(
+            *args, M, ptr(nears), ptr(fars), ptr(noises, F32, "noises", allow_none=True), ptr(rays),
+            ptr(t, allow_none=M == 0), ptr(ray_ids, allow_none=M == 0), ptr(ws), cap, stream_ptr()),
+            "march_rays_patch_write_records")
+        return t, ray_ids, None, rays
     xyzs = torch.empty(M, 3, dtype=F32, device=dev)
     dirs = None if table else torch.empty(M, 3, dtype=F32, device=dev)
     ray_ids = torch.empty(M, dtype=I32, device=dev) if table else None
@@ -221,7 +233,15 @@
     return xyzs, (ray_ids if table else dirs), deltas, rays
 
 
-def composite_rays_patch(sigmas, rgbs, deltas, rays, T_thresh=1e-4, extra=None, return_weights=False, skippable=None):
+class MarchRecords:
+
+    def __init__(self, nears, noises, dt_gamma, max_steps, C, H):
+        self.nears, self.noises = _f(nears), (_f(noises) if noises is not None else None)
+        self.dt_gamma, self.max_steps, self.C, self.H = float(dt_gamma), int(max_steps), int(C), int(H)
+
+
+def composite_rays_patch(sigmas, rgbs, deltas, rays, T_thresh=1e-4, extra=None, return_weights=False, skippable=None,
+                         records=None):
     lib = _lib.load()
     sigmas, rgbs, deltas = _f(sigmas), _f(rgbs), _f(deltas)
     dev = rays.device
@@ -233,6 +253,19 @@
     extra_out = torch.empty(N, K, dtype=F32, device=dev) if K else None
     wbuf = torch.empty(max(M, 1), dtype=F32, device=dev) if (K or return_weights) else None
     none_ok = M == 0
+    if records is not None:
+        if deltas.dim() != 1 or records.nears.shape[0] != N:
+            raise ValueError("composite_rays_patch(records=): t [M] and the nears of the N marched rays are needed")
+        check(lib.inr_composite_rays_patch_forward_records(
+            ptr(sigmas, F32, "sigmas", allow_none=none_ok), ptr(rgbs, F32, "rgbs", allow_none=none_ok),
+            ptr(deltas, F32, "t", allow_none=none_ok), ptr(rays, I32, "rays"), N, M, float(T_thresh),
+            ptr(records.nears, F32, "nears"), ptr(records.noises, F32, "noises", allow_none=True), records.dt_gamma,
+            records.max_steps, records.C, records.H, ptr(_f(extra) if extra is not None else None, allow_none=True), K,
+            ptr(ws), ptr(depth), ptr(image), ptr(extra_out, allow_none=True), ptr(wbuf, allow_none=True),
+            ptr(skippable, torch.int64, "skippable", allow_none=True), stream_ptr()),
+            "composite_rays_patch_forward_records")
+        out = (ws, depth, image) + ((extra_out,) if K else ())
+        return out + ((wbuf,) if return_weights else ())
     check(lib.inr_composite_rays_patch_forward(
         ptr(sigmas, F32, "sigmas", allow_none=none_ok), ptr(rgbs, F32, "rgbs", allow_none=none_ok),
         ptr(deltas, F32, "deltas", allow_none=none_ok), ptr(rays, I32, "rays"), N, M, float(T_thresh),
```

After: 6775 Msamples/s (median of 6 runs). 3.6% higher.
